# mbdriscoll/indigo

Hardware: AMD Instinct MI355X
Metric: SENSE AHA evals/sec (256^3 x 8-coil non-Cartesian) (higher is better)
Workload: dtype complex64 (f32)

## Files before the change

indigo_amd/backends/hip_csr.py:

```python
import logging

import numpy as np

from indigo_amd import _lib, grid_formats
from indigo_amd._lib import cplx as _cplx
from indigo_amd.backends.backend import Backend

log = logging.getLogger(__name__)
_C64 = np.dtype('complex64')

_BRICK_ARRAYS = dict(tasks=".brickTasks", table=".brickTable", entries=".brickEntries", rounds=".brickRoundRows", shared=".sharedBricks")
_SLOT_ARRAYS = dict(tasks=".slotTasks", table=".slotTable", entries=".slotEntries", slot_ptr=".slotPtr", shared=".slotSharedBricks")
_SHARE_ARRAYS = dict(tasks=".shareTasks", table=".shareTable", shares=".shares", shared=".shareSharedBricks")
_WIDE_ARRAYS = dict(owned=".wideOwnedTiles", tasks=".wideTasks", table=".wideTable", entries=".wideEntries", rows=".wideEntryRows")
_RUN_ARRAYS = dict(order=".runOrder", dptr=".runPtr", dcols=".runCols", entries=".runEntries")


def _ptr(a):
    return None if a is None else a._arr


class csr_matrix(Backend.csr_matrix):

    def __init__(self, backend, A, name='mat'):
        super().__init__(backend, A, name)
        self._host_csr = A if A.dtype == _C64 else A.astype(_C64)
        self._perm = self._sep = self._grid_dims = None
        self._support, self._support_host, self._support_zw = None, None, 16
        self._support_fine, self._support_fine_by, self._support_fine_host_by = None, {}, {}
        self._bricks, self._bricks_by, self._slots, self._slots_by, self._shares_by = None, {}, None, {}, {}
        self._invalidate()

    def _invalidate(self):
        self._t = None
        self._weights_real = None
        self._xrows = None
        self._values_re = self._runs_fmt = None
        self._wide = False
        self._tried = set()

    def _upload(self, fmt, names):
        if fmt is None:
            return None
        b = self._backend
        return dict(fmt, **{key: b.copy_array(fmt[key], name=self._name + suffix) for key, suffix in names.items() if fmt[key] is not None})

    def _host(self, part):
        if self._host_csr is not None:
            return getattr(self._host_csr, part)
        return dict(indptr=self.rowPtrs, indices=self.colInds, data=self.values)[part].to_host()

    def _transposed(self):
        if self._t is None:
            b = self._backend
            pt, it, dt = b.csr_transpose(self._host_csr)
            self._t = (b.copy_array(pt, name=self._name + ".T.rowPtrs"),
                       b.copy_array(it, name=self._name + ".T.colInds"),
                       b.copy_array(dt, name=self._name + ".T.data"))
            self._host_csr = None
        return self._t

    def set_grid_support(self, table, n0, nm, zw=16):
        self._support = (self._backend.copy_array(np.ascontiguousarray(table, dtype=np.int16).reshape(-1),
                                                  name=self._name + ".support"), int(n0), int(nm))
        self._support_zw = int(zw)
        self._support_host = table

    def set_grid_support_fine(self, table, tile, ncols=None):
        built, key = self._bricks_by, None if ncols is None else int(ncols)
        assert not (any(v is not None for v in built.values()) if key is None else built.get(key) is not None), \
            "set_grid_support_fine must come before set_grid_bricks: the runs of bricks are sized for the table's segments"
        assert int(tile) in (4, 8, 16)
        self._support_fine = (self._backend.copy_array(np.ascontiguousarray(table, dtype=np.int16).reshape(-1),
                                                       name=self._name + ".supportFine"), int(tile))
        self._support_fine_by[key] = self._support_fine
        self._support_fine_host_by[key] = (table, int(tile))

    def _format(self, which, ncols, exact=False):
        by = getattr(self, which + '_by')
        key = None if ncols is None else int(ncols)
        if key in by or exact:
            return by.get(key)
        return by.get(None)

    def _fine_tile(self, ncols):
        fine = self._format('_support_fine', ncols)
        return fine[1] if fine is not None else 16

    def set_grid_bricks(self, n0, nm, ns, ncols=8, bm=2, bs=2, chunk=4096, run=4096):
        A = self._host_csr
        assert A is not None and A.shape[1] == n0 * nm * ns
        fmt = grid_formats.bricks(A.indptr, A.indices, A.data, n0, nm, ns, ncols, bm, bs, chunk, run,
                                  tile=self._fine_tile(ncols), real_entries=self._real_weights(A.data))
        if fmt is None:
            log.info("%s: no brick-binned format (%s); the adjoint keeps the gather route", self._name, _lib.last_error(None))
        self._bricks = self._bricks_by[int(ncols)] = self._upload(fmt, _BRICK_ARRAYS)

    def set_grid_slots(self, n0, nm, ns, ncols=1, bm=2, bs=2, chunk=256, run=128):
        A = self._host_csr
        assert A is not None and A.shape[1] == n0 * nm * ns
        fmt = grid_formats.slots(A.indptr, A.indices, A.data, n0, nm, ns, ncols, bm, bs, chunk, run,
                                 tile=self._fine_tile(ncols), real_entries=self._real_weights(A.data))
        if fmt is None:
            log.info("%s: no slot format; the adjoint keeps the gather route", self._name)
        self._slots = self._slots_by[int(ncols)] = self._upload(fmt, _SLOT_ARRAYS)

    def set_grid_separable(self, sep):
        n0, nm, ns = (int(v) for v in sep['dims'])
        assert sep['records'].shape[0] == self.shape[0] and n0 * nm * ns == self.shape[1]
        rec = np.ascontiguousarray(sep['records'])
        self._sep = dict(tw=int(sep['tw']), dims=(n0, nm, ns), gconst=complex(sep['gconst']), host=rec, stride=rec.shape[1],
                         records=self._backend.copy_array(rec.reshape(-1), name=self._name + ".sepRecords"), recx=None, stride_x=0, order={})

    def _gather_order(self, ncols):
        by = self._sep['order']
        if ncols not in by:
            order = grid_formats.gather_order(self._sep['host'], self._sep['tw'], ncols)
            by[ncols] = None if order is None else self._backend.copy_array(order, name=self._name + ".gatherOrder%d" % ncols)
        return by[ncols]

    def set_grid_shares(self, ncols=8, bm=8, bs=2, chunk=1024, run=1024):
        sep = self._sep
        assert sep is not None
        fine = self._format('_support_fine_host', ncols)
        tab, tile = fine if fine is not None else (self._support_host, 16)
        fmt = grid_formats.shares(sep['host'], sep['tw'], sep['dims'], ncols, bm, bs, chunk, run,
                                  table=tab, tile=tile, zw=self._support_zw)
        if fmt is None:
            log.info("%s: no share format; the adjoint keeps the stored-tap routes", self._name)
        elif sep['recx'] is None:
            recx, sep['stride_x'] = grid_formats.records_with_rows(sep['host'])
            sep['recx'] = self._backend.copy_array(recx, name=self._name + ".sepRecordsWithRows")
        self._shares_by[int(ncols)] = self._upload(fmt, _SHARE_ARRAYS)

    def set_grid_dims(self, n0, nm, ns):
        assert int(n0) * int(nm) * int(ns) == self.shape[1]
        self._grid_dims = (int(n0), int(nm), int(ns))
        self._wide = False
        self._tried.discard('wide')

    def _dims(self):
        return self._grid_dims or grid_formats.guess_grid_dims(self.shape[1])

    def _wide_bricks(self):
        if 'wide' not in self._tried:
            self._tried.add('wide')
            t, data = self._backend.tuning, self._host('data')
            self._wide = self._upload(grid_formats.wide_bricks(
                self._host('indptr'), self._host('indices'), data, self.shape[1], self._dims(),
                t.get('wide_brick_shape', (2, 2)), t.get('wide_task_shape', (8192, 2048)), real_entries=self._real_weights(data)), _WIDE_ARRAYS)
        return self._wide

    def _touched(self):
        if self._xrows is None:
            b = self._backend
            indices = self._host('indices')
            mark = np.zeros(self.shape[1], dtype=bool)
            mark[indices] = True
            touched = np.flatnonzero(mark).astype(np.int32)
            compact = np.searchsorted(touched, indices).astype(np.int32)
            self._xrows = (b.copy_array(touched, name=self._name + ".touchedCols"), b.copy_array(compact, name=self._name + ".compactColInds"))
        return self._xrows

    def _runs(self, sub):
        if 'runs' not in self._tried:
            self._tried.add('runs')
            fmt = grid_formats.runs(self._host('indptr'), sub[1].to_host(), self._host('data'), sub[0].to_host(), self._dims(),
                                    self._backend.tuning.get('runs_order', True))
            if fmt is None:
                log.info("%s: no run format (%s); the forward product keeps the per-nonzero gather", self._name, _lib.last_error(None))
            self._runs_fmt = self._upload(fmt, _RUN_ARRAYS)
        return self._runs_fmt

    def set_row_order(self, perm):
        b = self._backend
        perm = np.ascontiguousarray(perm, dtype=np.int32)
        assert self._host_csr is not None and perm.shape == (self.shape[0],)
        Ap = self._host_csr[perm]
        Ap.sort_indices()
        self.rowPtrs = b.copy_array(Ap.indptr.astype(np.int32), name=self._name + ".rowPtrs")
        self.colInds = b.copy_array(Ap.indices.astype(np.int32), name=self._name + ".colInds")
        self.values = b.copy_array(Ap.data.astype(_C64), name=self._name + ".data")
        self._host_csr = Ap
        self._invalidate()
        self._perm = b.copy_array(perm, name=self._name + ".rowOrder")

    def _real_weights(self, data):
        if not self._backend.tuning.get('real_entries', True):
            return False
        if self._weights_real is None:
            self._weights_real = grid_formats.weights_are_real(data)
        return self._weights_real

    def _real_values(self):
        if 'values_re' not in self._tried:
            self._tried.add('values_re')
            data = self._host('data')
            if self._real_weights(data):
                self._values_re = self._backend.copy_array(np.ascontiguousarray(data.real, dtype=np.float32), name=self._name + ".dataRe")
        return self._values_re

    def forward_route(self, ncols):
        t = self._backend.tuning
        if self._grid_il:
            if self._sep is not None and ncols in (2, 4, 8) and t.get('sep_gather', True):
                return 'sep'
            return 'il_rw' if ncols in (2, 4, 8) and self._real_values() is not None else 'il'
        if self._perm is None and 16 <= ncols <= 64 and self._col_frac <= 0.6 and self.values.size >= self.shape[1] and t['xrows']:
            sub = self._touched()
            return 'xrows_runs' if ncols == 64 and t.get('runs', True) and sub[0].size * 512 < 2 ** 32 and self._runs(sub) is not None else 'xrows'
        return 'csr' if self._perm is None else 'rowperm'

    def adjoint_route(self, ncols, beta, y):
        b, perm = self._backend, self._perm
        scatter = perm is None and beta == 0 and y.contiguous
        shf = self._format('_shares', ncols, exact=True)
        if shf is not None and scatter and self._grid_il and shf['ntasks'] > 0 and b.tuning.get('sep_scatter', True):
            return 'shares'
        br = self._format('_bricks', ncols, exact=True)
        if br is not None and scatter and self._grid_il and ncols == br['ncols']:
            return 'bricks'
        sl = self._format('_slots', ncols, exact=True)
        if sl is not None and scatter and ncols == sl['ncols'] and sl['ntasks'] > 0:
            return 'slots'
        if (ncols == 64 and beta == 0 and perm is None and not self._grid_il and self.shape[1] % 16 == 0
# ... 107 lines not shown
```

indigo_amd/csrc/ig_fft.hip:

```cpp
#include "ig_common.h"
#include "ig_packed.h"
#include "ig_fft_ab.h"
#include "ig_fft_ab_list.h"
#include "ig_fft_zc.h"
#include <array>
#include <vector>
#include <functional>
#include <algorithm>
#include <cmath>
#include <cmath>
#include <cstring>
#include <string>
#include <memory>
#include <complex>

namespace {

constexpr int MAX_STAGES = 16;
constexpr int E = 8;
constexpr int LDS_NMAX = 4096;
constexpr size_t LDS_BUDGET = 150 * 1024;

struct Radices { int r[MAX_STAGES]; };

// ... 137 lines not shown
            z[0][r] = x[r];
#pragma unroll
            for (int q = 1; q < 4; ++q) z[q][r] = mul_w32(x[r + q * M], r * q * (32 / N));
        }
#pragma unroll
        for (int q = 0; q < 4; ++q) RegFFT<M>::run(z[q]);
#pragma unroll
        for (int q = 0; q < 4; ++q)
#pragma unroll
            for (int k = 0; k < M; ++k) x[4 * k + q] = z[q][k];
    }
};

template <int N> struct RegFFTHalfIn {
    __device__ static __forceinline__ void run(float2 (&x)[N]) {
        constexpr int M = N / 4;
        float2 z[4][M];
#pragma unroll
        for (int r = 0; r < M; ++r) {
            const float2 a1 = x[r + M], a2 = x[r + 2 * M];
            const float2 t3 = mul_mi(a1);
            z[0][r] = cadd(a2, a1);
            z[1][r] = mul_w32(csub(t3, a2), r * (32 / N));
            z[2][r] = mul_w32(csub(a2, a1), r * 2 * (32 / N));
            const float2 s = cadd(a2, t3);
            z[3][r] = mul_w32(make_float2(-s.x, -s.y), r * 3 * (32 / N));
        }
#pragma unroll
        for (int q = 0; q < 4; ++q) RegFFT<M>::run(z[q]);
#pragma unroll
        for (int q = 0; q < 4; ++q)
#pragma unroll
            for (int k = 0; k < M; ++k) x[4 * k + q] = z[q][k];
    }
};

__device__ __forceinline__ void pbfly2(cx& a, cx& b) { const cx t = a - b; a = a + b; b = t; }
template <bool INV = false, bool ASM = true>
__device__ __forceinline__ void pbfly4(cx& a0, cx& a1, cx& a2, cx& a3) {
    const cx t0 = a0 + a2, t1 = a0 - a2, t2 = a1 + a3, dd = a1 - a3;
    a0 = t0 + t2; a2 = t0 - t2;
    if (ASM) {
        a1 = INV ? padd_pi(t1, dd) : padd_mi(t1, dd);
        a3 = INV ? padd_mi(t1, dd) : padd_pi(t1, dd);
    } else {
        const cx t3 = INV ? cmul_pi_c(dd) : cmul_mi_c(dd);
        a1 = t1 + t3; a3 = t1 - t3;
    }
}
template <bool INV = false, bool ASM = true>
__device__ __forceinline__ cx pmul_w32(cx a, int j) {
    j &= 31;
    if (INV) j = (32 - j) & 31;
    if (j == 0) return a;
    if (j == 8) return ASM ? cmul_mi(a) : cmul_mi_c(a);
    if (j == 16) return cneg(a);
    if (j == 24) return ASM ? cmul_pi(a) : cmul_pi_c(a);
    const float c = cos32(j), s = -cos32(j + 24);
    return cxmul(a, mk(c, s));
}
template <int N, bool INV = false, bool ASM = true> struct PFFT;
template <bool INV, bool ASM> struct PFFT<4, INV, ASM> {
    __device__ static __forceinline__ void run(cx (&x)[4]) { pbfly4<INV, ASM>(x[0], x[1], x[2], x[3]); }
};
template <bool INV, bool ASM> struct PFFT<8, INV, ASM> {
    __device__ static __forceinline__ void run(cx (&v)[8]) {
        pbfly4<INV, ASM>(v[0], v[2], v[4], v[6]);
        pbfly4<INV, ASM>(v[1], v[3], v[5], v[7]);
        const float h = 0.70710678118654752440f;
        v[3] = cxmul(v[3], mk(h, INV ? h : -h));
        v[7] = cxmul(v[7], mk(-h, INV ? h : -h));
        pbfly2(v[0], v[1]); pbfly2(v[2], v[3]); pbfly2(v[6], v[7]);
        if (ASM) {
            const cx e = v[4], o = v[5];
            v[4] = INV ? padd_pi(e, o) : padd_mi(e, o);
            v[5] = INV ? padd_mi(e, o) : padd_pi(e, o);
        } else {
            v[5] = INV ? cmul_pi_c(v[5]) : cmul_mi_c(v[5]);
            pbfly2(v[4], v[5]);
        }
        const cx x4 = v[1], x1 = v[2], x5 = v[3], x2 = v[4], x6 = v[5], x3 = v[6];
        v[1] = x1; v[2] = x2; v[3] = x3; v[4] = x4; v[5] = x5; v[6] = x6;
    }
};
template <int N, bool INV, bool ASM> struct PFFT {
    __device__ static __forceinline__ void run(cx (&x)[N]) {
        constexpr int M = N / 4;
        cx z[4][M];
#pragma unroll
        for (int r = 0; r < M; ++r) {
            pbfly4<INV, ASM>(x[r], x[r + M], x[r + 2 * M], x[r + 3 * M]);
            z[0][r] = x[r];
#pragma unroll
            for (int q = 1; q < 4; ++q) z[q][r] = pmul_w32<INV, ASM>(x[r + q * M], r * q * (32 / N));
        }
#pragma unroll
        for (int q = 0; q < 4; ++q) PFFT<M, INV, ASM>::run(z[q]);
#pragma unroll
        for (int q = 0; q < 4; ++q)
#pragma unroll
            for (int k = 0; k < M; ++k) x[4 * k + q] = z[q][k];
    }
};
template <int N> struct PFFTHalfIn {
    __device__ static __forceinline__ void run(cx (&x)[N]) {
        constexpr int M = N / 4;
        cx z[4][M];
#pragma unroll
        for (int r = 0; r < M; ++r) {
            const cx a1 = x[r + M], a2 = x[r + 2 * M];
            z[0][r] = a2 + a1;
            z[1][r] = pmul_w32(cneg(padd_pi(a2, a1)), r * (32 / N));
            z[2][r] = pmul_w32(a2 - a1, r * 2 * (32 / N));
            z[3][r] = pmul_w32(cneg(padd_mi(a2, a1)), r * 3 * (32 / N));
        }
#pragma unroll
        for (int q = 0; q < 4; ++q) PFFT<M>::run(z[q]);
#pragma unroll
        for (int q = 0; q < 4; ++q)
#pragma unroll
            for (int k = 0; k < M; ++k) x[4 * k + q] = z[q][k];
    }
};

template <int R1, int R2, int T, int W, bool AXIS0, int WMODE, bool BOXED, int HALF>
__global__ void __launch_bounds__(W * T, (!AXIS0 && R1 == 32 && (W == 32 || HALF == 1 || HALF == 3)) ? 4 : 1)
k_fft_2stage(PassDesc d, const float2* __restrict__ tw) {
    constexpr int n = R1 * R2, B1 = R2 / T, B2 = R1 / T, NT = W * T;
    constexpr bool NT_LD = true, NT_ST = true;
    constexpr bool HALF_IN = HALF == 1 || HALF == 3, HALF_OUT = HALF == 2 || HALF == 4;
    constexpr int SUMW = WMODE >= 3 ? (1 << (WMODE - 3)) : 0;
    constexpr bool SINV = HALF_OUT;
    const bool inv = (HALF_OUT || HALF_IN) ? false : (d.inverse != 0);
    static_assert(R2 % T == 0 && R1 % T == 0 && T == 16 && B1 == 1, "lane groups of 16, one stage-1 butterfly per thread");
    extern __shared__ float2 lds[];
    float2* __restrict__ tws = lds + (AXIS0 ? 16 * 17 * W : 16 * T * W);
    const int tid = threadIdx.x;
    constexpr int TWN = n / NT;
    constexpr bool TW_LATE = (n % NT == 0) && TWN <= 2;
    float2 tw_mine[TW_LATE ? TWN : 1];
    if (TW_LATE) {
#pragma unroll
        for (int i = 0; i < TWN; ++i) tw_mine[i] = tw[n + tid + i * NT];
    } else for (int k = tid; k < n; k += NT) tws[k] = tw[n + k];

    const int t = AXIS0 ? (tid % T) : (tid / W);
    const int w = AXIS0 ? (tid / T) : (tid % W);
    unsigned tr, k1, k2;
    pass_tile(d, tr, k1, k2);
    const int64_t k0u = (int64_t)tr * ((!AXIS0 && d.cw) ? (d.cw_log2 >= 0 ? W >> d.cw_log2 : W / d.cw) : W);
    int in_lo = d.in_lo, in_hi = d.in_hi, out_lo = d.out_lo, out_hi = d.out_hi;
    short2 k1r = make_short2(0, 0x7fff), trg = make_short2(0, 0x7fff);
    PassRecords rcd{0u, 0u, 0x7fff0000u, 0xffffffffu, false, false, false, true, false};
    if (BOXED && !AXIS0) rcd = pass_records(d, tw, tr, k1, 16, t, true);
    const bool has_k1r = rcd.has_k1r, has_trg = rcd.has_trg, has_zb = rcd.has_zb;
    int64_t o_in = k0u * d.in_s[0], o_out = k0u * d.out_s[0];
    if (BOXED && !AXIS0 && WMODE == 0 && d.zc_log2) {
        const int64_t q = k0u >> d.zc_log2, e = k0u - (q << d.zc_log2);
        if (d.in_zt) o_in = q * d.in_zt + e;
        if (d.out_zt) o_out = q * d.out_zt + e;
    }
    const float2* const b_in = d.in + (o_in + (int64_t)k1 * d.in_s[1] + (int64_t)k2 * d.in_s[2]);
    float2* const b_out = d.out + (o_out + (int64_t)k1 * d.out_s[1] + (int64_t)k2 * d.out_s[2]);
    const float2* const b_w = WMODE ? d.w + (k0u * d.w_s[0] + (int64_t)k1 * d.w_s[1] + (int64_t)k2 * d.w_s[2]) : nullptr;
    const rsrc_t r_in = make_rsrc(b_in), r_out = make_rsrc(b_out), r_w = make_rsrc(b_w);
    const unsigned isj = AXIS0 ? 1u : (unsigned)d.in_sj, osj = AXIS0 ? 1u : (unsigned)d.out_sj, wsj = AXIS0 ? 1u : (unsigned)d.w_sj;
    bool valid;
    unsigned l_in, l_out, l_w;
    if (!AXIS0 && d.cw) {
        const unsigned yl = d.cw_log2 >= 0 ? (unsigned)w >> d.cw_log2 : (unsigned)w / (unsigned)d.cw, a = (unsigned)w - yl * (unsigned)d.cw;
        valid = k0u + yl < d.ext0;
        l_in = (a * (unsigned)d.in_sa + yl * (unsigned)d.in_s[0] + (unsigned)t * isj) * 8u;
        l_out = (a * (unsigned)d.out_sa + yl * (unsigned)d.out_s[0] + (unsigned)t * osj) * 8u;
        l_w = (a * (unsigned)d.w_sa + yl * (unsigned)d.w_s[0] + (unsigned)t * wsj) * 8u;
    } else {
        valid = k0u + w < d.ext0;
        l_in = ((unsigned)w * (unsigned)d.in_s[0] + (unsigned)t * isj) * 8u;
        l_out = ((unsigned)w * (unsigned)d.out_s[0] + (unsigned)t * osj) * 8u;
        l_w = ((unsigned)w * (unsigned)d.w_s[0] + (unsigned)t * wsj) * 8u;
    }
    if (!valid) l_in = l_out = l_w = IG_OOB;
    if (!WMODE) l_w = IG_OOB;
    if (SUMW && (w % SUMW) != 0) l_out = IG_OOB;
    if (has_k1r) k1r = rcd.k1_hull();
    if (has_k1r) {
        if ((int)k1 < k1r.x || (int)k1 >= k1r.y) return;
    }
    const bool defer_out = HALF_IN && has_trg && d.tile_range_mode == 1 && (rcd.scalar || has_k1r);
    if (has_trg && !defer_out) {
        const short2 r = trg = rcd.range();
        if (d.tile_range_mode == 1) {
            out_lo = out_lo > r.x ? out_lo : r.x;
            out_hi = out_hi < r.y ? out_hi : r.y;
            if (out_hi <= out_lo) return;
        } else {
            in_lo = in_lo > r.x ? in_lo : r.x;
            in_hi = in_hi < r.y ? in_hi : r.y;
        }
    }

    auto ceil16 = [](int a) -> int { a += 15; return a <= 0 ? 0 : (a >= 512 ? 32 : a >> 4); };
    auto below = [](int h) -> uint32_t { return h >= 32 ? 0xffffffffu : ((1u << h) - 1u); };
    uint32_t ibits = 0xffffffffu, obits = 0xffffffffu;
    if (BOXED) {
        ibits = below(ceil16(in_hi - t)) & ~below(ceil16(in_lo - t));
        if (has_zb && d.tile_range_mode != 1) ibits &= rcd.bits();
    }
    uint32_t gin = 0xffffffffu;
    if (BOXED && !AXIS0 && WMODE == 0 && !HALF_IN && HALF != 4) {
        gin = 0;
#pragma unroll
        for (int l = 0; l < 64; l += W) gin |= (uint32_t)__builtin_amdgcn_readlane((int)ibits, l);
    }
    constexpr bool GATE_ST = BOXED && !AXIS0 && WMODE == 0 && !HALF_OUT && HALF != 3;
    uint32_t gout = 0xffffffffu;
    constexpr int GRP = 4;
    auto opaque = [](const float2*& q) { asm("" : "+s"(q)); };
    cx v[R1];
    {
        cx wv[R1];
        constexpr int K0 = HALF_IN ? R1 / 4 : 0, K1 = HALF_IN ? 3 * R1 / 4 : R1;
        const int64_t st_in = (int64_t)R2 * d.in_sj, st_w = WMODE == 1 ? (int64_t)R2 * d.w_sj : 0;
        const unsigned so_in = (unsigned)st_in * 8u, so_w = (unsigned)st_w * 8u;
        const float2* p_in = AXIS0 ? b_in : b_in + K0 * st_in;
        const float2* p_w = (AXIS0 || WMODE != 1) ? b_w : b_w + K0 * st_w;
        rsrc_t g_in = make_rsrc(p_in), g_w = make_rsrc(p_w);
#pragma unroll
        for (int k = K0; k < K1; ++k) {
            const int g = (k - K0) % GRP;
            if (!AXIS0 && g == 0 && k > K0) {
                p_in += GRP * st_in; opaque(p_in); g_in = make_rsrc(p_in);
                if (WMODE == 1) { p_w += GRP * st_w; opaque(p_w); g_w = make_rsrc(p_w); }
            }
            const bool stat = !BOXED || HALF_IN || HALF == 4;
            const unsigned off = stat ? 0u : (unsigned)__builtin_amdgcn_sbfe((int)~ibits, k, 1);
            if (!stat && !AXIS0 && WMODE == 0 && !((gin >> k) & 1u)) v[k] = mk(0.f, 0.f);
            else if (AXIS0) {
                v[k] = from2(buf_ld<NT_LD>(r_in, l_in | off, (unsigned)(k * R2) * 8u));
                if (WMODE == 1) wv[k] = from2(buf_ld<false>(r_w, l_w | off, (unsigned)(k * R2) * 8u));
            } else {
                v[k] = from2(buf_ld<NT_LD>(g_in, l_in | off, (unsigned)g * so_in));
                if (WMODE == 1) wv[k] = from2(buf_ld<false>(g_w, l_w | off, (unsigned)g * so_w));
            }
        }
#pragma unroll
        for (int k = K0; k < K1; ++k) {
            if (WMODE == 1) v[k] = cxmul_r(v[k], wv[k]);
            if (inv) v[k] = cconj(v[k]);
        }
    }
    if (defer_out) {
        trg = rcd.range();
        out_lo = out_lo > trg.x ? out_lo : trg.x;
        out_hi = out_hi < trg.y ? out_hi : trg.y;
    }
    if (BOXED) {
        obits = below(ceil16(out_hi - t)) & ~below(ceil16(out_lo - t));
        if (has_zb && d.tile_range_mode == 1) obits &= rcd.bits();
    }
    if (GATE_ST) {
        gout = 0;
#pragma unroll
        for (int l = 0; l < 64; l += W) gout |= (uint32_t)__builtin_amdgcn_readlane((int)obits, l);
    }
    if (TW_LATE) {
#pragma unroll
        for (int i = 0; i < TWN; ++i) tws[tid + i * NT] = tw_mine[i];
    }
    __syncthreads();
    if (HALF_IN) PFFTHalfIn<R1>::run(v);
    else PFFT<R1, SINV>::run(v);
    {
        const float2* __restrict__ twt = tws + t * R1;
#pragma unroll
        for (int k = 1; k < R1; ++k) v[k] = SINV ? cxmulc(from2(twt[k]), v[k]) : cxmul_r(v[k], from2(twt[k]));
    }

    float2* __restrict__ lw = AXIS0 ? lds + w * (16 * 17) + t * 17 : lds + (t * 16) * W + w;
    float2* __restrict__ lr = AXIS0 ? lds + w * (16 * 17) + t      : lds + t * W + w;
#pragma unroll
    for (int q = 0; q < B2; ++q) {
        if (q > 0) __syncthreads();
#pragma unroll
        for (int kk = 0; kk < 16; ++kk) lw[kk * (AXIS0 ? 1 : W)] = to2(v[16 * q + kk]);
        __syncthreads();
        cx u[R2];
#pragma unroll
        for (int r = 0; r < R2; ++r) u[r] = from2(lr[r * (AXIS0 ? 17 : 16 * W)]);
        PFFT<R2, SINV>::run(u);
        constexpr int Q0 = HALF_OUT ? R2 / 4 : 0, Q1 = HALF_OUT ? 3 * R2 / 4 : R2;
        const int64_t st_out = (int64_t)R1 * d.out_sj, st_w = WMODE >= 2 ? (int64_t)R1 * d.w_sj : 0;
        const unsigned so_out = (unsigned)st_out * 8u, so_w = (unsigned)st_w * 8u;
        const float2* p_out = AXIS0 ? b_out : b_out + (q * T) * d.out_sj + Q0 * st_out;
        const float2* p_w = (AXIS0 || WMODE < 2) ? b_w : b_w + (q * T) * d.w_sj + Q0 * st_w;
        cx wv[R2];
        if (WMODE >= 2) {
            rsrc_t g_w = make_rsrc(p_w);
#pragma unroll
            for (int r = Q0; r < Q1; ++r) {
                const int g = (r - Q0) % GRP;
                if (!AXIS0 && g == 0 && r > Q0) { p_w += GRP * st_w; opaque(p_w); g_w = make_rsrc(p_w); }
                const bool stat = !BOXED || HALF_OUT || HALF == 3;
                const unsigned off = stat ? 0u : (unsigned)__builtin_amdgcn_sbfe((int)~obits, q + r * B2, 1);
                if (AXIS0) wv[r] = from2(buf_ld<false>(r_w, l_w | off, (unsigned)(q * T + r * R1) * 8u));
                else wv[r] = from2(buf_ld<false>(g_w, l_w | off, (unsigned)g * so_w));
            }
        }
        rsrc_t g_out = make_rsrc(p_out);
        v4i_t gw_out = make_rsrc_words(p_out);
#pragma unroll
        for (int r = Q0; r < Q1; ++r) {
            const int g = (r - Q0) % GRP;
            if (!AXIS0 && g == 0 && r > Q0) {
                p_out += GRP * st_out; opaque(p_out);
                if (GATE_ST) gw_out = make_rsrc_words(p_out); else g_out = make_rsrc(p_out);
            }
            const bool stat = !BOXED || HALF_OUT || HALF == 3;
            cx ac = u[r];
            if (inv) ac = cconj(ac);
            if (WMODE >= 2) ac = cxmulc(wv[r], ac);
            float2 a = to2(ac);
            const unsigned off = stat ? 0u : (unsigned)__builtin_amdgcn_sbfe((int)~obits, q + r * B2, 1);
            if (SUMW) {
                if (SUMW >= 2)  { a.x += dpp_f<0xB1>(a.x);  a.y += dpp_f<0xB1>(a.y); }
                if (SUMW >= 4)  { a.x += dpp_f<0x4E>(a.x);  a.y += dpp_f<0x4E>(a.y); }
                if (SUMW >= 8)  { a.x += dpp_f<0x104>(a.x); a.y += dpp_f<0x104>(a.y); }
                if (SUMW >= 16) { a.x += dpp_f<0x108>(a.x); a.y += dpp_f<0x108>(a.y); }
            }
            if (AXIS0) buf_st<NT_ST>(r_out, l_out | off, (unsigned)(q * T + r * R1) * 8u, a);
            else if (GATE_ST) buf_st_gated<NT_ST>(gw_out, l_out | off, (unsigned)g * so_out, a, (gout >> (q + r * B2)) & 1u);
            else buf_st<NT_ST>(g_out, l_out | off, (unsigned)g * so_out, a);
        }
    }
}


constexpr bool F3A_NT_LD = true, F3A_NT_ST = false, F3B_NT_LD = false, F3B_NT_ST = false;
constexpr int F3_LDS_ELEMS = 64 * 72;

__device__ __forceinline__ void wave_sync() {
    __builtin_amdgcn_fence(__ATOMIC_RELEASE, "wavefront");
    __builtin_amdgcn_wave_barrier();
    __builtin_amdgcn_fence(__ATOMIC_ACQUIRE, "wavefront");
}

__global__ void __launch_bounds__(512, 4)
k_fft3d_a(const float2* __restrict__ in, float2* __restrict__ out, const float2* __restrict__ tw, int inverse) {
    extern __shared__ float2 lds[];
    float2* __restrict__ tws = lds + F3_LDS_ELEMS;
    const int tid = threadIdx.x;
    for (int k = tid; k < 256; k += 512) tws[k] = tw[k];
    const unsigned lin = blockIdx.x + gridDim.x * (blockIdx.y + gridDim.y * blockIdx.z), tot = gridDim.x * gridDim.y * gridDim.z;
    const unsigned logical = (lin & 7u) * (tot >> 3) + (lin >> 3);
    const int n2 = (int)(logical & 3u), z = (int)((logical >> 2) & 255u);
    const int64_t base = ((int64_t)(logical >> 10) << 24) + ((int64_t)z << 16);
    const int xl = tid & 63, a = tid >> 6;
    const bool inv = inverse != 0;

    cx v[4][8];
    {
        const int a_u = __builtin_amdgcn_readfirstlane(a);
        const rsrc_t r_in = make_rsrc(in + base + 256 * n2 + 1024 * a_u);
#pragma unroll
        for (int b = 0; b < 8; ++b)
#pragma unroll
            for (int j = 0; j < 4; ++j) {
                v[j][b] = from2(buf_ld<F3A_NT_LD>(r_in, (unsigned)xl * 8u, (unsigned)(64 * j + 8192 * b) * 8u));
                if (inv) v[j][b] = cconj(v[j][b]);
            }
    }
    __syncthreads();
#pragma unroll
    for (int j = 0; j < 4; ++j) {
        PFFT<8, false, false>::run(v[j]);
#pragma unroll
        for (int kb = 1; kb < 8; ++kb) v[j][kb] = cxmul(v[j][kb], from2(tws[(4 * a * kb) & 255]));
    }
    cx r[4][8];
    float2* __restrict__ img1 = lds + F3_LDS_ELEMS + 256;
#pragma unroll
    for (int jp = 0; jp < 2; ++jp) {
        if (jp) __syncthreads();
#pragma unroll
        for (int kb = 0; kb < 8; ++kb) {
            lds[(a * 8 + kb) * 64 + xl] = to2(v[2 * jp][kb]);
            img1[(a * 8 + kb) * 64 + xl] = to2(v[2 * jp + 1][kb]);
        }
        __syncthreads();
#pragma unroll
        for (int ap = 0; ap < 8; ++ap) {
            r[2 * jp][ap] = from2(lds[(ap * 8 + a) * 64 + xl]);
            r[2 * jp + 1][ap] = from2(img1[(ap * 8 + a) * 64 + xl]);
        }
    }
    const int kb = a;
    cx p[8][4];
#pragma unroll
    for (int j = 0; j < 4; ++j) PFFT<8, false, false>::run(r[j]);
#pragma unroll
    for (int ka = 0; ka < 8; ++ka) {
        const cx wy = from2(tws[(n2 * (kb + 8 * ka)) & 255]);
        cx t4[4];
#pragma unroll
        for (int j = 0; j < 4; ++j) t4[j] = cxmul(r[j][ka], wy);
        PFFT<4, false, false>::run(t4);
        p[ka][0] = t4[0];
#pragma unroll
        for (int kj = 1; kj < 4; ++kj) p[ka][kj] = cxmul(t4[kj], from2(tws[(xl * kj) & 255]));
    }
    const int c = tid & 7, l = (tid >> 3) & 7, line = (tid >> 3);
    cx q[4][8];
#pragma unroll
    for (int jp = 0; jp < 2; ++jp) {
        __syncthreads();
#pragma unroll
        for (int ka = 0; ka < 8; ++ka) {
// ... 329 lines not shown
    const int64_t blocks = (ncols + anyfft::AB_W - 1) / anyfft::AB_W;
    IG_REQUIRE(ctx, blocks <= 0x7fffffffLL, "ig_fft_exec: too many tiles");
    const dim3 grid((unsigned)blocks), block((unsigned)(anyfft::AB_W * ax.ab_B));
    const bool ax0 = ax.inner == 1;
    int r = ig_ab_launch_part0(ctx->stream, ax.n, ax0, grid, block, ax.lds_bytes, in, out, ax.d_tw, ax.inner, ncols, inverse);
    if (!r) r = ig_ab_launch_part1(ctx->stream, ax.n, ax0, grid, block, ax.lds_bytes, in, out, ax.d_tw, ax.inner, ncols, inverse);
    if (!r) r = ig_ab_launch_part2(ctx->stream, ax.n, ax0, grid, block, ax.lds_bytes, in, out, ax.d_tw, ax.inner, ncols, inverse);
    if (!r) r = ig_ab_launch_part3(ctx->stream, ax.n, ax0, grid, block, ax.lds_bytes, in, out, ax.d_tw, ax.inner, ncols, inverse);
    if (r == 2) return ig_fail(ctx, IG_ERR_UNSUPPORTED, "ig_fft_exec: device %d refused %zu bytes of LDS for the %lld-point kernel", ctx->device, ax.lds_bytes, (long long)ax.n);
    if (!r) return ig_fail(ctx, IG_ERR_UNSUPPORTED, "ig_fft_exec: no A x B kernel for n = %lld", (long long)ax.n);
    IG_LAUNCH_CHECK(ctx, "k_fft_ab");
    return IG_OK;
}

int plan_chirp(ig_ctx* ctx, AxisPlan& ax, int64_t m);

int64_t chirp_ab_length(int64_t n, int& A, int& B) {
    int64_t m = 0;
    for (int64_t c = 2 * n - 1; c <= 1024 && c * 100 <= (2 * n - 1) * 108; ++c)
        if (ab_split(c, A, B)) { if (!m) m = c; if (B % 4 == 0) { m = c; break; } }
    for (int64_t c = 2 * n - 1; c <= 1024 && !m; ++c) if (ab_split(c, A, B)) m = c;
    if (m) ab_split(m, A, B);
    return m;
}

int plan_axis(ig_ctx* ctx, ig_fft* p, int a) {
    AxisPlan& ax = p->axis[a];
    ax.n = p->dims[a];
    ax.inner = 1;
    for (int d = 0; d < a; ++d) ax.inner *= p->dims[d];
    ax.outer = p->total / (ax.n * ax.inner);
    if (ax.n == 1) { ax.kind = 2; return IG_OK; }

    const bool force_generic = ctx->opt_fft_kernels == 2;
    Radices rad{};
    int ns = 0;
    const bool two_stage = !force_generic && (ax.n == 512 || ax.n == 256) &&
                           32 * ax.inner * 8 < 0x7fffffffLL;
    if (two_stage) {
        ax.kind = 3; ax.W = 16; ax.T = 16; ax.nstages = 2;
        ax.rad.r[0] = ax.n == 512 ? 32 : 16; ax.rad.r[1] = 16;
        ax.lds_bytes = ((size_t)16 * 17 * ax.W + ax.n) * 8;
    }
    const bool use_ab = ctx->opt_fft_kernels == 0;
    bool ab = false;
    if (!two_stage && !force_generic && use_ab) {
        int A = 0, B = 0;
        if (ab_split(ax.n, A, B)) {
            ab = true;
            ax.kind = 4; ax.ab_A = A; ax.ab_B = B; ax.W = anyfft::AB_W; ax.T = B; ax.nstages = 2;
            ax.rad.r[0] = A; ax.rad.r[1] = B;
            ax.lds_bytes = ab_lds(ax.n, ax.inner == 1);
        }
    }
    bool lds_ok = !ab && !two_stage && !force_generic && ax.n <= LDS_NMAX && factor_lds(ax.n, rad, ns);
    if (lds_ok) {
        int T = 1;
        for (int s = 0; s < ns; ++s) {
            const int R = rad.r[s];
            const int bpt = E / R;
            const int nb = (int)(ax.n / R);
            const int need = (nb + bpt - 1) / bpt;
            if (need > T) T = need;
        }
        int W = 16;
        while (W > 1 && ((int64_t)W * T > 1024 || ((size_t)ax.n * (W + 1) + ax.n) * 8 > 72 * 1024)) W >>= 1;
        while (W < 64 && (int64_t)(W * 2) * T <= 256 && ((size_t)ax.n * (2 * W + 1) + ax.n) * 8 <= 72 * 1024) W <<= 1;
        const size_t lds = ((size_t)ax.n * (W + 1) + ax.n) * 8;
        if ((int64_t)W * T > 1024 || lds > LDS_BUDGET) lds_ok = false;
        else {
            ax.kind = 0; ax.rad = rad; ax.nstages = ns; ax.W = W; ax.T = T; ax.lds_bytes = lds;
            if (lds > 48 * 1024) {
                IG_HIP(ctx, hipFuncSetAttribute(reinterpret_cast<const void*>(&k_fft_lds<true>),
                                                hipFuncAttributeMaxDynamicSharedMemorySize, (int)LDS_BUDGET));
                IG_HIP(ctx, hipFuncSetAttribute(reinterpret_cast<const void*>(&k_fft_lds<false>),
                                                hipFuncAttributeMaxDynamicSharedMemorySize, (int)LDS_BUDGET));
            }
        }
    }
    if (!lds_ok && !two_stage && !ab) {
        ax.kind = 1;
        factor_generic(ax.n, ax.gen_radices);
        ax.nstages = (int)ax.gen_radices.size();
        int64_t big = 1;
        for (int64_t r : ax.gen_radices) big = std::max(big, r);
        if (big > 7 && ax.n >= 32 && ctx->opt_fft_kernels == 0 && !p->is_chirp_sub) {
            int A = 0, B = 0;
            int64_t m = chirp_ab_length(ax.n, A, B);
            Radices r2{};
            int ns2 = 0;
            for (int64_t c = 2 * ax.n - 1; c <= LDS_NMAX && !m; ++c) if (factor_lds(c, r2, ns2)) m = c;
            if (m) {
                if (int rc = plan_chirp(ctx, ax, m)) return rc;
                ax.kind = 5;
            }
        }
    }
    const size_t ntw = (size_t)ax.n * (ax.kind == 3 ? 2 : 1);
    std::vector<float2> tw(ntw);
    for (int64_t k = 0; k < ax.n; ++k) {
        const double ang = -2.0 * M_PI * (double)k / (double)ax.n;
        tw[k] = make_float2((float)cos(ang), (float)sin(ang));
    }
    if (ax.kind == 3) {
        const int64_t R1 = ax.n / 16;
        for (int64_t t = 0; t < 16; ++t)
            for (int64_t k = 0; k < R1; ++k) tw[ax.n + t * R1 + k] = tw[(t * k) % ax.n];
    }
    IG_HIP(ctx, hipMalloc((void**)&ax.d_tw, sizeof(float2) * ntw));
    IG_HIP(ctx, hipMemcpy(ax.d_tw, tw.data(), sizeof(float2) * ntw, hipMemcpyHostToDevice));
    return IG_OK;
}

static dim3 pass_grid(PassDesc& d, int64_t tpr) {
    d.tpr = (unsigned)tpr;
    d.cw_log2 = -1;
    if (d.cw > 0 && (d.cw & (d.cw - 1)) == 0) { d.cw_log2 = 0; while ((1 << d.cw_log2) < d.cw) ++d.cw_log2; }
    const int64_t rows = d.ncols / d.ext0, ext2 = d.ext1 > 0 ? rows / d.ext1 : 0;
    d.grid3 = (d.ext1 >= 1 && d.ext1 <= 65535 && ext2 >= 1 && ext2 <= 65535 && d.ext1 * ext2 == rows) ? 1 : 0;
    return d.grid3 ? dim3((unsigned)tpr, (unsigned)d.ext1, (unsigned)ext2) : dim3((unsigned)(tpr * rows));
}

static int pass_tiles(ig_ctx* ctx, PassDesc& d, int64_t cpt, int64_t reach, bool weights, const char* kernel, dim3& grid) {
    const int64_t tpr = (d.ext0 + cpt - 1) / cpt;
    const int64_t blocks = tpr * (d.ncols / d.ext0);
    IG_REQUIRE(ctx, blocks <= 0x7fffffffLL && d.ext1 <= 0x7fffffffLL, "ig_fft: too many tiles");
    grid = pass_grid(d, tpr);
    const int64_t lim = 0x7fffffffLL / 8;
    const int64_t span_in = reach * d.in_sj + 15 * d.in_s[0] + 15 * d.in_sa, span_out = reach * d.out_sj + 15 * d.out_s[0] + 15 * d.out_sa;
    const int64_t span_w = weights ? reach * d.w_sj + 15 * d.w_s[0] + 15 * d.w_sa : 0;
    IG_REQUIRE(ctx, d.in_sj >= 0 && d.out_sj >= 0 && d.in_s[0] >= 0 && d.out_s[0] >= 0 && span_in < lim && span_out < lim && span_w < lim,
               "ig_fft: axis stride too large for the %s kernel", kernel);
    return IG_OK;
}

static bool two_stage_variant(const AxisPlan& ax, const PassDesc& d, bool axis0, int wmode, bool& boxed, int& half) {
    boxed = d.tile_range || !(d.in_lo <= 0 && d.in_hi >= (int)ax.n && d.out_lo <= 0 && d.out_hi >= (int)ax.n);
    const int qn = (int)ax.n / 4;
    half = 0;
    if (boxed) {
        const bool in_full = d.in_lo <= 0 && d.in_hi >= (int)ax.n, out_full = d.out_lo <= 0 && d.out_hi >= (int)ax.n;
        if (d.in_lo == qn && d.in_hi == 3 * qn && !(d.tile_range && d.tile_range_mode == 2))
            half = (out_full && !d.tile_range && !d.tile_bits) ? 3 : 1;
        else if (d.out_lo == qn && d.out_hi == 3 * qn && !(d.tile_range && d.tile_range_mode == 1))
            half = (in_full && !d.tile_range && !d.tile_bits) ? 4 : 2;
        if (wmode == 1 && half != 3) half = 0;
        if (wmode >= 2 && half != 4) half = 0;
        if (((half == 1 || half == 3) && d.inverse) || ((half == 2 || half == 4) && !d.inverse)) half = 0;
    }
    const bool big_stride = (d.in_sj > d.out_sj ? d.in_sj : d.out_sj) * 8 >= (1 << 20);
    const bool w32_generic = half == 0 && (big_stride || d.tile_bits != nullptr);
    const bool w32 = (ax.n == 512 && !axis0 && wmode == 0 && !d.cw && d.ext0 % 32 == 0 &&
        (half == 1 || half == 3 || half == 2 || half == 4 || w32_generic) &&
        (!d.tile_range || d.tile_shift >= 1));
    return d.wide ? d.wide == 2 : w32;
}

int launch_2stage(ig_ctx* ctx, const AxisPlan& ax, const PassDesc& d_in, bool axis0, int wmode) {
    PassDesc d = d_in;
    if (d.ncols == 0) return IG_OK;
    IG_REQUIRE(ctx, !d.tile_bits || d.tile_words == 16 || d.tile_words == 0, "ig_fft: the two-stage kernel reads support bitmaps of 16 words per entry (got %d)", d.tile_words);
    const int64_t cpt = (!axis0 && d.cw) ? ax.W / d.cw : ax.W;
    IG_REQUIRE(ctx, !d.cw || (!axis0 && d.cw <= ax.W && ax.W % d.cw == 0), "ig_fft: bad lane split");
    dim3 grid;
    if (int rc = pass_tiles(ctx, d, cpt, axis0 ? ax.n + 15 : 3 * (ax.n / 16) + 15, wmode != 0, "two-stage", grid)) return rc;
    const dim3 block((unsigned)(ax.W * ax.T));
#define IG_2S(R1_, AX0_, WM_, BX_, HF_)                                                             \
    hipLaunchKernelGGL((k_fft_2stage<R1_, 16, 16, 16, AX0_, WM_, BX_, HF_>), grid, block, ax.lds_bytes, ctx->stream, d, ax.d_tw)
#define IG_2S_W(R1_, AX0_)                                                                           \
    do {                                                                                             \
        if (!boxed && wmode == 0) IG_2S(R1_, AX0_, 0, false, 0);                                     \
        else if (wmode == 0) {                                                                       \
            if (half == 1) IG_2S(R1_, AX0_, 0, true, 1); else if (half == 2) IG_2S(R1_, AX0_, 0, true, 2);   \
            else if (half == 3) IG_2S(R1_, AX0_, 0, true, 3); else if (half == 4) IG_2S(R1_, AX0_, 0, true, 4); \
            else IG_2S(R1_, AX0_, 0, true, 0); }                                                     \
        else if (wmode == 1) { if (half == 3) IG_2S(R1_, AX0_, 1, true, 3); else IG_2S(R1_, AX0_, 1, true, 0); } \
        else { if (half == 4) IG_2S(R1_, AX0_, 2, true, 4); else IG_2S(R1_, AX0_, 2, true, 0); }      \
    } while (0)
    bool boxed; int half;
    const bool w32 = two_stage_variant(ax, d, axis0, wmode, boxed, half);
    if (w32) {
        PassDesc d2 = d;
        if (d2.tile_range) d2.tile_shift = d.tile_shift - 1;
        const dim3 g2 = pass_grid(d2, d.ext0 / 32), b2(512);
        const size_t lds2 = ((size_t)16 * 16 * 32 + 512) * 8;
        if (!ctx->fft_w32_attr) {
            IG_HIP(ctx, hipFuncSetAttribute(reinterpret_cast<const void*>(&k_fft_2stage<32, 16, 16, 32, false, 0, true, 1>), hipFuncAttributeMaxDynamicSharedMemorySize, (int)lds2));
            IG_HIP(ctx, hipFuncSetAttribute(reinterpret_cast<const void*>(&k_fft_2stage<32, 16, 16, 32, false, 0, true, 3>), hipFuncAttributeMaxDynamicSharedMemorySize, (int)lds2));
            IG_HIP(ctx, hipFuncSetAttribute(reinterpret_cast<const void*>(&k_fft_2stage<32, 16, 16, 32, false, 0, true, 2>), hipFuncAttributeMaxDynamicSharedMemorySize, (int)lds2));
            IG_HIP(ctx, hipFuncSetAttribute(reinterpret_cast<const void*>(&k_fft_2stage<32, 16, 16, 32, false, 0, true, 4>), hipFuncAttributeMaxDynamicSharedMemorySize, (int)lds2));
            IG_HIP(ctx, hipFuncSetAttribute(reinterpret_cast<const void*>(&k_fft_2stage<32, 16, 16, 32, false, 0, true, 0>), hipFuncAttributeMaxDynamicSharedMemorySize, (int)lds2));
            ctx->fft_w32_attr = true;
        }
        if (half == 0) hipLaunchKernelGGL((k_fft_2stage<32, 16, 16, 32, false, 0, true, 0>), g2, b2, lds2, ctx->stream, d2, ax.d_tw);
        else if (half == 1) hipLaunchKernelGGL((k_fft_2stage<32, 16, 16, 32, false, 0, true, 1>), g2, b2, lds2, ctx->stream, d2, ax.d_tw);
        else if (half == 3) hipLaunchKernelGGL((k_fft_2stage<32, 16, 16, 32, false, 0, true, 3>), g2, b2, lds2, ctx->stream, d2, ax.d_tw);
        else if (half == 2) hipLaunchKernelGGL((k_fft_2stage<32, 16, 16, 32, false, 0, true, 2>), g2, b2, lds2, ctx->stream, d2, ax.d_tw);
        else hipLaunchKernelGGL((k_fft_2stage<32, 16, 16, 32, false, 0, true, 4>), g2, b2, lds2, ctx->stream, d2, ax.d_tw);
    } else
    if (wmode == 3) {
        IG_REQUIRE(ctx, !axis0 && d.cw >= 1, "ig_fft: the coil-summing pass is a strided pass with a lane split");
#define IG_2S_SUM(R1_, HF_) do { switch (d.cw) { case 1: IG_2S(R1_, false, 3, true, HF_); break; case 2: IG_2S(R1_, false, 4, true, HF_); break; \
                                 case 4: IG_2S(R1_, false, 5, true, HF_); break; case 8: IG_2S(R1_, false, 6, true, HF_); break;              \
                                 default: IG_2S(R1_, false, 7, true, HF_); break; } } while (0)
        if (ax.n == 512) { if (half == 4) IG_2S_SUM(32, 4); else IG_2S_SUM(32, 0); }
        else             { if (half == 4) IG_2S_SUM(16, 4); else IG_2S_SUM(16, 0); }
#undef IG_2S_SUM
    } else
    if (ax.n == 512) { if (axis0) IG_2S_W(32, true); else IG_2S_W(32, false); }
    else             { if (axis0) IG_2S_W(16, true); else IG_2S_W(16, false); }
#undef IG_2S_W
#undef IG_2S
    IG_LAUNCH_CHECK(ctx, "k_fft_2stage");
    return IG_OK;
}

bool abd_supported(int64_t n) {
#define IG_ABD_CASE(A_, B_, R_) if (n == (A_) * (B_)) return true;
    IG_ABD_LIST(IG_ABD_CASE)
#undef IG_ABD_CASE
    return false;
}
int launch_ab_desc(ig_ctx* ctx, const AxisPlan& ax, const PassDesc& d_in, int wmode) {
    PassDesc d = d_in;
    if (d.ncols == 0) return IG_OK;
    IG_REQUIRE(ctx, !d.cw || (d.cw <= anyfft::AB_W && anyfft::AB_W % d.cw == 0), "ig_fft: bad lane split");
    IG_REQUIRE(ctx, !d.tile_bits || d.tile_words == (d.tile_range_mode == 1 ? ax.ab_A : ax.ab_B), "ig_fft: the support bitmap has %d words per entry, this pass needs %d",
               d.tile_words, d.tile_range_mode == 1 ? ax.ab_A : ax.ab_B);
    const int64_t cpt = d.cw ? anyfft::AB_W / d.cw : anyfft::AB_W;
    dim3 grid;
    if (int rc = pass_tiles(ctx, d, cpt, ax.ab_B - 1, wmode != 0, "two-stage", grid)) return rc;
    int wm = wmode;
    if (wmode == 3) {
        IG_REQUIRE(ctx, d.cw == 2 || d.cw == 4 || d.cw == 8 || d.cw == 16, "ig_fft: the coil-summing A x B pass takes 2, 4, 8 or 16 interleaved coils");
        wm = d.cw == 2 ? 4 : d.cw == 4 ? 5 : d.cw == 8 ? 6 : 7;
    }
    const dim3 block((unsigned)(anyfft::AB_W * ax.ab_B));
    int r = ig_abd_launch_part0(ctx->stream, ax.n, wm, grid, block, d, ax.d_tw);
    if (!r) r = ig_abd_launch_part1(ctx->stream, ax.n, wm, grid, block, d, ax.d_tw);
    if (!r) r = ig_abd_launch_part2(ctx->stream, ax.n, wm, grid, block, d, ax.d_tw);
    if (!r) r = ig_abd_launch_part3(ctx->stream, ax.n, wm, grid, block, d, ax.d_tw);
    if (r == 2) return ig_fail(ctx, IG_ERR_UNSUPPORTED, "ig_fft: device %d refused the LDS the %lld-point zero-pad-aware kernel needs", ctx->device, (long long)ax.n);
    if (!r)
        return ig_fail(ctx, IG_ERR_UNSUPPORTED, "ig_fft: no zero-pad-aware kernel for n = %lld", (long long)ax.n);
    IG_LAUNCH_CHECK(ctx, "k_fft_ab_desc");
    return IG_OK;
}

int plan_chirp(ig_ctx* ctx, AxisPlan& ax, int64_t m) {
    auto ch = std::make_shared<Chirp>();
    ch->m = m;
    const int64_t n = ax.n;
    {
        ig_fft tmp;
        tmp.ctx = ctx; tmp.is_chirp_sub = true; tmp.rank = 3; tmp.batch = 1;
        tmp.dims[0] = ax.inner; tmp.dims[1] = m; tmp.dims[2] = ax.outer;
        tmp.total = ax.inner * m * ax.outer;
        if (int rc = plan_axis(ctx, &tmp, 1)) return rc;
        ch->sub = tmp.axis[1];
        tmp.axis[1].d_tw = nullptr;
    }
    IG_REQUIRE(ctx, ch->sub.kind == 0 || ch->sub.kind == 3 || ch->sub.kind == 4, "ig_fft_plan: no fast kernel for the chirp-z length %lld", (long long)m);
    ch->fused = ch->sub.kind == 4 && ax.inner >= 16;
    typedef std::complex<double> cd;
    std::vector<cd> b((size_t)n), h((size_t)m, cd(0, 0)), H((size_t)m);
    for (int64_t j = 0; j < n; ++j) {
        const double ang = -M_PI * (double)((j * j) % (2 * n)) / (double)n;
        b[j] = cd(cos(ang), sin(ang));
    }
    h[0] = cd(1, 0);
    for (int64_t j = 1; j < n; ++j) h[j] = h[m - j] = std::conj(b[j]);
    {
        std::vector<double> cs((size_t)m);
        for (int64_t k = 0; k < m; ++k) cs[k] = cos(2.0 * M_PI * (double)k / (double)m);
        for (int64_t k = 0; k < m; ++k) {
            cd acc = h[0];
            for (int64_t j = 1; j < n; ++j) acc += 2.0 * h[j] * cs[(j * k) % m];
            H[k] = acc;
        }
    }
    std::vector<float2> t((size_t)m);
    auto upload = [&](float2*& dst, const std::function<cd(int64_t)>& f) -> int {
        for (int64_t k = 0; k < m; ++k) { const cd v = f(k); t[k] = make_float2((float)v.real(), (float)v.imag()); }
        IG_HIP(ctx, hipMalloc((void**)&dst, sizeof(float2) * (size_t)m));
        IG_HIP(ctx, hipMemcpy(dst, t.data(), sizeof(float2) * (size_t)m, hipMemcpyHostToDevice));
        return IG_OK;
    };
    for (int dir = 0; dir < 2; ++dir) {
        auto cj = [dir](cd v) { return dir ? std::conj(v) : v; };
        if (int rc = upload(ch->d_b[dir], [&](int64_t k) { return k < n ? cj(b[k]) : cd(0, 0); })) return rc;
        if (int rc = upload(ch->d_bhat[dir], [&](int64_t k) { return cj(H[k]); })) return rc;
        if (int rc = upload(ch->d_bout[dir], [&](int64_t k) { return k < n ? cj(b[k]) / (double)m : cd(0, 0); })) return rc;
        IG_HIP(ctx, hipMalloc((void**)&ch->d_hat_out[dir], sizeof(float2) * 2 * (size_t)m));
        IG_HIP(ctx, hipMemcpy(ch->d_hat_out[dir], ch->d_bhat[dir], sizeof(float2) * (size_t)m, hipMemcpyDeviceToDevice));
        IG_HIP(ctx, hipMemcpy(ch->d_hat_out[dir] + m, ch->d_bout[dir], sizeof(float2) * (size_t)m, hipMemcpyDeviceToDevice));
    }
    ax.chirp = ch;
    return IG_OK;
}

int plan_chirp_shift(ig_ctx* ctx, Chirp& ch, int64_t n, int64_t c) {
    typedef std::complex<double> cd;
    const int64_t m = ch.m;
    for (int d = 0; d < 2; ++d) {
        if (ch.d_in_s[d]) { (void)hipFree(ch.d_in_s[d]); ch.d_in_s[d] = nullptr; }
        if (ch.d_hat_out_s[d]) { (void)hipFree(ch.d_hat_out_s[d]); ch.d_hat_out_s[d] = nullptr; }
    }
    ch.shift = c;
    if (c == 0) return IG_OK;
    auto bt = [n](int64_t t) { const double ang = -M_PI * (double)((t * t) % (2 * n)) / (double)n; return cd(cos(ang), sin(ang)); };
    std::vector<double> cs((size_t)m), sn((size_t)m);
    for (int64_t k = 0; k < m; ++k) { cs[k] = cos(2.0 * M_PI * (double)k / (double)m); sn[k] = sin(2.0 * M_PI * (double)k / (double)m); }
    std::vector<float2> t((size_t)(2 * m));
    for (int dir = 0; dir < 2; ++dir) {
        std::vector<cd> h((size_t)m, cd(0, 0)), H((size_t)m);
        for (int64_t u = -(n - 1); u <= n - 1; ++u)
            h[(size_t)((u % m + m) % m)] = dir == 0 ? std::conj(bt(u + c)) : bt(u - c);
        for (int64_t k = 0; k < m; ++k) {
            cd acc(0, 0);
            for (int64_t u = 0; u < m; ++u) {
                if (h[u] == cd(0, 0)) continue;
                const int64_t q = (u * k) % m;
                acc += h[u] * cd(cs[q], -sn[q]);
            }
            H[k] = acc;
        }
        for (int64_t j = 0; j < m; ++j) {
            const cd v = j < n ? (dir == 0 ? bt(j - c) : std::conj(bt(j))) : cd(0, 0);
            t[j] = make_float2((float)v.real(), (float)v.imag());
        }
        IG_HIP(ctx, hipMalloc((void**)&ch.d_in_s[dir], sizeof(float2) * (size_t)m));
        IG_HIP(ctx, hipMemcpy(ch.d_in_s[dir], t.data(), sizeof(float2) * (size_t)m, hipMemcpyHostToDevice));
        for (int64_t k = 0; k < m; ++k) {
            t[k] = make_float2((float)H[k].real(), (float)H[k].imag());
            const cd v = k < n ? (dir == 0 ? bt(k) : std::conj(bt(k - c))) / (double)m : cd(0, 0);
            t[m + k] = make_float2((float)v.real(), (float)v.imag());
// ... 168 lines not shown
            d.in_sj = d.out_sj = ax.inner; d.w_sj = 0;
            d.ncols = ax.inner * ax.outer;
            if (ax.inner == 1) {
                d.ext0 = ax.outer; d.ext1 = 1; d.in_s[0] = d.out_s[0] = ax.n; d.in_s[1] = d.out_s[1] = 0;
            } else {
                d.ext0 = ax.inner; d.ext1 = ax.outer; d.in_s[0] = d.out_s[0] = 1; d.in_s[1] = d.out_s[1] = ax.inner * ax.n;
            }
            d.in_s[2] = d.out_s[2] = 0;
            d.in_lo = d.out_lo = 0; d.in_hi = d.out_hi = (int)ax.n; d.inverse = inv;
            return launch_2stage(ctx, ax, d, ax.inner == 1, 0);
        }
        if (ax.kind == 4) {
            ig_prof_scope prof(ctx, a == 0 ? "fft_ab_axis0" : a == 1 ? "fft_ab_axis1" : "fft_ab_axis2", bytes);
            return launch_ab(ctx, ax, in, out, inv);
        }
        IG_REQUIRE(ctx, ax.kind == 0, "ig_fft_exec: not a fast axis");
        ig_prof_scope prof(ctx, a == 0 ? "fft_lds_axis0" : a == 1 ? "fft_lds_axis1" : "fft_lds_axis2", bytes);
        const int64_t ncols = ax.inner * ax.outer;
        const int64_t blocks = (ncols + ax.W - 1) / ax.W;
        IG_REQUIRE(ctx, blocks <= 0x7fffffffLL, "ig_fft_exec: too many tiles");
        const dim3 grid((unsigned)blocks), block((unsigned)(ax.W * ax.T));
        if (ax.inner == 1)
            hipLaunchKernelGGL(k_fft_lds<true>, grid, block, ax.lds_bytes, ctx->stream, in, out, ax.d_tw,
                               (int)ax.n, ax.inner, ncols, ax.W, ax.T, ax.nstages, ax.rad, inv);
        else
            hipLaunchKernelGGL(k_fft_lds<false>, grid, block, ax.lds_bytes, ctx->stream, in, out, ax.d_tw,
                               (int)ax.n, ax.inner, ncols, ax.W, ax.T, ax.nstages, ax.rad, inv);
        IG_LAUNCH_CHECK(ctx, "k_fft_lds");
        return IG_OK;
    };
    for (int a = 0; a < p->rank; ++a) {
        const AxisPlan& ax = p->axis[a];
        if (ax.kind == 2) continue;
        if (ax.kind == 0 || ax.kind == 3 || ax.kind == 4) {
            if (int rc = fast_axis(ax, cur, y, inverse, a, pass_bytes)) return rc;
            cur = y;
        } else if (ax.kind == 5) {
            const Chirp& ch = *ax.chirp;
            const int dir = inverse ? 1 : 0;
            if (cur == work) {
                IG_HIP(ctx, hipMemcpyAsync(y, cur, (size_t)p->total * 8, hipMemcpyDeviceToDevice, ctx->stream));
                cur = y;
            }
            if (ch.fused) {
                ig_prof_scope prof(ctx, a == 1 ? "fft_chirp_axis1" : "fft_chirp_axis2", pass_bytes);
                PassDesc d{};
                d.in = cur; d.in_sj = ax.inner; d.in_s[0] = 1; d.in_s[1] = ax.inner * ax.n;
                d.out = y; d.out_sj = ax.inner; d.out_s[0] = 1; d.out_s[1] = ax.inner * ax.n;
                d.ext0 = ax.inner; d.ext1 = ax.outer; d.ncols = ax.inner * ax.outer;
                d.in_lo = d.out_lo = 0; d.in_hi = d.out_hi = (int)ax.n; d.inverse = inverse;
                if (int rc = launch_chirp_desc(ctx, ax, d)) return rc;
            } else {
                const int64_t total_m = p->total / ax.n * ch.m;
                int64_t g = (total_m + 255) / 256;
                const int64_t cap = (int64_t)ctx->num_cu * 16;
                if (g > cap) g = cap;
                {
                    ig_prof_scope prof(ctx, "fft_chirp_pre");
                    hipLaunchKernelGGL(k_chirp_pre, dim3((unsigned)g), dim3(256), 0, ctx->stream, cur, work, ch.d_b[dir], ax.n, ch.m, ax.inner, total_m);
                    IG_LAUNCH_CHECK(ctx, "k_chirp_pre");
                }
                if (int rc = fast_axis(ch.sub, work, work, 0, a, 0.0)) return rc;
                {
                    ig_prof_scope prof(ctx, "fft_chirp_mul");
                    hipLaunchKernelGGL(k_chirp_mul, dim3((unsigned)g), dim3(256), 0, ctx->stream, work, ch.d_bhat[dir], ch.m, ax.inner, total_m);
                    IG_LAUNCH_CHECK(ctx, "k_chirp_mul");
                }
                if (int rc = fast_axis(ch.sub, work, work, 1, a, 0.0)) return rc;
                {
                    ig_prof_scope prof(ctx, "fft_chirp_post");
                    hipLaunchKernelGGL(k_chirp_post, dim3((unsigned)g), dim3(256), 0, ctx->stream, (const float2*)work, y, ch.d_bout[dir], ax.n, ch.m, ax.inner, p->total);
                    IG_LAUNCH_CHECK(ctx, "k_chirp_post");
                }
            }
            cur = y;
        } else {
            int64_t Ns = 1;
            int64_t g = (p->total + 255) / 256;
            const int64_t cap = (int64_t)ctx->num_cu * 16;
            if (g > cap) g = cap;
            for (size_t s = 0; s < ax.gen_radices.size(); ++s) {
                const int64_t R = ax.gen_radices[s];
                IG_REQUIRE(ctx, R <= 0x7fffffffLL, "ig_fft_exec: radix too large");
                float2* dst = (cur == y) ? work : y;
                ig_prof_scope prof(ctx, "fft_generic_stage", pass_bytes / (double)ax.gen_radices.size());
                hipLaunchKernelGGL(k_fft_generic_stage, dim3((unsigned)g), dim3(256), 0, ctx->stream,
                                   cur, dst, ax.d_tw, ax.n, ax.inner, p->total, (int)R, Ns, inverse);
                IG_LAUNCH_CHECK(ctx, "k_fft_generic_stage");
                cur = dst;
                Ns *= R;
            }
        }
    }
    if (cur != y) {
        IG_HIP(ctx, hipMemcpyAsync(y, cur, (size_t)p->total * 8, hipMemcpyDeviceToDevice, ctx->stream));
    }
    return IG_OK;
}


int ig_fft_plan_padded(ig_ctx* ctx, const int64_t* dims, const int64_t* box_lo, const int64_t* box_dims,
                       int64_t batch, int grid_layout, ig_fft** plan, size_t* workspace_bytes) {
    IG_REQUIRE(ctx, ctx && dims && box_lo && box_dims && plan, "ig_fft_plan_padded: bad arguments");
    IG_REQUIRE(ctx, grid_layout >= 0 && grid_layout <= 2, "ig_fft_plan_padded: grid_layout must be 0 (x,y,z), 1 (x,z,y) or 2 (c,x,z,y)");
    IG_REQUIRE(ctx, grid_layout != 2 || batch == 1 || batch == 2 || batch == 4 || batch == 8 || batch == 16,
               "ig_fft_plan_padded: the coil-interleaved layout needs a batch of 1, 2, 4, 8 or 16 (got %lld)", (long long)batch);
    for (int a = 0; a < 3; ++a) {
        IG_REQUIRE(ctx, box_lo[a] >= 0 && box_dims[a] >= 1 && box_lo[a] + box_dims[a] <= dims[a],
                   "ig_fft_plan_padded: box [%lld, %lld) outside grid axis %d of length %lld", (long long)box_lo[a],
                   (long long)(box_lo[a] + box_dims[a]), a, (long long)dims[a]);
    }
    size_t ws = 0;
    int rc = ig_fft_plan(ctx, 3, dims, batch, plan, &ws);
    if (rc != IG_OK) return rc;
    ig_fft* p = *plan;
    for (int a = 0; a < 3; ++a) {
        const bool cz_ok = p->axis[a].kind == 5 && p->axis[a].chirp->sub.kind == 4 && a >= 1 && grid_layout == 2 && batch >= 2;
        if (cz_ok) p->axis[a].chirp->fused = true;
        const bool ab_ok = (p->axis[a].kind == 4 && abd_supported(dims[a]) && grid_layout == 2 && batch >= 2) || cz_ok;
        if (p->axis[a].kind != 3 && !ab_ok) {
            ig_fft_destroy(p);
            *plan = nullptr;
            return ig_fail(ctx, IG_ERR_UNSUPPORTED,
                           "ig_fft_plan_padded: grid axis %d has length %lld; the padded path needs 256 or 512 -- or, with 2, 4, 8 or 16 "
                           "coil-interleaved batch members (grid_layout 2: a chunk of any coil count padded to such a width, indigo_amd.fused.plan_chunks), "
                           "any length from 128 to 640 with factors 2, 3, 5, 7 only that splits as A x B with A, B <= 32, or on the y / z axes a length "
                           "with a larger prime factor (chirp-z)", a, (long long)dims[a]);
        }
        if (ab_ok) p->has_ab_axis = true;
        if (a == 2) { p->zw_in = cz_ok ? p->axis[a].chirp->sub.ab_B : ab_ok ? p->axis[a].ab_B : 16; p->zw_out = cz_ok ? p->axis[a].chirp->sub.ab_B : ab_ok ? p->axis[a].ab_A : 16; }
        if (cz_ok) p->has_chirp_axis = true;
        p->box_lo[a] = box_lo[a];
        p->box_dims[a] = box_dims[a];
    }
    p->padded = true;
    p->layout = grid_layout;
    p->workspace_bytes = ((size_t)p->total + (size_t)(dims[0] * box_dims[1] * box_dims[2] * batch)) * 8;
    if (workspace_bytes) *workspace_bytes = p->workspace_bytes;
    p->desc = std::string("padded layout=") + (grid_layout == 2 ? "cxzy " : grid_layout ? "xzy " : "xyz ") + p->desc;
    return IG_OK;
}

typedef std::array<int64_t, 4> Strides;

struct PaddedGeom {
    int64_t n[3], b[3], l[3], C;
    int64_t vol, bvol, cvol;
    bool interleaved;
    Strides img, wgt, mid, grid;
    bool mid_in_grid;
    int64_t mid_base;
    int64_t snt;
    int tile_shift;
    int zw_in, zw_out;
    int64_t hull_y, bits, bits_out;
};

static int lg2(int64_t v) { int s = 0; while ((1LL << s) < v) ++s; return s; }

static PaddedGeom padded_geom(const ig_fft* p, bool inverse, int64_t x_bstride, bool sum_coils) {
    PaddedGeom g{};
    for (int a = 0; a < 3; ++a) { g.n[a] = p->dims[a]; g.b[a] = p->box_dims[a]; g.l[a] = p->box_lo[a]; }
    const int64_t n0 = g.n[0], n1 = g.n[1], n2 = g.n[2], b0 = g.b[0], b1 = g.b[1], C = g.C = p->batch;
    g.vol = n0 * n1 * n2; g.bvol = b0 * b1 * g.b[2]; g.cvol = n0 * b1 * g.b[2];
    g.interleaved = p->layout == 2;
    const int64_t k = g.interleaved ? C : 1;
    if (g.interleaved && inverse) g.img = sum_coils ? Strides{1, b0, b0 * b1, 0} : Strides{C, C * b0, C * b0 * b1, 1};
    else g.img = {1, b0, b0 * b1, x_bstride};
    g.wgt = {k, k * b0, k * b0 * b1, g.interleaved ? 1 : g.bvol};
    if (p->layout == 0) g.grid = {1, n0, n0 * n1, g.vol};
    else g.grid = {k, k * n0 * n2, k * n0, g.interleaved ? 1 : g.vol};
    g.mid_in_grid = p->layout == 0;
    if (g.mid_in_grid) { g.mid = g.grid; g.mid_base = g.l[1] * n0 + g.l[2] * n0 * n1; }
    else g.mid = {k, k * n0, k * n0 * b1, g.interleaved ? 1 : g.cvol};
    if (p->layout >= 1) {
        g.snt = n0 / p->support_tile;
        g.tile_shift = g.interleaved ? lg2((int)(C * p->support_tile / 16)) : 0;
        g.zw_in = p->zw_in; g.zw_out = p->zw_out;
        g.hull_y = n1 * g.snt; g.bits = g.hull_y + g.snt;
        g.bits_out = g.zw_out != g.zw_in ? n1 * g.snt * g.zw_in : 0;
    }
    return g;
}

struct PaddedBufs { float2* img; float2* grid; float2* full; float2* mid; };

static PaddedBufs padded_bufs(const ig_fft* p, const PaddedGeom& g, float2* img, float2* grid, float2* full, float2* work) {
    return PaddedBufs{img, grid, full, g.mid_in_grid ? full + g.mid_base : work + (size_t)p->total};
}

static void pass_strides(const PaddedGeom& g, const Strides& S, int a, int64_t& sj, int64_t& sa, int64_t* s) {
    sj = S[a]; s[0] = S[a == 0 ? 1 : 0]; s[1] = S[a == 2 ? 1 : 2];
    if (!g.interleaved) s[2] = S[3];
    else if (a == 0) sa = S[3];
    else s[0] = S[3];
}

static PassDesc pass_desc(const PaddedGeom& g, int a, bool inverse, float2* box, const Strides& box_s, float2* full, const Strides& full_s,
                          int64_t e0, int64_t e1) {
    PassDesc d{};
    const bool lanes = g.interleaved && a == 0, folded = g.interleaved && a != 0;
    const int lo = (int)g.l[a], hi = (int)(g.l[a] + g.b[a]), n = (int)g.n[a];
    d.inverse = inverse ? 1 : 0;
    d.in = inverse ? full : box; d.out = inverse ? box : full;
    pass_strides(g, inverse ? full_s : box_s, a, d.in_sj, d.in_sa, d.in_s);
    pass_strides(g, inverse ? box_s : full_s, a, d.out_sj, d.out_sa, d.out_s);
    d.in_lo = inverse ? 0 : lo; d.in_hi = inverse ? n : hi; d.out_lo = inverse ? lo : 0; d.out_hi = inverse ? hi : n;
    d.cw = lanes ? (int)g.C : 0;
    d.ext0 = e0 * (folded ? g.C : 1); d.ext1 = e1; d.ncols = e0 * e1 * (lanes ? 1 : g.C);
    return d;
}

static PassDesc pass_x(const PaddedGeom& g, bool inverse, const PaddedBufs& m, const float2* w, int64_t z0, int64_t nz, bool sum_coils,
                       int& wmode, bool& axis0) {
    PassDesc d = pass_desc(g, 0, inverse, m.img - g.l[0] * g.img[0] + z0 * g.img[2], g.img, m.mid + z0 * g.mid[2], g.mid, g.b[1], nz);
    d.w = w ? w - g.l[0] * g.wgt[0] + z0 * g.wgt[2] : nullptr;
    pass_strides(g, g.wgt, 0, d.w_sj, d.w_sa, d.w_s);
    wmode = sum_coils ? 3 : !w ? 0 : inverse ? 2 : 1;
    axis0 = !g.interleaved;
    return d;
}

static PassDesc pass_y(const PaddedGeom& g, bool inverse, const PaddedBufs& m, const short2* support, int64_t z0, int64_t nz) {
    PassDesc d = pass_desc(g, 1, inverse, m.mid - g.l[1] * g.mid[1] + z0 * g.mid[2], g.mid, m.full + (g.l[2] + z0) * g.grid[2], g.grid, g.n[0], nz);
    if (support) { d.tile_range = support + g.hull_y; d.tile_range_mode = inverse ? 2 : 1; d.tile_range_k1 = 0; d.tile_shift = g.tile_shift; }
    return d;
}

static PassDesc pass_z(const PaddedGeom& g, bool inverse, const PaddedBufs& m, const short2* support) {
    PassDesc d = pass_desc(g, 2, inverse, m.full, g.grid, m.grid, g.grid, g.n[0], g.n[1]);
    if (g.snt) {
        d.tile_range = support; d.tile_range_mode = inverse ? 2 : 1; d.tile_range_k1 = g.snt; d.tile_shift = g.tile_shift;
    }
    if (support) {
        d.tile_bits = reinterpret_cast<const uint32_t*>(support + g.bits) + (inverse ? 0 : g.bits_out);
        d.tile_words = inverse ? g.zw_in : g.zw_out;
        if (inverse) d.k1_range = support + g.hull_y;
    }
    return d;
}

static bool zc_route(const ig_fft* p, const PaddedGeom& g, float2* zc, bool inverse, int64_t z0, PassDesc& dy, PassDesc& dz) {
    if (!p->ctx->opt_fft_zc || !g.interleaved || !zc || p->axis[1].kind != 3 || p->axis[2].kind != 3) return false;
    bool by, bz; int half;
    const bool wy = two_stage_variant(p->axis[1], dy, false, 0, by, half), wz = two_stage_variant(p->axis[2], dz, false, 0, bz, half);
    if (!by || !bz || (wy && !wz)) return false;
    const ZcGeom z{g.n[0], g.n[1], g.b[2], g.C, wz ? 32 : 16};
    if (!zc_valid(z)) return false;
    const ZcSide sy = zc_side(z, 1), sz = zc_side(z, 2);
    float2* const y_base = zc + zc_offset(z, 0, 0, z0, 0);
    float2* const z_base = zc - g.l[2] * sz.sj;
    if (!inverse) {
        dy.out = y_base; dy.out_sj = sy.sj; dy.out_s[0] = 1; dy.out_s[1] = sy.s1; dy.out_s[2] = 0; dy.out_zt = sy.zt;
        dz.in = z_base;  dz.in_sj = sz.sj;  dz.in_s[0] = 1;  dz.in_s[1] = sz.s1;  dz.in_s[2] = 0;  dz.in_zt = sz.zt;
    } else {
        dz.out = z_base; dz.out_sj = sz.sj; dz.out_s[0] = 1; dz.out_s[1] = sz.s1; dz.out_s[2] = 0; dz.out_zt = sz.zt;
        dy.in = y_base;  dy.in_sj = sy.sj;  dy.in_s[0] = 1;  dy.in_s[1] = sy.s1;  dy.in_s[2] = 0;  dy.in_zt = sy.zt;
    }
    dy.zc_log2 = dz.zc_log2 = sz.piece_log2;
    dy.wide = wy ? 2 : 1; dz.wide = wz ? 2 : 1;
    return true;
}

static int exec_padded(ig_fft* p, float2* x, int64_t x_bstride, const float2* w, float2* y, float2* work, const short2* support) {
    ig_ctx* ctx = p->ctx;
    const PaddedGeom g = padded_geom(p, false, x_bstride, false);
    const PaddedBufs m = padded_bufs(p, g, x, y, y, work);
    const int64_t plane = g.n[0] * g.n[1], b2 = g.b[2];
    PassDesc dy = pass_y(g, false, m, support, 0, b2), dz = pass_z(g, false, m, support);
    zc_route(p, g, work, false, 0, dy, dz);
    {
        ig_prof_scope prof(ctx, "fft_pad_x", (double)(g.bvol + (w ? g.bvol : 0) + g.cvol) * g.C * 8.0);
        int wmode; bool axis0;
        const PassDesc d = pass_x(g, false, m, w, 0, b2, false, wmode, axis0);
        if (int rc = launch_pass(ctx, p->axis[0], d, axis0, wmode)) return rc;
    }
    {
        ig_prof_scope prof(ctx, "fft_pad_y", (double)(g.cvol + plane * b2) * g.C * 8.0);
        if (int rc = launch_pass(ctx, p->axis[1], dy, false, 0)) return rc;
    }
    {
        ig_prof_scope prof(ctx, "fft_pad_z", (double)(plane * b2 + g.vol) * g.C * 8.0);
        if (int rc = launch_pass(ctx, p->axis[2], dz, false, 0)) return rc;
    }
    return IG_OK;
}

static int exec_cropped(ig_fft* p, float2* y, const float2* w, float2* x, int64_t x_bstride, float2* work, const short2* support,
                        bool sum_coils, int phases, int64_t z0, int64_t z1) {
    ig_ctx* ctx = p->ctx;
    const PaddedGeom g = padded_geom(p, true, x_bstride, sum_coils);
    const PaddedBufs m = padded_bufs(p, g, x, y, work, work);
    const int64_t plane = g.n[0] * g.n[1], b2 = g.b[2];
    const int64_t nz = z1 - z0;
    PassDesc dy = pass_y(g, true, m, support, z0, nz > 0 ? nz : 0), dz = pass_z(g, true, m, support);
    zc_route(p, g, work, true, z0, dy, dz);
    if (phases & 1) {
        ig_prof_scope prof(ctx, "fft_crop_z", (double)(g.vol + plane * b2) * g.C * 8.0);
        if (int rc = launch_pass(ctx, p->axis[2], dz, false, 0)) return rc;
    }
    if (!(phases & 2) || nz <= 0) return IG_OK;
    {
        ig_prof_scope prof(ctx, "fft_crop_y", (double)(plane * nz + g.n[0] * g.b[1] * nz) * g.C * 8.0);
        if (int rc = launch_pass(ctx, p->axis[1], dy, false, 0)) return rc;
    }
    {
        const double bytes = sum_coils ? (double)(g.cvol + g.bvol) * g.C * 8.0 + (double)g.bvol * 8.0 : (double)(g.cvol + g.bvol + (w ? g.bvol : 0)) * g.C * 8.0;
        ig_prof_scope prof(ctx, "fft_crop_x", bytes * (double)nz / (double)b2);
        int wmode; bool axis0;
        const PassDesc d = pass_x(g, true, m, w, z0, nz, sum_coils, wmode, axis0);
        if (int rc = launch_pass(ctx, p->axis[0], d, axis0, wmode)) return rc;
    }
    return IG_OK;
}

int64_t ig_fft_zc_size(const int64_t* dims, const int64_t* box_dims, int64_t coils, int64_t piece_bytes) {
    if (!dims || !box_dims || piece_bytes < 8 || piece_bytes % 8) return -1;
    const ZcGeom z{dims[0], dims[1], box_dims[2], coils, piece_bytes / 8};
    return zc_valid(z) && box_dims[2] <= dims[2] ? zc_size(z) * 8 : -1;
}

int64_t ig_fft_zc_offset(const int64_t* dims, const int64_t* box_dims, int64_t coils, int64_t piece_bytes, int64_t kx, int64_t ky, int64_t z, int64_t coil) {
    if (ig_fft_zc_size(dims, box_dims, coils, piece_bytes) < 0) return -1;
    const ZcGeom g{dims[0], dims[1], box_dims[2], coils, piece_bytes / 8};
    if (kx < 0 || kx >= g.n0 || ky < 0 || ky >= g.n1 || z < 0 || z >= g.b2 || coil < 0 || coil >= g.C) return -1;
    return zc_offset(g, kx, ky, z, coil) * 8;
}

int ig_fft_support_words(int64_t n, int* zw_in, int* zw_out) {
    if (!zw_in || !zw_out) return ig_fail(nullptr, IG_ERR_ARG, "ig_fft_support_words: bad arguments");
    int A = 0, B = 0;
    if (n == 256 || n == 512) { *zw_in = *zw_out = 16; return IG_OK; }
    if (abd_supported(n) && ab_split(n, A, B)) { *zw_in = B; *zw_out = A; return IG_OK; }
    {
        const int64_t big = largest_prime_factor(n);
        if (big > 7 && n >= 32 && chirp_ab_length(n, A, B) && n <= 32 * (int64_t)B) { *zw_in = *zw_out = B; return IG_OK; }
    }
    return ig_fail(nullptr, IG_ERR_UNSUPPORTED, "ig_fft_support_words: no zero-pad-aware z pass for an axis of %lld points", (long long)n);
}

int ig_fft_padded_axis_kind(int64_t n, int* kind) {
    if (!kind || n < 1) return ig_fail(nullptr, IG_ERR_ARG, "ig_fft_padded_axis_kind: bad arguments");
    int A = 0, B = 0;
    *kind = 0;
    if (n == 256 || n == 512) { *kind = 3; return IG_OK; }
    if (abd_supported(n)) { *kind = 4; return IG_OK; }
    const int64_t big = largest_prime_factor(n);
    if (big > 7 && n >= 32)
        for (int64_t c = 2 * n - 1; c <= 1024; ++c) if (ab_split(c, A, B)) { *kind = 5; break; }
    return IG_OK;
}

int ig_fft_set_axis_shift(ig_fft* p, int axis, int64_t shift) {
    if (!p) return ig_fail(nullptr, IG_ERR_ARG, "ig_fft_set_axis_shift: plan is NULL");
    ig_ctx* ctx = p->ctx;
    IG_REQUIRE(ctx, p->padded && p->layout == 2 && axis >= 1 && axis < p->rank, "ig_fft_set_axis_shift: the y or z axis of a zero-padded plan of the coil-interleaved layout");
    AxisPlan& ax = p->axis[axis];
    IG_REQUIRE(ctx, shift >= 0 && shift < ax.n, "ig_fft_set_axis_shift: shift %lld outside [0, %lld)", (long long)shift, (long long)ax.n);
    if (shift == 0 && !(ax.kind == 5 && ax.chirp && ax.chirp->shift)) return IG_OK;
    if (!(ax.kind == 5 && ax.chirp && ax.chirp->fused))
        return ig_fail(ctx, IG_ERR_UNSUPPORTED, "ig_fft_set_axis_shift: axis %d (%lld points) is no one-launch chirp-z axis", axis, (long long)ax.n);
    if (int rc = ig_set_device(ctx)) return rc;
    IG_HIP(ctx, hipStreamSynchronize(ctx->stream));
    return plan_chirp_shift(ctx, *ax.chirp, ax.n, shift);
}

int ig_fft_set_support_tile(ig_fft* p, int tile) {
    if (!p) return ig_fail(nullptr, IG_ERR_ARG, "ig_fft_set_support_tile: plan is NULL");
    ig_ctx* ctx = p->ctx;
    IG_REQUIRE(ctx, p->padded && p->layout == 2, "ig_fft_set_support_tile: a zero-padded plan of the coil-interleaved layout");
    IG_REQUIRE(ctx, (tile == 2 || tile == 4 || tile == 8 || tile == 16) && p->batch * tile >= 16 && p->dims[0] % tile == 0,
               "ig_fft_set_support_tile: tile %d (2, 4, 8 or 16 kx points; coils * tile >= 16)", tile);
    p->support_tile = tile;
    return IG_OK;
}

static int check_padded_exec(ig_fft* p, const char* fn, int need_layout, bool arrays, const int16_t* support,
                             bool slab = false, int phase = 0, int64_t z0 = 0, int64_t z1 = 0) {
    if (!p) return ig_fail(nullptr, IG_ERR_ARG, "%s: plan is NULL", fn);
    ig_ctx* ctx = p->ctx;
    if (need_layout == 1) IG_REQUIRE(ctx, p->padded && p->layout == 1, "%s: needs a plan of ig_fft_plan_padded with grid_layout 1 (layout 2: ig_fft_exec_cropped_sum_slab)", fn);
    else if (need_layout == 2) IG_REQUIRE(ctx, p->padded && p->layout == 2, "%s: needs a plan of ig_fft_plan_padded with grid_layout 2", fn);
    else IG_REQUIRE(ctx, p->padded, "%s: plan was not made by ig_fft_plan_padded", fn);
    IG_REQUIRE(ctx, arrays, "%s: NULL array", fn);
    IG_REQUIRE(ctx, !support || (p->layout >= 1 && (!p->has_chirp_axis || p->layout == 2)), "%s: a support table needs grid layout 1 or 2 (chirp-z axes: layout 2, hulls only)", fn);
// ... 66 lines not shown
```

indigo_amd/csrc/ig_fft_ab.h:

```cpp
#pragma once
#include <type_traits>

struct PassDesc {
    const float2* in; float2* out; const float2* w;
    const float2* w2;
    int chirp_out;
    int64_t in_sj, out_sj, w_sj;
    int64_t in_s[3], out_s[3], w_s[3];
    int64_t ext0, ext1, ncols;
    unsigned tpr;
    int grid3;
    int cw_log2;
    int cw;
    int64_t in_sa, out_sa, w_sa;
    int tile_shift;
    int in_lo, in_hi, out_lo, out_hi;
    int inverse;
    const short2* tile_range;
    int tile_range_mode;
    int64_t tile_range_k1;
    const uint32_t* tile_bits;
    int tile_words;
    const short2* k1_range;
    int zc_log2;
    int64_t in_zt, out_zt;
    int wide;
};


#include "ig_packed.h"

__device__ __forceinline__ void pass_tile(const PassDesc& d, unsigned& tr, unsigned& k1, unsigned& k2) {
    if (d.grid3) { tr = blockIdx.x; k1 = blockIdx.y; k2 = blockIdx.z; }
    else { const unsigned tile = blockIdx.x, rest = tile / d.tpr; tr = tile % d.tpr; k1 = rest % (unsigned)d.ext1; k2 = rest / (unsigned)d.ext1; }
}
struct PassRecords {
    uint32_t rec_v, rec_s, hull_s, zb_raw;
    bool has_k1r, has_trg, has_zb, word_ok, scalar;
    __device__ __forceinline__ short2 k1_hull() const { return make_short2((short)(hull_s & 0xffffu), (short)(hull_s >> 16)); }
    __device__ __forceinline__ short2 range() const {
        const uint32_t a = scalar ? rec_s : (uint32_t)__builtin_amdgcn_readfirstlane((int)rec_v);
        return make_short2((short)(a & 0xffffu), (short)(a >> 16));
    }
    __device__ __forceinline__ uint32_t bits() const { return has_zb ? (word_ok ? zb_raw : 0u) : 0xffffffffu; }
};
__device__ __forceinline__ PassRecords pass_records(const PassDesc& d, const void* safe, unsigned tr, unsigned k1, int words, int word, bool word_ok) {
    PassRecords r;
    r.rec_v = 0; r.rec_s = 0; r.hull_s = 0x7fff0000u; r.zb_raw = 0xffffffffu; r.word_ok = word_ok;
    r.has_k1r = d.k1_range != nullptr; r.has_trg = d.tile_range != nullptr; r.has_zb = d.tile_bits != nullptr;
    r.scalar = r.has_trg && d.tile_range_k1 == 0;
    if (r.has_k1r) r.hull_s = *reinterpret_cast<const uint32_t*>(d.k1_range + (tr >> d.tile_shift));
    if (r.scalar) r.rec_s = *reinterpret_cast<const uint32_t*>(d.tile_range + (tr >> d.tile_shift));
    if ((r.has_trg && !r.scalar) || r.has_zb) {
        const int64_t tidx = (int64_t)k1 * d.tile_range_k1 + (tr >> d.tile_shift);
        const uint32_t* pt = (r.has_trg && !r.scalar) ? reinterpret_cast<const uint32_t*>(d.tile_range + tidx) : reinterpret_cast<const uint32_t*>(safe);
        const uint32_t* pb = (r.has_zb && word_ok) ? d.tile_bits + (tidx * words + word) : reinterpret_cast<const uint32_t*>(safe);
        r.zb_raw = *pb;
        r.rec_v = *pt;
    }
    return r;
}

namespace anyfft {

constexpr double kPi = 3.14159265358979323846264338327950288;

constexpr double c_cos_x(double x) {
    double x2 = x * x, term = 1.0, sum = 1.0;
    for (int k = 1; k <= 16; ++k) { term *= -x2 / ((2.0 * k - 1.0) * (2.0 * k)); sum += term; }
    return sum;
}
constexpr double c_sin_x(double x) {
    double x2 = x * x, term = x, sum = x;
    for (int k = 1; k <= 16; ++k) { term *= -x2 / ((2.0 * k) * (2.0 * k + 1.0)); sum += term; }
    return sum;
}
constexpr int c_mod(int m, int n) { return ((m % n) + n) % n; }
constexpr double c_angle(int m, int n) {
    int r = c_mod(m, n);
    if (2 * r > n) r -= n;
    return 2.0 * kPi * (double)r / (double)n;
}
constexpr float cos2pi(int m, int n) {
    const int r = c_mod(m, n);
    if (r == 0) return 1.0f;
    if (2 * r == n) return -1.0f;
    if (4 * r == n || 4 * r == 3 * n) return 0.0f;
    return (float)c_cos_x(c_angle(m, n));
}
constexpr float sin2pi(int m, int n) {
    const int r = c_mod(m, n);
    if (r == 0 || 2 * r == n) return 0.0f;
    if (4 * r == n) return 1.0f;
    if (4 * r == 3 * n) return -1.0f;
    return (float)c_sin_x(c_angle(m, n));
}

template <int I, int N, typename F>
__device__ __forceinline__ void static_for(F&& f) {
    if constexpr (I < N) {
        f(std::integral_constant<int, I>{});
        static_for<I + 1, N>(f);
    }
}

__device__ __forceinline__ float2 d_add(float2 a, float2 b) { return make_float2(a.x + b.x, a.y + b.y); }
__device__ __forceinline__ float2 d_sub(float2 a, float2 b) { return make_float2(a.x - b.x, a.y - b.y); }
__device__ __forceinline__ float2 d_addmi(float2 a, float2 b) { return make_float2(a.x + b.y, a.y - b.x); }
__device__ __forceinline__ float2 d_addpi(float2 a, float2 b) { return make_float2(a.x - b.y, a.y + b.x); }
__device__ __forceinline__ float2 d_fma_r(float c, float2 t, float2 acc) { return make_float2(fmaf(c, t.x, acc.x), fmaf(c, t.y, acc.y)); }
__device__ __forceinline__ float2 d_mul_r(float c, float2 t) { return make_float2(c * t.x, c * t.y); }
__device__ __forceinline__ cx d_add(cx a, cx b) { return a + b; }
__device__ __forceinline__ cx d_sub(cx a, cx b) { return a - b; }
__device__ __forceinline__ cx d_addmi(cx a, cx b) { return padd_mi(a, b); }
__device__ __forceinline__ cx d_addpi(cx a, cx b) { return padd_pi(a, b); }
__device__ __forceinline__ cx d_fma_r(float c, cx t, cx acc) { return cfma_r(c, t, acc); }
__device__ __forceinline__ cx d_mul_r(float c, cx t) { cx r; r.v = t.v * v2f{c, c}; return r; }

template <int M, int N>
__device__ __forceinline__ float2 rot(float2 a) {
    constexpr int r = c_mod(M, N);
    if constexpr (r == 0) return a;
    else if constexpr (4 * r == N) return make_float2(a.y, -a.x);
    else if constexpr (2 * r == N) return make_float2(-a.x, -a.y);
    else if constexpr (4 * r == 3 * N) return make_float2(-a.y, a.x);
    else {
        constexpr float c = cos2pi(r, N), s = -sin2pi(r, N);
        return make_float2(fmaf(a.x, c, -a.y * s), fmaf(a.x, s, a.y * c));
    }
}
template <int M, int N>
__device__ __forceinline__ cx rot(cx a) {
    constexpr int r = c_mod(M, N);
    if constexpr (r == 0) return a;
    else if constexpr (4 * r == N) return cmul_mi(a);
    else if constexpr (2 * r == N) return cneg(a);
    else if constexpr (4 * r == 3 * N) return cmul_pi(a);
    else {
        constexpr float c = cos2pi(r, N), s = -sin2pi(r, N);
        return cxmul(a, mk(c, s));
    }
}

constexpr int pick_radix(int n) { return n % 4 == 0 ? 4 : n % 2 == 0 ? 2 : n % 3 == 0 ? 3 : n % 5 == 0 ? 5 : n % 7 == 0 ? 7 : n; }

template <int N, typename T = float2, bool BASE = (pick_radix(N) == N)>
struct RegDFT;

template <typename T> struct RegDFT<1, T, true> { __device__ static __forceinline__ void run(T (&)[1]) {} };
template <typename T> struct RegDFT<2, T, true> {
    __device__ static __forceinline__ void run(T (&x)[2]) {
        const T a = x[0], b = x[1];
        x[0] = d_add(a, b); x[1] = d_sub(a, b);
    }
};
template <typename T> struct RegDFT<4, T, true> {
    __device__ static __forceinline__ void run(T (&x)[4]) {
        const T t0 = d_add(x[0], x[2]), t1 = d_sub(x[0], x[2]), t2 = d_add(x[1], x[3]), d = d_sub(x[1], x[3]);
        x[0] = d_add(t0, t2); x[2] = d_sub(t0, t2);
        x[1] = d_addmi(t1, d); x[3] = d_addpi(t1, d);
    }
};
template <int P, typename T>
struct RegDFT<P, T, true> {
    static_assert(P == 3 || P == 5 || P == 7, "RegDFT: lengths with factors 2, 3, 5, 7 only");
    __device__ static __forceinline__ void run(T (&x)[P]) {
        constexpr int H = (P - 1) / 2;
        T t[H], d[H];
        static_for<0, H>([&](auto q_) {
            constexpr int q = decltype(q_)::value + 1;
            t[q - 1] = d_add(x[q], x[P - q]);
            d[q - 1] = d_sub(x[q], x[P - q]);
        });
        const T x0 = x[0];
        T s0 = x0;
        static_for<0, H>([&](auto q_) { s0 = d_add(s0, t[decltype(q_)::value]); });
        x[0] = s0;
        static_for<0, H>([&](auto k_) {
            constexpr int k = decltype(k_)::value + 1;
            T a = x0, b = d_mul_r(sin2pi(k, P), d[0]);
            static_for<0, H>([&](auto q_) {
                constexpr int q = decltype(q_)::value + 1;
                constexpr float c = cos2pi(q * k, P), s = sin2pi(q * k, P);
                a = d_fma_r(c, t[q - 1], a);
                if constexpr (q > 1) b = d_fma_r(s, d[q - 1], b);
            });
            x[k] = d_addmi(a, b);
            x[P - k] = d_addpi(a, b);
        });
    }
};
template <int N, typename T>
struct RegDFT<N, T, false> {
    __device__ static __forceinline__ void run(T (&x)[N]) {
        constexpr int P = pick_radix(N), Q = N / P;
        T y[Q][P];
        static_for<0, Q>([&](auto n2_) {
            constexpr int n2 = decltype(n2_)::value;
            T a[P];
            static_for<0, P>([&](auto n1_) { constexpr int n1 = decltype(n1_)::value; a[n1] = x[Q * n1 + n2]; });
            RegDFT<P, T>::run(a);
            static_for<0, P>([&](auto k1_) { constexpr int k1 = decltype(k1_)::value; y[n2][k1] = rot<n2 * k1, N>(a[k1]); });
        });
// ... 382 lines not shown
```

indigo_amd/csrc/ig_spmm.hip:

```cpp
#include "ig_spmm_common.h"
#include <hip/amd_detail/amd_hip_unsafe_atomics.h>
#include <algorithm>
#include <atomic>
#include <cstring>
#include <type_traits>

namespace {

struct GridMask {
    const uint32_t* bits;
    int64_t n0, nm;
};

constexpr int WL_SUB = 32;
struct WorkLists {
    int32_t*  rows[2];
    uint32_t* count;
    uint32_t  cap;
    const int32_t* yperm;
};

__device__ __forceinline__ bool wl_append(const WorkLists& wl, int which, int sub, bool want, int32_t row) {
    const uint64_t bal = __ballot(want);
    if (!bal) return false;
// ... 734 lines not shown
                float2 sum = make_float2(0.f, 0.f);
#pragma unroll
                for (int w = 0; w < 16; ++w) sum = cadd(sum, part[w][tid]);
                if (col_ok) {
                    float2* yp = Y + j * ldy + out_row(yperm, row) * syr;
                    float2 out = cmul(alpha, sum);
                    if (BMODE == 1) cfma(out, beta, *yp);
                    *yp = out;
                }
            }
            __syncthreads();
        }
    }
}

template <int CL, int NL, bool ATOMIC>
__global__ void __launch_bounds__(BLK)
k_csrmm_scatter(int64_t M, int64_t N,
                const int32_t* __restrict__ rowptr, const int32_t* __restrict__ colind,
                const float2* __restrict__ vals,
                const float2* __restrict__ X, int64_t ldx,
                float2* __restrict__ Y, int64_t ldy,
                float2 alpha, int xcd_remap) {
    constexpr int RPW = 64 / (CL * NL);
    const int lane = threadIdx.x & 63;
    const int c = lane % CL;
    const int i = (lane / CL) % NL;
    const int r = lane / (CL * NL);
    const int64_t blk = xcd_remap ? xcd_block(blockIdx.x, gridDim.x) : (int64_t)blockIdx.x;
    const int64_t wave = blk * WAVES_PER_BLOCK + (threadIdx.x >> 6);
    const int64_t row = wave * RPW + r;
    if (row >= M) return;
    const int32_t p0 = rowptr[row], p1 = rowptr[row + 1];
    if (p0 == p1) return;

    for (int64_t jb = 0; jb < N; jb += CL) {
        const int64_t j = jb + c;
        if (j >= N) continue;
        const float2 ax = cmul(alpha, X[j * ldx + row]);
        float2* __restrict__ ycol = Y + j * ldy;
        for (int32_t p = p0 + i; p < p1; p += NL) {
            const int32_t k = colind[p];
            const float2 t = cmulc(vals[p], ax);
            if (ATOMIC) {
                unsafeAtomicAdd(&ycol[k].x, t.x);
                unsafeAtomicAdd(&ycol[k].y, t.y);
            } else {
                float2 y = ycol[k];
                y.x += t.x; y.y += t.y;
                ycol[k] = y;
            }
        }
    }
}

template <bool ZERO>
__global__ void __launch_bounds__(BLK)
k_panel_scale(int64_t rows, int64_t N, float2* __restrict__ Y, int64_t ld, float2 beta) {
    const int64_t j = blockIdx.y;
    float2* __restrict__ col = Y + j * ld;
    for (int64_t k = (int64_t)blockIdx.x * BLK + threadIdx.x; k < rows; k += (int64_t)gridDim.x * BLK) {
        if (ZERO) col[k] = make_float2(0.f, 0.f);
        else      col[k] = cmul(beta, col[k]);
    }
}

template <int NP>
__global__ void __launch_bounds__(BLK)
k_pack_panel(int64_t rows, int64_t N, const float2* __restrict__ X, int64_t ld, float2* __restrict__ Xp,
             const int32_t* __restrict__ xperm) {
    for (int64_t e = (int64_t)blockIdx.x * BLK + threadIdx.x; e < rows * NP; e += (int64_t)gridDim.x * BLK) {
        const int64_t k = e / NP;
        const int c = (int)(e % NP);
        const int64_t src = xperm ? (int64_t)xperm[k] : k;
        Xp[e] = c < N ? X[c * ld + src] : make_float2(0.f, 0.f);
    }
}

template <int NP>
__global__ void __launch_bounds__(BLK)
k_pack_panel_tiled(int64_t rows, int64_t N, const float2* __restrict__ X, int64_t ld, float2* __restrict__ Xp,
                   const int32_t* __restrict__ xperm) {
    __shared__ float2 tile[NP][65];
    const int tid = threadIdx.x;
    const int kk = tid & 63, c0 = tid >> 6;
    constexpr int PER = NP / (BLK / 64);
    float2 v[PER];
    auto load = [&](int64_t k0) {
        const int64_t k = k0 + kk;
        const int64_t src = k < rows ? (xperm ? (int64_t)xperm[k] : k) : 0;
#pragma unroll
        for (int u = 0; u < PER; ++u) {
            const int c = c0 + u * (BLK / 64);
            v[u] = (c < N && k < rows) ? X[c * ld + src] : make_float2(0.f, 0.f);
        }
    };
    int64_t k0 = (int64_t)blockIdx.x * 64;
    if (k0 < rows) load(k0);
    for (; k0 < rows; k0 += (int64_t)gridDim.x * 64) {
#pragma unroll
        for (int u = 0; u < PER; ++u) tile[c0 + u * (BLK / 64)][kk] = v[u];
        __syncthreads();
        const int64_t kn = k0 + (int64_t)gridDim.x * 64;
        if (kn < rows) load(kn);
        for (int e = tid; e < 64 * NP; e += BLK) {
            const int r = e / NP, c = e % NP;
            if (k0 + r < rows) Xp[(k0 + r) * NP + c] = tile[c][r];
        }
        __syncthreads();
    }
}

}

int ig_pack_panel(ig_ctx* ctx, int64_t rows, int64_t N, int np, const float2* X, int64_t ldx, const int32_t* xperm,
                  bool may_decline, const float2** packed) {
    *packed = nullptr;
    const size_t need = (size_t)rows * np * 8;
    if (may_decline && (need == 0 || need > ((size_t)16 << 30))) return IG_OK;
    if (ctx->xpack_bytes < need) {
        if (may_decline) {
            size_t free_b = 0, total_b = 0;
            if (hipMemGetInfo(&free_b, &total_b) != hipSuccess) { (void)hipGetLastError(); free_b = 0; }
            if (need > (free_b + ctx->xpack_bytes) / 4) return IG_OK;
        }
        if (ctx->d_xpack) { IG_HIP(ctx, hipStreamSynchronize(ctx->stream)); IG_HIP(ctx, hipFree(ctx->d_xpack)); ctx->d_xpack = nullptr; ctx->xpack_bytes = 0; }
        if (!may_decline) {
            IG_HIP(ctx, hipMalloc((void**)&ctx->d_xpack, need));
        } else if (hipMalloc((void**)&ctx->d_xpack, need) != hipSuccess) { (void)hipGetLastError(); ctx->d_xpack = nullptr; return IG_OK; }
        ctx->xpack_bytes = need;
    }
    ig_prof_scope prof(ctx, "pack_panel", (double)rows * N * 8.0 + (double)need);
    float2* xp = (float2*)ctx->d_xpack;
    const int64_t cap = (int64_t)ctx->num_cu * 16;
    int64_t g = np <= 8 ? (rows * np + BLK - 1) / BLK : (rows + 63) / 64;
    if (g > cap) g = cap;
#define IG_PACK(KERNEL_) hipLaunchKernelGGL(KERNEL_, dim3((unsigned)g), dim3(BLK), 0, ctx->stream, rows, N, X, ldx, xp, xperm)
    if (np == 1)       IG_PACK(k_pack_panel<1>);
    else if (np == 2)  IG_PACK(k_pack_panel<2>);
    else if (np == 4)  IG_PACK(k_pack_panel<4>);
    else if (np == 8)  IG_PACK(k_pack_panel<8>);
    else if (np == 16) IG_PACK(k_pack_panel_tiled<16>);
    else if (np == 32) IG_PACK(k_pack_panel_tiled<32>);
    else               IG_PACK(k_pack_panel_tiled<64>);
#undef IG_PACK
    IG_LAUNCH_CHECK(ctx, "k_pack_panel");
    *packed = xp;
    return IG_OK;
}

namespace {


template <int NC, int NSEG , bool PAIR = false, bool REALW = false>
__global__ void __launch_bounds__(BLK)
k_grid_bricks(const BrickTask* __restrict__ tasks, int ntasks, const BrickRef* __restrict__ btab,
              const BrickEntry* __restrict__ entries , const uint32_t* __restrict__ round_rows,
              const float2* __restrict__ Xp ,
              float2* __restrict__ Y, float2 alpha, const uint32_t* __restrict__ bits,
              int n0, int nm, int bm_log2, int bs_log2, int nbx, int nbm, int st_log2 , int zw ) {
    extern __shared__ float2 acc_all[];
    constexpr int TPR = 64 / NC;
    constexpr int RS = 64 / TPR;
    const int tid = threadIdx.x, lane = tid & 63;
    const int wv = __builtin_amdgcn_readfirstlane(tid >> 6);
    const int task = blockIdx.x * WAVES_PER_BLOCK + wv;
    if (task >= ntasks) return;
    const BrickTask tk = tasks[task];
    const int nb = tk.nb_flags & 0xffff;
    const bool shared = (tk.nb_flags >> 16) & 1;
    const int32_t nent = tk.hi - tk.lo, nround = nent / TPR;
    const int xs_log2 = 4 - st_log2, seg_log2 = xs_log2 + bm_log2 + bs_log2;
    const int BM = 1 << bm_log2, nseg = NSEG ? (PAIR ? 2 * NSEG : NSEG) : 1 << seg_log2, ncell = 16 << (bm_log2 + bs_log2);
    float2* __restrict__ acc = acc_all + (size_t)wv * ncell * NC;
    const int coil = lane % NC, tsub = lane / NC, xround = (lane / NC) % RS;
    constexpr bool REGS = NC == 8;
    const int eslot = REGS ? ((lane & 15) >> 1) * 8 + 2 * (lane >> 4) + (lane & 1) : lane;
    const rsrc_t r_en = REALW ? make_rsrc(reinterpret_cast<const float2*>(entries) + tk.lo) : make_rsrc(entries + tk.lo);
    const rsrc_t r_rr = make_rsrc(round_rows + tk.lo / TPR), r_x = make_rsrc(Xp);

    struct Set { u3 en; uint32_t rid; float2 x; };
    Set s0, s1, s2, s3;
    auto request_samples = [&](Set& s, int st) {
        const int32_t q = st * RS + xround;
        s.rid = (uint32_t)buf_ld_i32(r_rr, q < nround ? (unsigned)q * 4u : IG_OOB);
    };
    auto request_entries = [&](Set& s, int st) {
        const int32_t idx = st * 64 + eslot;
        if (REALW) {
            const float2 t = buf_ld<false>(r_en, idx < nent ? (unsigned)idx * 8u : IG_OOB, 0);
            s.en.x = __float_as_uint(t.x); s.en.y = __float_as_uint(t.y); s.en.z = 0u;
        } else {
            s.en = buf_ld_u3(r_en, idx < nent ? (unsigned)idx * 12u : IG_OOB);
        }
    };
    auto request_rows = [&](Set& s, int st) {
        const int32_t q = st * RS + xround;
        s.x = buf_ld<false>(r_x, q < nround ? (s.rid * (unsigned)NC + (unsigned)coil) * 8u : IG_OOB, 0);
    };
    request_samples(s0, 0);
    request_samples(s1, 1);
    const float2 my_ref = buf_ld<false>(make_rsrc(btab + tk.bt), lane < nb ? (unsigned)lane * 8u : IG_OOB, 0);
    request_entries(s0, 0);
    request_samples(s2, 2);
    request_samples(s3, 3);
    request_entries(s1, 1);
    request_entries(s2, 2);
    request_rows(s0, 0);
    request_samples(s0, 4);
    request_rows(s1, 1);
    int my_end = 0x7fffffff, my_pt = 0, my_bx = 0, my_m0 = 0, my_s0 = 0;
    if (lane < nb) {
        const int brick = (int)__float_as_uint(my_ref.x);
        if (!shared) my_end = (int)__float_as_uint(my_ref.y) - tk.lo;
        my_bx = brick % nbx;
        my_m0 = ((brick / nbx) % nbm) << bm_log2;
        my_s0 = (brick / (nbx * nbm)) << bs_log2;
        my_pt = my_bx * 16 + n0 * (my_m0 + nm * my_s0);
    }
    uint32_t my_mask = 0xffffffffu;
    if (bits) {
        const int nt = n0 >> st_log2;
        const rsrc_t r_bits = make_rsrc(bits);
        uint32_t w[8];
#pragma unroll
        for (int p = 0; p < 8; ++p) {
            const int pair = p * 64 + lane, j = pair >> seg_log2, seg = pair & (nseg - 1);
            const int jbx = __shfl(my_bx, j & 63), jm0 = __shfl(my_m0, j & 63), js0 = __shfl(my_s0, j & 63);
            const int xs = seg & ((1 << xs_log2) - 1), im = (seg >> xs_log2) & (BM - 1), is = seg >> (xs_log2 + bm_log2);
            const int km = jm0 + im, ks = js0 + is;
            const int kmq = km / zw, kmr = km - kmq * zw;
            w[p] = (uint32_t)buf_ld_i32(r_bits, j < nb ? (unsigned)((ks * nt + (jbx << xs_log2) + xs) * zw + kmr) * 4u : IG_OOB) >> kmq;
        }
        my_mask = 0u;
#pragma unroll
        for (int p = 0; p < 8; ++p) {
            const uint64_t bal = __ballot(w[p] & 1u);
            const int first = (p * 64) >> seg_log2, per = 64 >> seg_log2;
            if (lane >= first && lane < first + per)
                my_mask = (uint32_t)(bal >> ((lane - first) << seg_log2)) & (nseg == 32 ? 0xffffffffu : (1u << nseg) - 1u);
        }
    }
    for (int e = lane; e < ncell * NC; e += 64) acc[e] = make_float2(0.f, 0.f);

    int cur = 0;
    int32_t cur_end = __builtin_amdgcn_readlane(my_end, 0);
    auto flush_segment = [&](int pt, uint32_t mask, int seg) {
        const uint32_t flags = PAIR ? (mask >> (2 * seg)) & 3u : (mask >> seg) & 1u;
        if (!flags) return;
        const bool mine = PAIR ? ((flags >> (lane >> 5)) & 1u) != 0 : true;
        const int f_log2 = PAIR ? 3 : st_log2, fx_log2 = 4 - f_log2;
        const int xs = seg & ((1 << fx_log2) - 1), im = (seg >> fx_log2) & (BM - 1), is = seg >> (fx_log2 + bm_log2);
        const int cell0 = (xs << f_log2) + 16 * (im + BM * is);
        float2* src = acc + (size_t)cell0 * NC;
        float2* dst = Y + ((int64_t)pt + (xs << f_log2) + (int64_t)n0 * (im + (int64_t)nm * is)) * NC;
        const int nel = NC << f_log2;
        for (int e = lane; e < nel; e += 64) {
            const float2 o = cmul(alpha, src[e]);
            if (mine) {
                if (shared) {
                    asm volatile("global_atomic_add_f32 %0, %1, off\n\tglobal_atomic_add_f32 %0, %2, off offset:4"
                                 :: "v"(dst + e), "v"(o.x), "v"(o.y) : "memory");
                } else {
                    asm volatile("global_store_dwordx2 %0, %1, off" :: "v"(dst + e), "v"(o) : "memory");
                }
            }
            src[e] = make_float2(0.f, 0.f);
        }
    };
    auto flush = [&]() {
        const int pt = __builtin_amdgcn_readlane(my_pt, cur);
        const uint32_t mask = (uint32_t)__builtin_amdgcn_readlane((int)my_mask, cur);
        if (NSEG) {
#pragma unroll
            for (int seg = 0; seg < (NSEG ? NSEG : 1); ++seg) flush_segment(pt, mask, seg);
        } else {
            for (int seg = 0; seg < nseg; ++seg) flush_segment(pt, mask, seg);
        }
        ++cur;
        cur_end = __builtin_amdgcn_readlane(my_end, cur & 63);
    };
    auto super_trip = [&](const Set& s, Set& next, Set& rows_ahead, Set& entries_ahead, int st) {
        const uint32_t e_cell = s.en.x, e_re = s.en.y, e_im = s.en.z;
        const float x_re = s.x.x, x_im = s.x.y;
        request_rows(rows_ahead, st + 2);
        request_entries(entries_ahead, st + 3);
        request_samples(next, st + 5);
        auto accumulate = [&](uint32_t cell, float vr, float vi, float xr, float xi) {
            if (cell != 0xffffffffu) {
                float2* a = acc + (int)cell * NC + coil;
                float2 v = *a;
                if (REALW) {
                    v.x = fmaf(vr, xr, v.x);
                    v.y = fmaf(vr, xi, v.y);
                } else {
                    v.x += fmaf(vr, xr, vi * xi);
                    v.y += fmaf(vr, xi, -vi * xr);
                }
                *a = v;
            }
        };
        if constexpr (REGS) {
            int ur[4], ui[4];
            {
                const unsigned wr = __float_as_uint(x_re), wi = __float_as_uint(x_im);
                const auto hr = __builtin_amdgcn_permlane32_swap(wr, wr, false, false);
                const auto hi = __builtin_amdgcn_permlane32_swap(wi, wi, false, false);
                const auto r01 = __builtin_amdgcn_permlane16_swap(hr[0], hr[0], false, false), r23 = __builtin_amdgcn_permlane16_swap(hr[1], hr[1], false, false);
                const auto i01 = __builtin_amdgcn_permlane16_swap(hi[0], hi[0], false, false), i23 = __builtin_amdgcn_permlane16_swap(hi[1], hi[1], false, false);
                ur[0] = (int)r01[0]; ur[1] = (int)r01[1]; ur[2] = (int)r23[0]; ur[3] = (int)r23[1];
                ui[0] = (int)i01[0]; ui[1] = (int)i01[1]; ui[2] = (int)i23[0]; ui[3] = (int)i23[1];
            }
            int ec = (int)e_cell, ew = (int)e_re, ez = (int)e_im;
            auto round = [&](int start, auto half) -> bool {
                constexpr int H = decltype(half)::value;
                if (start >= nent) return false;
                if (start >= cur_end) flush();
                constexpr int LO = 0x150 + 2 * H, HI = 0x151 + 2 * H;
                const uint32_t cell = (uint32_t)__builtin_amdgcn_update_dpp(__builtin_amdgcn_mov_dpp(ec, LO, 0xf, 0x3, false), ec, HI, 0xf, 0xc, false);
                const float vr = __int_as_float(__builtin_amdgcn_update_dpp(__builtin_amdgcn_mov_dpp(ew, LO, 0xf, 0x3, false), ew, HI, 0xf, 0xc, false));
                const float vi = REALW ? 0.f : __int_as_float(__builtin_amdgcn_update_dpp(__builtin_amdgcn_mov_dpp(ez, LO, 0xf, 0x3, false), ez, HI, 0xf, 0xc, false));
                const float xr = __int_as_float(__builtin_amdgcn_update_dpp(ur[0], ur[0], 0x128, 0xf, H ? 0x3 : 0xc, false));
                const float xi = __int_as_float(__builtin_amdgcn_update_dpp(ui[0], ui[0], 0x128, 0xf, H ? 0x3 : 0xc, false));
                accumulate(cell, vr, vi, xr, xi);
                return true;
            };
#pragma unroll 1
            for (int p = 0; p < RS / 2; ++p) {
                const int32_t start = st * 64 + p * 2 * TPR;
                if (!round(start, std::integral_constant<int, 0>())) break;
                if (!round(start + TPR, std::integral_constant<int, 1>())) break;
                ec = __builtin_amdgcn_mov_dpp(ec, 0x12c, 0xf, 0xf, false);
                ew = __builtin_amdgcn_mov_dpp(ew, 0x12c, 0xf, 0xf, false);
                if (!REALW) ez = __builtin_amdgcn_mov_dpp(ez, 0x12c, 0xf, 0xf, false);
                ur[0] = ur[1]; ur[1] = ur[2]; ur[2] = ur[3];
                ui[0] = ui[1]; ui[1] = ui[2]; ui[2] = ui[3];
            }
        } else {
            for (int r = 0; r < RS; ++r) {
                const int32_t start = st * 64 + r * TPR;
                if (start >= nent) break;
                if (start >= cur_end) flush();
                const int from_e = (r * TPR + tsub) * 4, from_x = (r * NC + coil) * 4;
                const uint32_t cell = (uint32_t)__builtin_amdgcn_ds_bpermute(from_e, (int)e_cell);
                const float vr = __int_as_float(__builtin_amdgcn_ds_bpermute(from_e, (int)e_re));
                const float vi = REALW ? 0.f : __int_as_float(__builtin_amdgcn_ds_bpermute(from_e, (int)e_im));
                const float xr = __int_as_float(__builtin_amdgcn_ds_bpermute(from_x, __float_as_int(x_re)));
                const float xi = __int_as_float(__builtin_amdgcn_ds_bpermute(from_x, __float_as_int(x_im)));
                accumulate(cell, vr, vi, xr, xi);
            }
        }
    };
    const int nst = (nent + 63) / 64;
    for (int st = 0; st < nst; st += 4) {
        super_trip(s0, s1, s2, s3, st);
        super_trip(s1, s2, s3, s0, st + 1);
        super_trip(s2, s3, s0, s1, st + 2);
        super_trip(s3, s0, s1, s2, st + 3);
    }
    flush();
}

struct SlotEntry { uint32_t cell; float re, im; uint32_t row; };

template <int NC, bool REALW = false>
__global__ void __launch_bounds__(BLK)
k_grid_slots(const BrickTask* __restrict__ tasks, int ntasks, const BrickRef* __restrict__ btab,
             const int32_t* __restrict__ slot_ptr, const SlotEntry* __restrict__ entries,
             const float2* __restrict__ Xp , float2* __restrict__ Y, float2 alpha,
             const uint32_t* __restrict__ bits, int n0, int nm, int bm_log2, int bs_log2, int nbx, int nbm, int st_log2, int zw ) {
    extern __shared__ float2 acc_all[];
    const int tid = threadIdx.x, lane = tid & 63;
    const int wv = __builtin_amdgcn_readfirstlane(tid >> 6);
    const int task = blockIdx.x * WAVES_PER_BLOCK + wv;
    if (task >= ntasks) return;
    const BrickTask tk = tasks[task];
    const int nb = tk.nb_flags & 0xffff;
    const bool shared = (tk.nb_flags >> 16) & 1;
    const int32_t nslot = tk.hi - tk.lo;
    const int xs_log2 = 4 - st_log2, seg_log2 = xs_log2 + bm_log2 + bs_log2;
    const int BM = 1 << bm_log2, nseg = 1 << seg_log2, ncell = 16 << (bm_log2 + bs_log2);
    float2* __restrict__ acc = acc_all + (size_t)wv * ncell * NC;
    const float2 my_ref = buf_ld<false>(make_rsrc(btab + tk.bt), lane < nb ? (unsigned)lane * 8u : IG_OOB, 0);
    int my_end = 0x7fffffff, my_pt = 0, my_bx = 0, my_m0 = 0, my_s0 = 0;
    if (lane < nb) {
        const int brick = (int)__float_as_uint(my_ref.x);
        if (!shared) my_end = (int)__float_as_uint(my_ref.y) - tk.lo;
        my_bx = brick % nbx;
        my_m0 = ((brick / nbx) % nbm) << bm_log2;
        my_s0 = (brick / (nbx * nbm)) << bs_log2;
        my_pt = my_bx * 16 + n0 * (my_m0 + nm * my_s0);
    }
    uint32_t my_mask = 0xffffffffu;
    if (bits) {
        const int nt = n0 >> st_log2;
        const rsrc_t r_bits = make_rsrc(bits);
        uint32_t w[8];
#pragma unroll
        for (int p = 0; p < 8; ++p) {
            const int pair = p * 64 + lane, j = pair >> seg_log2, seg = pair & (nseg - 1);
            const int jbx = __shfl(my_bx, j & 63), jm0 = __shfl(my_m0, j & 63), js0 = __shfl(my_s0, j & 63);
            const int xs = seg & ((1 << xs_log2) - 1), im = (seg >> xs_log2) & (BM - 1), is = seg >> (xs_log2 + bm_log2);
            const int km = jm0 + im, ks = js0 + is;
            const int kmq = km / zw, kmr = km - kmq * zw;
            w[p] = (uint32_t)buf_ld_i32(r_bits, j < nb ? (unsigned)((ks * nt + (jbx << xs_log2) + xs) * zw + kmr) * 4u : IG_OOB) >> kmq;
        }
        my_mask = 0u;
#pragma unroll
        for (int p = 0; p < 8; ++p) {
            const uint64_t bal = __ballot(w[p] & 1u);
            const int first = (p * 64) >> seg_log2, per = 64 >> seg_log2;
            if (lane >= first && lane < first + per)
                my_mask = (uint32_t)(bal >> ((lane - first) << seg_log2)) & (nseg == 32 ? 0xffffffffu : (1u << nseg) - 1u);
        }
    }
    for (int e = lane; e < ncell * NC; e += 64) acc[e] = make_float2(0.f, 0.f);

    int cur = 0;
    int32_t cur_end = __builtin_amdgcn_readlane(my_end, 0);
    auto flush = [&]() {
        __builtin_amdgcn_fence(__ATOMIC_RELEASE, "wavefront");
        __builtin_amdgcn_wave_barrier();
        __builtin_amdgcn_fence(__ATOMIC_ACQUIRE, "wavefront");
        const int pt = __builtin_amdgcn_readlane(my_pt, cur);
        const uint32_t mask = (uint32_t)__builtin_amdgcn_readlane((int)my_mask, cur);
        for (int seg = 0; seg < nseg; ++seg) {
            if (!((mask >> seg) & 1u)) continue;
            const int xs = seg & ((1 << xs_log2) - 1), im = (seg >> xs_log2) & (BM - 1), is = seg >> (xs_log2 + bm_log2);
            const int cell0 = (xs << st_log2) + 16 * (im + BM * is);
            float2* src = acc + (size_t)cell0 * NC;
            float2* dst = Y + ((int64_t)pt + (xs << st_log2) + (int64_t)n0 * (im + (int64_t)nm * is)) * NC;
            const int nel = NC << st_log2;
            for (int e = lane; e < nel; e += 64) {
                const float2 o = cmul(alpha, src[e]);
                if (shared) {
                    asm volatile("global_atomic_add_f32 %0, %1, off\n\tglobal_atomic_add_f32 %0, %2, off offset:4"
                                 :: "v"(dst + e), "v"(o.x), "v"(o.y) : "memory");
                } else {
                    asm volatile("global_store_dwordx2 %0, %1, off" :: "v"(dst + e), "v"(o) : "memory");
                }
                src[e] = make_float2(0.f, 0.f);
            }
        }
        ++cur;
        cur_end = __builtin_amdgcn_readlane(my_end, cur & 63);
    };

    const rsrc_t r_sp = make_rsrc(slot_ptr + tk.lo), r_en = make_rsrc(entries), r_x = make_rsrc(Xp);
    struct XV { float2 v[NC]; };
    auto load_entry = [&](int32_t off, int32_t n) -> SlotEntry {
        SlotEntry e;
        if (REALW) {
            const u3 q = buf_ld_u3(r_en, lane < n ? (unsigned)(off + lane) * 12u : IG_OOB);
            e.cell = lane < n ? q.x : 0xffffffffu; e.re = __uint_as_float(q.y); e.im = 0.f; e.row = q.z;
        } else {
            const float4 q = buf_ld_f4(r_en, lane < n ? (unsigned)(off + lane) * 16u : IG_OOB);
            e.cell = lane < n ? __float_as_uint(q.x) : 0xffffffffu; e.re = q.y; e.im = q.z; e.row = __float_as_uint(q.w);
        }
        return e;
    };
    auto load_x = [&](const SlotEntry& e) -> XV {
        XV x;
        const unsigned o = e.cell != 0xffffffffu ? e.row * (unsigned)(NC * 8) : IG_OOB;
        if (NC == 1) x.v[0] = buf_ld<false>(r_x, o, 0);
        else {
#pragma unroll
            for (int c = 0; c < NC; c += 2) {
                const float4 q = buf_ld_f4(r_x, o == IG_OOB ? IG_OOB : o + (unsigned)c * 8u);
                x.v[c] = make_float2(q.x, q.y); x.v[c + 1] = make_float2(q.z, q.w);
            }
        }
        return x;
    };
    for (int32_t base = 0; base < nslot; base += 63) {
        const int32_t left = nslot - base, cnt = left < 63 ? left : 63;
        const int32_t sp = buf_ld_i32(r_sp, lane <= cnt ? (unsigned)(base + lane) * 4u : IG_OOB);
        auto slot_off = [&](int i) { return __builtin_amdgcn_readlane(sp, i); };
        SlotEntry e0 = load_entry(slot_off(0), slot_off(1) - slot_off(0));
        SlotEntry e1 = cnt > 1 ? load_entry(slot_off(1), slot_off(2) - slot_off(1)) : SlotEntry{0xffffffffu, 0.f, 0.f, 0u};
        XV x0 = load_x(e0);
#pragma unroll 1
        for (int i = 0; i < cnt; ++i) {
            SlotEntry e2{0xffffffffu, 0.f, 0.f, 0u};
            if (i + 2 < cnt) e2 = load_entry(slot_off(i + 2), slot_off(i + 3) - slot_off(i + 2));
            const XV x1 = load_x(e1);
            if (base + i >= cur_end) flush();
            if (e0.cell != 0xffffffffu) {
#pragma unroll
                for (int c = 0; c < NC; ++c) {
                    float2* a = acc + (int)e0.cell * NC + c;
                    float2 t = *a;
                    if (REALW) {
                        t.x = fmaf(e0.re, x0.v[c].x, t.x);
                        t.y = fmaf(e0.re, x0.v[c].y, t.y);
                    } else {
                        t.x += fmaf(e0.re, x0.v[c].x, e0.im * x0.v[c].y);
                        t.y += fmaf(e0.re, x0.v[c].y, -e0.im * x0.v[c].x);
                    }
                    *a = t;
                }
            }
            e0 = e1; e1 = e2; x0 = x1;
        }
    }
    flush();
}

template <int NC>
__global__ void __launch_bounds__(BLK)
k_grid_bricks_zero(const int32_t* __restrict__ shared_bricks, float2* __restrict__ Y, const uint32_t* __restrict__ bits,
                   int n0, int nm, int bm_log2, int bs_log2, int nbx, int nbm, int st_log2, int zw) {
    const int brick = shared_bricks[blockIdx.x];
    const int xs_log2 = 4 - st_log2;
    const int BM = 1 << bm_log2, nseg = 1 << (xs_log2 + bm_log2 + bs_log2);
// ... 421 lines not shown
                               (const float2*)X, ldx, (float2*)Y_il, K, make_float2(ar, ai), make_float2(0.f, 0.f),
                               mask, nullptr, nullptr, false, true);
}

namespace {
struct RowBricks {
    int64_t id[64]; int32_t cnt[64]; int n = 0;
    bool add(int64_t b) {
        for (int q = 0; q < n; ++q) if (id[q] == b) { ++cnt[q]; return true; }
        if (n == 64) return false;
        id[n] = b; cnt[n] = 1; ++n;
        return true;
    }
};
}

namespace {
struct BrickGeom { int64_t n0, nm, ns, nbx, nbm, nbs, nb; int bm, bs, unit; };
int count_rows(const BrickGeom& g, const int32_t* rowptr, const int32_t* colind, int64_t lo, int64_t hi, int32_t* cnt, int* overflow) {
    const int64_t P = g.n0 * g.nm * g.ns;
    for (int64_t t = lo; t < hi; ++t) {
        RowBricks rb;
        for (int32_t p = rowptr[t]; p < rowptr[t + 1]; ++p) {
            const int64_t col = colind[p];
            if (col < 0 || col >= P) return 1;
            const int64_t kx = col % g.n0, km = (col / g.n0) % g.nm, ks = col / (g.n0 * g.nm);
            if (!rb.add(kx / 16 + g.nbx * (km / g.bm + g.nbm * (ks / g.bs)))) return 2;
        }
        for (int q = 0; q < rb.n; ++q) {
            const int64_t padded = (rb.cnt[q] + g.unit - 1) / g.unit * g.unit;
            if ((int64_t)cnt[rb.id[q]] + padded > 0x7fffffffLL) { *overflow = 1; return 0; }
            cnt[rb.id[q]] += (int32_t)padded;
        }
    }
    return 0;
}
}

int ig_grid_bricks_count(int64_t M, const int32_t* rowptr, const int32_t* colind, int64_t n0, int64_t nm, int64_t ns,
                         int bm, int bs, int unit, int32_t* brick_entries ) {
    if (M < 0 || !rowptr || !brick_entries || !bricks_ok(n0, nm, ns, bm, bs, unit))
        return ig_fail(nullptr, IG_ERR_ARG, "ig_grid_bricks_count: the grid must divide into 16 x bm x bs bricks (powers of two, bm*bs <= 64), unit a power of two <= 64");
    BrickGeom g{n0, nm, ns, n0 / 16, nm / bm, ns / bs, 0, bm, bs, unit};
    g.nb = g.nbx * g.nbm * g.nbs;
    const int nt = brick_threads(M);
    const int64_t per = (M + nt - 1) / nt;
    std::vector<std::vector<int32_t>> cnt((size_t)nt);
    std::vector<int> rc((size_t)nt, 0), ovf((size_t)nt, 0);
    run_threads(nt, [&](int t) {
        cnt[t].assign((size_t)g.nb, 0);
        const int64_t lo = std::min<int64_t>(M, t * per), hi = std::min<int64_t>(M, lo + per);
        rc[t] = count_rows(g, rowptr, colind, lo, hi, cnt[t].data(), &ovf[t]);
    });
    for (int t = 0; t < nt; ++t) {
        if (rc[t] == 1) return ig_fail(nullptr, IG_ERR_ARG, "ig_grid_bricks_count: column index outside the grid");
        if (rc[t] == 2) return ig_fail(nullptr, IG_ERR_UNSUPPORTED, "ig_grid_bricks_count: a row touches more than 64 bricks");
    }
    std::atomic<int> bad{0};
    run_threads(nt, [&](int t) {
        const int64_t pb = (g.nb + nt - 1) / nt, lo = std::min<int64_t>(g.nb, t * pb), hi = std::min<int64_t>(g.nb, lo + pb);
        for (int64_t b = lo; b < hi; ++b) {
            int64_t sum = 0;
            for (int u = 0; u < nt; ++u) sum += cnt[u][b];
            if (sum > 0x7fffffffLL) { bad = 1; sum = 0; }
            brick_entries[b] = (int32_t)sum;
        }
    });
    for (int t = 0; t < nt; ++t) if (ovf[t]) bad = 1;
    if (bad) return ig_fail(nullptr, IG_ERR_ARG, "ig_grid_bricks_count: a brick exceeds 2^31 entries");
    return IG_OK;
}

int ig_grid_bricks_fill(int64_t M, const int32_t* rowptr, const int32_t* colind, const void* vals, int64_t n0, int64_t nm, int64_t ns,
                        int bm, int bs, int unit, const int64_t* brick_ptr ,
                        void* entries ,
                        uint32_t* round_rows ) {
    if (M < 0 || !rowptr || !brick_ptr || !bricks_ok(n0, nm, ns, bm, bs, unit) || (rowptr[M] > rowptr[0] && (!colind || !vals || !entries || !round_rows)))
        return ig_fail(nullptr, IG_ERR_ARG, "ig_grid_bricks_fill: bad arguments");
    BrickGeom g{n0, nm, ns, n0 / 16, nm / bm, ns / bs, 0, bm, bs, unit};
    g.nb = g.nbx * g.nbm * g.nbs;
    const int64_t nbx = g.nbx, nbm = g.nbm;
    const int nt = brick_threads(M);
    const int64_t per = (M + nt - 1) / nt;
    std::vector<std::vector<int32_t>> cur((size_t)nt);
    std::vector<int> rc((size_t)nt, 0), ovf((size_t)nt, 0);
    run_threads(nt, [&](int t) {
        cur[t].assign((size_t)g.nb, 0);
        const int64_t lo = std::min<int64_t>(M, t * per), hi = std::min<int64_t>(M, lo + per);
        rc[t] = count_rows(g, rowptr, colind, lo, hi, cur[t].data(), &ovf[t]);
    });
    for (int t = 0; t < nt; ++t)
        if (rc[t] || ovf[t]) return ig_fail(nullptr, rc[t] == 2 ? IG_ERR_UNSUPPORTED : IG_ERR_ARG, "ig_grid_bricks_fill: the matrix does not fit the brick format (see ig_grid_bricks_count)");
    std::atomic<int> mismatch{0};
    run_threads(nt, [&](int t) {
        const int64_t pb = (g.nb + nt - 1) / nt, lo = std::min<int64_t>(g.nb, t * pb), hi = std::min<int64_t>(g.nb, lo + pb);
        for (int64_t b = lo; b < hi; ++b) {
            int64_t run = 0;
            for (int u = 0; u < nt; ++u) { const int32_t c = cur[u][b]; cur[u][b] = (int32_t)run; run += c; }
            if (run != brick_ptr[b + 1] - brick_ptr[b]) mismatch = 1;
        }
    });
    if (mismatch) return ig_fail(nullptr, IG_ERR_ARG, "ig_grid_bricks_fill: brick_ptr does not come from ig_grid_bricks_count");
    const float2* v = (const float2*)vals;
    BrickEntry* out = (BrickEntry*)entries;
    run_threads(nt, [&](int th) {
        int32_t* cursor = cur[th].data();
        const int64_t lo = std::min<int64_t>(M, th * per), hi = std::min<int64_t>(M, lo + per);
        for (int64_t t = lo; t < hi; ++t) {
            RowBricks rb;
            int64_t start[64];
            for (int32_t p = rowptr[t]; p < rowptr[t + 1]; ++p) {
                const int64_t col = colind[p];
                const int64_t kx = col % n0, km = (col / n0) % nm, ks = col / (n0 * nm);
                const int64_t b = kx / 16 + nbx * (km / bm + nbm * (ks / bs));
                const int before = rb.n;
                rb.add(b);
                int q = 0;
                while (rb.id[q] != b) ++q;
                if (rb.n > before) start[q] = brick_ptr[b] + cursor[b];
                BrickEntry e;
                e.cell = (uint32_t)((kx % 16) + 16 * ((km % bm) + bm * (ks % bs)));
                e.re = v[p].x; e.im = v[p].y;
                out[start[q] + rb.cnt[q] - 1] = e;
            }
            for (int q = 0; q < rb.n; ++q) {
                const int64_t padded = (rb.cnt[q] + unit - 1) / unit * unit;
                for (int64_t i = rb.cnt[q]; i < padded; ++i) {
                    BrickEntry e; e.cell = 0xffffffffu; e.re = 0.f; e.im = 0.f;
                    out[start[q] + i] = e;
                }
                for (int64_t i = 0; i < padded; i += unit) round_rows[(start[q] + i) / unit] = (uint32_t)t;
                cursor[rb.id[q]] += (int32_t)padded;
            }
        }
    });
    return IG_OK;
}

int ig_ccsrmm_t_bricks(ig_ctx* ctx, int64_t M, int64_t K, int64_t N, float ar, float ai,
                       const void* entries, const uint32_t* round_rows, const void* X, int64_t ldx, void* Y_il, const int16_t* support, int64_t n0, int64_t nm,
                       int bm, int bs, const int32_t* tasks, int64_t ntasks, const int32_t* brick_table,
                       const int32_t* shared_bricks, int64_t nshared, int support_tile, int support_zwords, int entry_words) {
    IG_REQUIRE(ctx, ctx != nullptr, "ig_ccsrmm_t_bricks: ctx is NULL");
    IG_REQUIRE(ctx, entry_words == 3 || entry_words == 2, "ig_ccsrmm_t_bricks: entries of 3 words {cell, re, im} or 2 {cell, re} (got %d)", entry_words);
    const bool realw = entry_words == 2;
    const int zw = support_zwords > 0 ? support_zwords : 16;
    IG_REQUIRE(ctx, M >= 0 && K >= 0 && M <= 0x7fffffffLL, "ig_ccsrmm_t_bricks: bad dimensions");
    IG_REQUIRE(ctx, N == 4 || N == 8, "ig_ccsrmm_t_bricks: 4 or 8 columns (got %lld); entries must be padded to 64/N per row and brick", (long long)N);
    IG_REQUIRE(ctx, (ntasks == 0 || (entries && round_rows)) && (M == 0 || X) && (K == 0 || Y_il) && ldx >= M, "ig_ccsrmm_t_bricks: NULL array or short leading dimension");
    IG_REQUIRE(ctx, n0 > 0 && nm > 0 && K % (n0 * nm) == 0 && K < 0x7fffffffLL && bricks_ok(n0, nm, K / (n0 * nm), bm, bs, 8) && bm * bs <= 32,
               "ig_ccsrmm_t_bricks: rows (%lld) are not a grid of n0=%lld x nm=%lld x ... that divides into 16 x %d x %d bricks", (long long)K, (long long)n0, (long long)nm, bm, bs);
    const int64_t ns = K / (n0 * nm);
    IG_REQUIRE(ctx, !support || (zw <= 64 && nm <= 32 * (int64_t)zw), "ig_ccsrmm_t_bricks: the support bitmaps hold 32 bits in each of %d words: nm <= %d", zw, 32 * zw);
    IG_REQUIRE(ctx, support_tile == 16 || support_tile == 8 || support_tile == 4, "ig_ccsrmm_t_bricks: support_tile %d (kx points per entry of the support table: 16, 8 or 4)", support_tile);
    IG_REQUIRE(ctx, (16 / support_tile) * bm * bs <= 32, "ig_ccsrmm_t_bricks: at most 32 segments per brick (%d x %d x %d)", 16 / support_tile, bm, bs);
    const int st_log2 = support_tile == 16 ? 4 : support_tile == 8 ? 3 : 2;
    IG_REQUIRE(ctx, ntasks >= 0 && ntasks <= 0x7fffffffLL && (ntasks == 0 || (tasks && brick_table)) && nshared >= 0 && (nshared == 0 || shared_bricks), "ig_ccsrmm_t_bricks: bad task list");
    IG_REQUIRE(ctx, M * N * 8 < 0x7fffffffLL, "ig_ccsrmm_t_bricks: the panel (%lld x %lld) exceeds the 2 GB window of a buffer descriptor", (long long)M, (long long)N);
    if (K == 0 || ntasks == 0) return IG_OK;
    if (int rc = ig_set_device(ctx)) return rc;
    const int64_t nt = n0 / 16;
    const int64_t snt = n0 / support_tile;
    const uint32_t* bits = support ? reinterpret_cast<const uint32_t*>(support + 2 * (ns * snt + snt)) : nullptr;
    const float2 alpha = make_float2(ar, ai);
    const float2* xp = nullptr;
    if (int rc = ig_pack_panel(ctx, M, N, (int)N, (const float2*)X, ldx, nullptr, false, &xp)) return rc;
    int bm_log2 = 0, bs_log2 = 0;
    while ((1 << bm_log2) < bm) ++bm_log2;
    while ((1 << bs_log2) < bs) ++bs_log2;
    const int nbx = (int)nt, nbm = (int)(nm / bm);
    const size_t lds = (size_t)WAVES_PER_BLOCK * 16 * bm * bs * N * 8;
    IG_REQUIRE(ctx, lds <= 64 * 1024, "ig_ccsrmm_t_bricks: bricks of 16 x %d x %d points x %lld columns need %zu bytes of LDS per workgroup (limit 64 KB)", bm, bs, (long long)N, lds);
    const unsigned blocks = (unsigned)((ntasks + WAVES_PER_BLOCK - 1) / WAVES_PER_BLOCK);
#define IG_BRICKS(NC_, NSEG_) IG_BRICKS_P(NC_, NSEG_, false)
#define IG_BRICKS_P(NC_, NSEG_, PAIR_) do {                                                                                            \
        if (nshared) {                                                                                                          \
            ig_prof_scope prof(ctx, "grid_bricks_zero");                                                                        \
            hipLaunchKernelGGL((k_grid_bricks_zero<NC_>), dim3((unsigned)nshared), dim3(BLK), 0, ctx->stream, shared_bricks, (float2*)Y_il, bits, (int)n0, (int)nm, bm_log2, bs_log2, nbx, nbm, st_log2, zw); } \
        ig_prof_scope prof(ctx, "csrmm_bricks_conj");                                                                           \
        with_flag(realw, [&](auto rw) {                                                                                         \
            hipLaunchKernelGGL((k_grid_bricks<NC_, NSEG_, PAIR_, rw>), dim3(blocks), dim3(BLK), lds, ctx->stream, (const BrickTask*)tasks, (int)ntasks, (const BrickRef*)brick_table, (const BrickEntry*)entries, round_rows, \
                           xp, (float2*)Y_il, alpha, bits, (int)n0, (int)nm, bm_log2, bs_log2, nbx, nbm, st_log2, zw); }); } while (0)
    const int nseg_total = (16 / support_tile) * bm * bs;
    if (N == 8 && nseg_total == 4) IG_BRICKS(8, 4);
    else if (N == 8 && nseg_total == 8) IG_BRICKS(8, 8);
    else if (N == 8 && nseg_total == 16 && support_tile == 4) IG_BRICKS_P(8, 8, true);
    else if (N == 8) IG_BRICKS(8, 0);
    else IG_BRICKS(4, 0);
#undef IG_BRICKS
#undef IG_BRICKS_P
    IG_LAUNCH_CHECK(ctx, "k_grid_bricks");
    return IG_OK;
}

int ig_grid_slots_build(int64_t nbricks, const int64_t* brick_ptr, const void* entries12, const uint32_t* entry_rows, int ncell,
                        void* entries16, int32_t* brick_slots, int32_t* slot_ptr, int64_t* nslots) {
    if (nbricks < 0 || !brick_ptr || ncell < 1 || ncell > 1024 || !brick_slots || !slot_ptr || !nslots ||
        (brick_ptr[nbricks] > 0 && (!entries12 || !entry_rows || !entries16)) || brick_ptr[nbricks] > 0x7fffffffLL)
        return ig_fail(nullptr, IG_ERR_ARG, "ig_grid_slots_build: bad arguments");
    const BrickEntry* in = (const BrickEntry*)entries12;
    SlotEntry* out = (SlotEntry*)entries16;
    const int nt = brick_threads(nbricks * 8);
    const int64_t per = (nbricks + nt - 1) / nt;
    std::atomic<int> bad{0};
    run_threads(nt, [&](int th) {
        std::vector<int32_t> mult((size_t)ncell), gsize;
        const int64_t lo = std::min<int64_t>(nbricks, th * per), hi = std::min<int64_t>(nbricks, lo + per);
        for (int64_t b = lo; b < hi; ++b) {
            const int64_t p0 = brick_ptr[b], p1 = brick_ptr[b + 1];
            if (p1 == p0) { brick_slots[b] = 0; continue; }
            std::fill(mult.begin(), mult.end(), 0);
            gsize.clear();
            for (int64_t p = p0; p < p1; ++p) {
                const uint32_t c = in[p].cell;
                if (c >= (uint32_t)ncell) { bad = 1; continue; }
                const int k = mult[c]++;
                if ((size_t)k >= gsize.size()) gsize.push_back(0);
                ++gsize[k];
            }
            int64_t ns = 0;
            for (int32_t g : gsize) ns += (g + 63) / 64;
            brick_slots[b] = (int32_t)ns;
        }
    });
    if (bad) return ig_fail(nullptr, IG_ERR_ARG, "ig_grid_slots_build: a cell index outside the brick");
    std::vector<int64_t> first((size_t)nbricks + 1, 0);
    for (int64_t b = 0; b < nbricks; ++b) first[b + 1] = first[b] + brick_slots[b];
    if (first[nbricks] > 0x7fffffffLL) return ig_fail(nullptr, IG_ERR_ARG, "ig_grid_slots_build: more than 2^31 - 1 slots");
    *nslots = first[nbricks];
    run_threads(nt, [&](int th) {
        std::vector<int32_t> mult((size_t)ncell), gstart;
        std::vector<int32_t> gsize;
        const int64_t lo = std::min<int64_t>(nbricks, th * per), hi = std::min<int64_t>(nbricks, lo + per);
        for (int64_t b = lo; b < hi; ++b) {
            const int64_t p0 = brick_ptr[b], p1 = brick_ptr[b + 1];
            if (p1 == p0) continue;
            std::fill(mult.begin(), mult.end(), 0);
            gsize.clear();
            for (int64_t p = p0; p < p1; ++p) {
                const int k = mult[in[p].cell]++;
                if ((size_t)k >= gsize.size()) gsize.push_back(0);
                ++gsize[k];
            }
            gstart.assign(gsize.size() + 1, 0);
            for (size_t k = 0; k < gsize.size(); ++k) gstart[k + 1] = gstart[k] + gsize[k];
            int64_t s = first[b];
            for (size_t k = 0; k < gsize.size(); ++k)
                for (int32_t o = 0; o < gsize[k]; o += 64) slot_ptr[s++] = (int32_t)(p0 + gstart[k] + o);
            std::fill(mult.begin(), mult.end(), 0);
            std::vector<int32_t> cursor(gstart.begin(), gstart.end() - 1);
            for (int64_t p = p0; p < p1; ++p) {
                const int k = mult[in[p].cell]++;
                SlotEntry e; e.cell = in[p].cell; e.re = in[p].re; e.im = in[p].im; e.row = entry_rows[p];
                out[p0 + cursor[k]++] = e;
            }
        }
    });
    slot_ptr[first[nbricks]] = (int32_t)brick_ptr[nbricks];
    return IG_OK;
}

int ig_ccsrmm_t_slots(ig_ctx* ctx, int64_t M, int64_t K, int64_t N, float ar, float ai,
                      const void* entries16, const int32_t* slot_ptr, const void* X, int64_t ldx, void* Y_il, const int16_t* support,
                      int64_t n0, int64_t nm, int bm, int bs, const int32_t* tasks, int64_t ntasks, const int32_t* brick_table,
                      const int32_t* shared_bricks, int64_t nshared, int support_tile, int support_zwords, int entry_words) {
    IG_REQUIRE(ctx, ctx != nullptr, "ig_ccsrmm_t_slots: ctx is NULL");
    IG_REQUIRE(ctx, entry_words == 4 || entry_words == 3, "ig_ccsrmm_t_slots: entries of 4 words {cell, re, im, row} or 3 {cell, re, row} (got %d)", entry_words);
    const bool realw = entry_words == 3;
    const int zw = support_zwords > 0 ? support_zwords : 16;
    IG_REQUIRE(ctx, M >= 0 && K >= 0 && M <= 0x7fffffffLL, "ig_ccsrmm_t_slots: bad dimensions");
    IG_REQUIRE(ctx, N == 1 || N == 2 || N == 4, "ig_ccsrmm_t_slots: 1, 2 or 4 columns (got %lld; at 8 the round format of ig_ccsrmm_t_bricks is faster: 0.77 against 1.28 ms)", (long long)N);
    IG_REQUIRE(ctx, (ntasks == 0 || (entries16 && slot_ptr)) && (M == 0 || X) && (K == 0 || Y_il) && ldx >= M, "ig_ccsrmm_t_slots: NULL array or short leading dimension");
    IG_REQUIRE(ctx, n0 > 0 && nm > 0 && K % (n0 * nm) == 0 && K < 0x7fffffffLL && bricks_ok(n0, nm, K / (n0 * nm), bm, bs, 1) && bm * bs <= 32,
               "ig_ccsrmm_t_slots: rows (%lld) are not a grid of n0=%lld x nm=%lld x ... that divides into 16 x %d x %d bricks", (long long)K, (long long)n0, (long long)nm, bm, bs);
    const int64_t ns = K / (n0 * nm);
    IG_REQUIRE(ctx, !support || (zw <= 64 && nm <= 32 * (int64_t)zw), "ig_ccsrmm_t_slots: the support bitmaps hold 32 bits in each of %d words: nm <= %d", zw, 32 * zw);
    IG_REQUIRE(ctx, support_tile == 16 || support_tile == 8 || support_tile == 4, "ig_ccsrmm_t_slots: support_tile %d", support_tile);
    IG_REQUIRE(ctx, (16 / support_tile) * bm * bs <= 32, "ig_ccsrmm_t_slots: at most 32 segments per brick");
    const int st_log2 = support_tile == 16 ? 4 : support_tile == 8 ? 3 : 2;
    IG_REQUIRE(ctx, ntasks >= 0 && ntasks <= 0x7fffffffLL && (ntasks == 0 || (tasks && brick_table)) && nshared >= 0 && (nshared == 0 || shared_bricks), "ig_ccsrmm_t_slots: bad task list");
    IG_REQUIRE(ctx, M * N * 8 < 0x7fffffffLL, "ig_ccsrmm_t_slots: the panel exceeds the 2 GB window of a buffer descriptor");
    if (K == 0 || ntasks == 0) return IG_OK;
    if (int rc = ig_set_device(ctx)) return rc;
    const int64_t snt = n0 / support_tile;
    const uint32_t* bits = support ? reinterpret_cast<const uint32_t*>(support + 2 * (ns * snt + snt)) : nullptr;
    const float2 alpha = make_float2(ar, ai);
    const float2* xp = (const float2*)X;
    if (N > 1)
        if (int rc = ig_pack_panel(ctx, M, N, (int)N, (const float2*)X, ldx, nullptr, false, &xp)) return rc;
    int bm_log2 = 0, bs_log2 = 0;
    while ((1 << bm_log2) < bm) ++bm_log2;
    while ((1 << bs_log2) < bs) ++bs_log2;
    const int nbx = (int)(n0 / 16), nbm = (int)(nm / bm);
    const size_t lds = (size_t)WAVES_PER_BLOCK * 16 * bm * bs * N * 8;
    IG_REQUIRE(ctx, lds <= 64 * 1024, "ig_ccsrmm_t_slots: brick images need %zu bytes of LDS per workgroup (limit 64 KB)", lds);
    const unsigned blocks = (unsigned)((ntasks + WAVES_PER_BLOCK - 1) / WAVES_PER_BLOCK);
#define IG_SLOTS(NC_) do {                                                                                                      \
        if (nshared) {                                                                                                          \
            ig_prof_scope prof(ctx, "grid_bricks_zero");                                                                        \
            hipLaunchKernelGGL((k_grid_bricks_zero<NC_>), dim3((unsigned)nshared), dim3(BLK), 0, ctx->stream, shared_bricks, (float2*)Y_il, bits, (int)n0, (int)nm, bm_log2, bs_log2, nbx, nbm, st_log2, zw); } \
        ig_prof_scope prof(ctx, "csrmm_slots_conj");                                                                            \
        with_flag(realw, [&](auto rw) {                                                                                         \
            hipLaunchKernelGGL((k_grid_slots<NC_, rw>), dim3(blocks), dim3(BLK), lds, ctx->stream, (const BrickTask*)tasks, (int)ntasks, (const BrickRef*)brick_table, slot_ptr, (const SlotEntry*)entries16, \
                           xp, (float2*)Y_il, alpha, bits, (int)n0, (int)nm, bm_log2, bs_log2, nbx, nbm, st_log2, zw); }); } while (0)
    if (N == 1) IG_SLOTS(1); else if (N == 2) IG_SLOTS(2); else IG_SLOTS(4);
#undef IG_SLOTS
    IG_LAUNCH_CHECK(ctx, "k_grid_slots");
    return IG_OK;
}


int ig_csr_inspect(const int32_t* rowptr, const int32_t* colind, int64_t M, int64_t K,
                   int64_t* nzrow, int64_t* nzcol, int* exwrite) {
    if (!rowptr || !nzrow || !nzcol || !exwrite || M < 0 || K < 0)
        return ig_fail(nullptr, IG_ERR_ARG, "ig_csr_inspect: bad arguments");
    std::vector<uint8_t> seen((size_t)K, 0);
    int64_t rows = 0;
    for (int64_t m = 0; m < M; ++m) {
        const int32_t b = rowptr[m], e = rowptr[m + 1];
        if (e < b) return ig_fail(nullptr, IG_ERR_ARG, "ig_csr_inspect: rowptr not monotone at row %lld", (long long)m);
        if (e > b) ++rows;
        for (int32_t p = b; p < e; ++p) {
            const int32_t k = colind[p];
            if (k < 0 || k >= K)
                return ig_fail(nullptr, IG_ERR_ARG, "ig_csr_inspect: column index %d out of range at nnz %d", k, p);
            if (seen[k] < 2) ++seen[k];
        }
    }
    int64_t cols = 0;
    int exw = 1;
    for (int64_t k = 0; k < K; ++k) {
        if (seen[k]) ++cols;
        if (seen[k] > 1) exw = 0;
    }
    *nzrow = rows; *nzcol = cols; *exwrite = exw;
    return IG_OK;
}

int ig_csr_transpose(int64_t M, int64_t K, int64_t nnz,
                     const int32_t* rowptr, const int32_t* colind, const void* vals,
                     int32_t* rowptr_t, int32_t* colind_t, void* vals_t) {
    if (M < 0 || K < 0 || nnz < 0 || !rowptr || !rowptr_t || (nnz > 0 && (!colind || !vals || !colind_t || !vals_t)))
        return ig_fail(nullptr, IG_ERR_ARG, "ig_csr_transpose: bad arguments");
// ... 28 lines not shown
```

indigo_amd/fused.py:

```python
import numpy as np
import scipy.sparse as spp

_C64 = np.dtype('complex64')


def permute_grid_columns(G, oN, order=(0, 2, 1)):
    n = [int(v) for v in oN]
    o = [int(a) for a in order]
    G = G.tocsr()
    idx = G.indices.astype(np.int64)
    k = (idx % n[0], (idx // n[0]) % n[1], idx // (n[0] * n[1]))
    out = spp.csr_matrix((G.data, (k[o[0]] + n[o[0]] * (k[o[1]] + n[o[1]] * k[o[2]])).astype(np.int32), G.indptr), shape=G.shape)
    out.sort_indices()
    return out


def image_permutation(backend, grid, ncoils=None):
    grid = tuple(int(v) for v in grid)
    if len(grid) != 3 or backend.supports_padded_fft(grid, ncoils):
        return None
    import itertools
    ok = [p for p in itertools.permutations(range(3))
          if p != (0, 1, 2) and backend.supports_padded_fft(tuple(grid[a] for a in p), ncoils)]
    if not ok:
        return None
    return min(ok, key=lambda p: (grid[p[0]] % 16 != 0, sum(p[a] != a for a in range(3)) != 2, p))


def touched_columns(G):
    c = getattr(G, '_ig_touched_columns', None)
    if c is None:
        mark = np.zeros(G.shape[1], dtype=bool)
        mark[G.indices] = True
        c = np.flatnonzero(mark)
        try:
            G._ig_touched_columns = c
        except AttributeError:
            pass
    return c


def grid_support(G, oN, tile=16, zw=(16, 16)):
    from indigo_amd import _lib
    n0, n1, n2 = (int(n) for n in oN)
    zi, zo = (int(v) for v in zw)
    assert n0 % tile == 0 and n2 <= 32 * min(zi, zo) and tile in (2, 4, 8, 16)
    nt = n0 // tile
    idx = np.ascontiguousarray(G.indices, dtype=np.int32)
    table = np.empty(2 * (n1 * nt + nt) + 2 * n1 * nt * (zi + (zo if zo != zi else 0)), dtype=np.int16)
    _lib.check(_lib.lib().ig_grid_support(idx.size, idx.ctypes.data, n0, n1, n2, int(tile), zi, zo, table.ctypes.data), None, "ig_grid_support")
    return table


def grid_support_numpy(G, oN, tile=16, zw=(16, 16)):
    n0, n1, n2 = (int(n) for n in oN)
    zi, zo = (int(v) for v in zw)
    assert n0 % tile == 0 and n2 <= 32 * min(zi, zo) and tile in (2, 4, 8, 16)
    nt = n0 // tile
    cols = touched_columns(G)
    kx = cols % n0
    kz = (cols // n0) % n2
    ky = cols // (n0 * n2)
    key = ky * nt + kx // tile
    bits = np.zeros((n1 * nt, zi), dtype=np.uint32)
    np.bitwise_or.at(bits, (key, kz % zi), np.uint32(1) << (kz // zi).astype(np.uint32))
    bits_out = None
    if zo != zi:
        bits_out = np.zeros((n1 * nt, zo), dtype=np.uint32)
        np.bitwise_or.at(bits_out, (key, kz % zo), np.uint32(1) << (kz // zo).astype(np.uint32))
    order = np.argsort(key, kind='stable')
    key, kz = key[order], kz[order]
    ranges = np.zeros((n1 * nt + nt, 2), dtype=np.int16)
    if key.size:
        starts = np.flatnonzero(np.r_[True, key[1:] != key[:-1]])
        ranges[key[starts], 0] = np.minimum.reduceat(kz, starts)
        ranges[key[starts], 1] = np.maximum.reduceat(kz, starts) + 1
    nonempty = (ranges[:n1 * nt, 1] > ranges[:n1 * nt, 0]).reshape(n1, nt)
    for t in range(nt):
        ys = np.flatnonzero(nonempty[:, t])
        if ys.size:
            ranges[n1 * nt + t] = (ys[0], ys[-1] + 1)
    parts = [ranges.reshape(-1), bits.reshape(-1).view(np.int16)]
    if bits_out is not None:
        parts.append(bits_out.reshape(-1).view(np.int16))
    return np.concatenate(parts)


def support_words(backend, oN):
    f = getattr(backend, 'support_words', None)
    if f is None or int(oN[0]) % 16:
        return None
    return f(int(oN[2]))


def split_support(table, oN, tile=16, zw_in=16):
    n0, n1, n2 = (int(n) for n in oN)
    nt = n0 // tile
    table = np.ascontiguousarray(table, dtype=np.int16).reshape(-1)
    a, b = 2 * n1 * nt, 2 * (n1 * nt + nt)
    return table[:a].reshape(-1, 2), table[a:b].reshape(-1, 2), table[b:b + 2 * n1 * nt * zw_in].view(np.uint32).reshape(n1 * nt, zw_in)


def pow2_divisor(n, cap):
    b = int(cap)
    while b > 1 and int(n) % b:
        b //= 2
    return max(b, 1)


CHUNK_COST = {16: 13.0, 8: 6.6, 4: 3.9, 2: 2.45, 1: 1.7}


def plan_chunks(Cn, chunk=8, single_ok=True, cost=None, pad=True):
    cost = dict(CHUNK_COST, **(cost or {}))
    widths = [w for w in (16, 8, 4, 2) if w <= max(int(chunk), 2)] + ([1] if single_ok else [])
    best = [(0.0, [])]
    for c in range(1, int(Cn) + 1):
        cand = [(best[max(c - w, 0)][0] + cost[w], best[max(c - w, 0)][1] + [w]) for w in widths if pad or w <= c]
        if not cand:
            cand = [(best[max(c - w, 0)][0] + cost[w], best[max(c - w, 0)][1] + [w]) for w in widths]
        best.append(min(cand, key=lambda t: (round(t[0], 6), len(t[1]))))
    out, lo = [], 0
    for w in sorted(best[int(Cn)][1], reverse=True):
        hi = min(lo + w, int(Cn))
        out.append((lo, hi, w))
        lo = hi
    return out


def coil_chunks(Cn, chunk=8):
    return [(lo, hi) for lo, hi, _ in plan_chunks(Cn, chunk)]


def choose_layout(Cn, chunk=8, layout=None, single_ok=True, cost=None, pad=True):
    if layout in (0, 1):
        return layout, [(0, int(Cn), 0)]
    chunks = plan_chunks(Cn, chunk, single_ok, cost, pad)
    return (2 if any(w > 1 for _, _, w in chunks) else 1), chunks


def pad_coils(w, width, interleaved=True):
    w = np.asarray(w)
    box, c = w.shape[:3], w.shape[3]
    if c == width:
        return w
    out = np.zeros(box[::-1] + (width,), dtype=_C64).transpose(2, 1, 0, 3) if interleaved else np.zeros(box + (width,), dtype=_C64, order='F')
    out[..., :c] = w
    return out


def assemble(backend, Gm, oN, N, weights_of, Cn, layout, chunks, table=None, box_lo=None, row_order=None,
             name='SENSE-fusedFFT', zw=(16, 16), sep=None, kshift=None):
    from indigo_amd import operators as op
    tuning = getattr(backend, 'tuning', {})
    chunks = [(c[0], c[1], (c[2] if len(c) > 2 else (c[1] - c[0] if layout == 2 else 0))) for c in chunks]
    il_widths = sorted({w for _, _, w in chunks if w > 1}, reverse=True)
    x16 = int(oN[0]) % 16 == 0

    tile_of = tuning.get('support_tile', 8)
    fine = {}
    by_tile = {}
    for w in il_widths:
        tile = int(tile_of.get(w, 8) if isinstance(tile_of, dict) else tile_of)
        if (table is not None and tile in (4, 8) and w * tile >= 32 and getattr(backend, 'supports_support_tile', False)
                and (w in tuning.get('bricks', ()) or (sep is not None and w in tuning.get('shares', ())))):
            if tile not in by_tile:
                by_tile[tile] = grid_support(Gm, oN, tile, zw)
            fine[w] = (by_tile[tile], tile)

    def gridding(interleaved, ncols=0):
        G = backend.SpMatrix(Gm, name='interp*mod*scale')
        if interleaved:
            G._grid_interleaved = True
            if sep is not None and tuning.get('separable', True):
                G._grid_separable = sep
        if table is not None:
            G._grid_support = (table, int(oN[0]), int(oN[2]), int(zw[0]))
        if row_order is not None:
            G._row_order = row_order
            return G
        bricks, slots, fines, shares = {}, {}, {}, {}
        for w in (il_widths if interleaved else [ncols]):
            if (interleaved and sep is not None and tuning.get('separable', True) and w in tuning.get('shares', ()) and x16
                    and sep['tw'] >= tuning.get('shares_min_tw', 6)):
                sshape = tuning.get('share_shape', {})
                sshape = tuple(sshape.get(w, (8, 2, 1024, 1024)) if isinstance(sshape, dict) else sshape)
                shares[w] = (int(sshape[0]), int(sshape[1])) + sshape[2:]
                if w in fine:
                    fines[w] = fine[w]
            elif interleaved and w in tuning.get('bricks', ()) and x16:
                shape = tuning.get('brick_shape', {})
                shape = shape.get(w, (2, 2, 4096, 4096)) if isinstance(shape, dict) else shape
                bricks[w] = (int(oN[0]), int(oN[2]), int(oN[1]), w, pow2_divisor(oN[2], shape[0]), pow2_divisor(oN[1], shape[1])) + tuple(shape[2:])
                if w in fine:
                    fines[w] = fine[w]
            elif w in tuning.get('slots', ()) and x16:
                sshape = tuple(tuning.get('slot_shape', (4, 4, 256, 64)))
                slots[w] = (int(oN[0]), int(oN[2]), int(oN[1]), w, pow2_divisor(oN[2], sshape[0]), pow2_divisor(oN[1], sshape[1])) + sshape[2:]
        if fines:
            G._grid_support_fine = fines
        if shares:
            G._grid_shares = shares
        if bricks:
            G._grid_bricks = bricks
        if slots:
            G._grid_slots = slots
        return G

    G_il = gridding(True) if il_widths else None
    kskw = {'kshift': tuple(int(v) for v in kshift)} if (kshift is not None and any(kshift)) else {}
    assert not kskw or all(w > 1 for _, _, w in chunks), "a transform that carries an axis shift exists for the coil-interleaved layout only"
    G_pc = None
    trees = []
    for lo, hi, w in chunks:
        real = hi - lo
        if w > 1:
            wts = pad_coils(weights_of(lo, hi), w)
            if w in fine:
                Z = backend.ZpadFFT(oN, N, wts, box_lo=box_lo, layout=2, support=fine[w][0], support_tile=fine[w][1], name='fft*zpad*apod*maps', **kskw)
            else:
                Z = backend.ZpadFFT(oN, N, wts, box_lo=box_lo, layout=2, support=table, name='fft*zpad*apod*maps', **kskw)
            Z._coil_range = (lo, hi)
            tree = backend.KronI(w, G_il) * Z
            if real < w:
                tree = op.HeadRows(backend, tree, real * Gm.shape[0], name='coils %d..%d of a %d-wide chunk' % (lo, hi, w))
        else:
            lay = layout if layout in (0, 1) else 1
            G_pc = G_pc or gridding(False, real)
            Z = backend.ZpadFFT(oN, N, weights_of(lo, hi), box_lo=box_lo, layout=lay, support=table if lay == 1 else None, name='fft*zpad*apod*maps')
            Z._coil_range = (lo, hi)
            tree = backend.KronI(real, G_pc) * Z
        trees.append(tree)
    A = trees[0] if len(trees) == 1 else backend.VStack(trees, name='coil-chunks')
    A._name = name
    A._support_fine = fine.get(il_widths[0]) if il_widths else None
    A._support_fine_by_width = fine
    A._support_zw = tuple(int(v) for v in zw)
    A._coil_chunks = chunks
    return A


def decode_zpad_maps(St, C, P, oN):
    St = St.tocsr()
    if St.shape[1] != C * P or St.nnz == 0:
        return None
    rows = np.repeat(np.arange(St.shape[0], dtype=np.int64), np.diff(St.indptr))
    return decode_zpad_entries(rows, St.indices.astype(np.int64), St.data, St.shape[0], C, P, oN)


def decode_zpad_entries(rows, cols, data, Nn, C, P, oN):
    rows, cols = np.asarray(rows, dtype=np.int64), np.asarray(cols, dtype=np.int64)
    Nn = int(Nn)
    if rows.size == 0 or cols.min() < 0 or cols.max() >= C * P or rows.min() < 0 or rows.max() >= Nn:
        return None
    coil, pos = cols // P, cols % P
    zrow = np.full(Nn, -1, dtype=np.int64)
    zrow[rows] = pos
    if not np.array_equal(pos, zrow[rows]):
        return None
    if np.bincount(rows * C + coil, minlength=Nn * C).max() > 1:
        return None
    present = np.flatnonzero(zrow >= 0)
    n0, n1, n2 = (int(n) for n in oN)
    z = zrow[present]
    kx, ky, kz = z % n0, (z // n0) % n1, z // (n0 * n1)
    if rows.size == Nn * C:
        dims = (int(kx.max() - kx.min()) + 1, int(ky.max() - ky.min()) + 1, int(kz.max() - kz.min()) + 1)
    else:
        Amat = np.stack([ky, kz, np.ones_like(ky)], axis=1).astype(np.float64)
        if np.linalg.matrix_rank(Amat) < 3:
            return None
        sol = np.linalg.lstsq(Amat, (present - kx).astype(np.float64), rcond=None)[0]
        d0, d01 = int(round(sol[0])), int(round(sol[1]))
        if d0 < 1 or d01 < d0 or d01 % d0 or Nn % d01:
            return None
        dims = (d0, d01 // d0, Nn // d01)
    if dims[0] * dims[1] * dims[2] != Nn:
        return None
    ix, iy, iz = present % dims[0], (present // dims[0]) % dims[1], present // (dims[0] * dims[1])
    lo = (int(kx[0] - ix[0]), int(ky[0] - iy[0]), int(kz[0] - iz[0]))
    if not (np.array_equal(kx, lo[0] + ix) and np.array_equal(ky, lo[1] + iy) and np.array_equal(kz, lo[2] + iz)):
        return None
    if min(lo) < 0 or lo[0] + dims[0] > n0 or lo[1] + dims[1] > n1 or lo[2] + dims[2] > n2:
        return None
    w = np.zeros((Nn, C), dtype=_C64)
    w[rows, coil] = np.conj(data)
    return lo, dims, np.asfortranarray(w).reshape(dims + (C,), order='F')
```

Baseline: 169.1.

## Support finer support tiles with paired FFT range records and quad-split brick flushes

Allows a support tile of 2 kx points (tile*coils == 16) and adds a quad-split brick gridding kernel that flushes at the finer tile granularity. The kernel body moves into a shared include so it can be instantiated both ways. The w32 FFT pass gains a 'pair' mode that merges two adjacent tile range records and bitmasks per wave-half, so it can still be selected under the finer tiling. The aim is to skip more empty grid regions in the scatter and FFT passes, at the cost of more support-table reads and extra readlane or hull logic.

```diff
diff --git a/indigo_amd/backends/hip_csr.py b/indigo_amd/backends/hip_csr.py
--- a/indigo_amd/backends/hip_csr.py
+++ b/indigo_amd/backends/hip_csr.py
@@ -70,7 +70,7 @@
         built, key = self._bricks_by, None if ncols is None else int(ncols)
         assert not (any(v is not None for v in built.values()) if key is None else built.get(key) is not None), \
             "set_grid_support_fine must come before set_grid_bricks: the runs of bricks are sized for the table's segments"
-        assert int(tile) in (4, 8, 16)
+        assert int(tile) in (2, 4, 8, 16)
         self._support_fine = (self._backend.copy_array(np.ascontiguousarray(table, dtype=np.int16).reshape(-1),
                                                        name=self._name + ".supportFine"), int(tile))
         self._support_fine_by[key] = self._support_fine
diff --git a/indigo_amd/csrc/ig_fft.hip b/indigo_amd/csrc/ig_fft.hip
--- a/indigo_amd/csrc/ig_fft.hip
+++ b/indigo_amd/csrc/ig_fft.hip
@@ -313,7 +313,7 @@
     int in_lo = d.in_lo, in_hi = d.in_hi, out_lo = d.out_lo, out_hi = d.out_hi;
     short2 k1r = make_short2(0, 0x7fff), trg = make_short2(0, 0x7fff);
     PassRecords rcd{0u, 0u, 0x7fff0000u, 0xffffffffu, false, false, false, true, false};
-    if (BOXED && !AXIS0) rcd = pass_records(d, tw, tr, k1, 16, t, true);
+    if (BOXED && !AXIS0) rcd = pass_records<W == 32>(d, tw, tr, k1, 16, t, true, (unsigned)w >> 4);
     const bool has_k1r = rcd.has_k1r, has_trg = rcd.has_trg, has_zb = rcd.has_zb;
     int64_t o_in = k0u * d.in_s[0], o_out = k0u * d.out_s[0];
     if (BOXED && !AXIS0 && WMODE == 0 && d.zc_log2) {
@@ -372,6 +372,7 @@
         gin = 0;
 #pragma unroll
         for (int l = 0; l < 64; l += W) gin |= (uint32_t)__builtin_amdgcn_readlane((int)ibits, l);
+        if (W == 32 && rcd.pair) gin |= (uint32_t)__builtin_amdgcn_readlane((int)ibits, 16) | (uint32_t)__builtin_amdgcn_readlane((int)ibits, 48);
     }
     constexpr bool GATE_ST = BOXED && !AXIS0 && WMODE == 0 && !HALF_OUT && HALF != 3;
     uint32_t gout = 0xffffffffu;
@@ -423,6 +424,7 @@
         gout = 0;
 #pragma unroll
         for (int l = 0; l < 64; l += W) gout |= (uint32_t)__builtin_amdgcn_readlane((int)obits, l);
+        if (W == 32 && rcd.pair) gout |= (uint32_t)__builtin_amdgcn_readlane((int)obits, 16) | (uint32_t)__builtin_amdgcn_readlane((int)obits, 48);
     }
     if (TW_LATE) {
 #pragma unroll
@@ -1058,7 +1060,7 @@
     const bool w32_generic = half == 0 && (big_stride || d.tile_bits != nullptr);
     const bool w32 = (ax.n == 512 && !axis0 && wmode == 0 && !d.cw && d.ext0 % 32 == 0 &&
         (half == 1 || half == 3 || half == 2 || half == 4 || w32_generic) &&
-        (!d.tile_range || d.tile_shift >= 1));
+        (!d.tile_range || d.tile_shift >= 1 || d.tile_pair));
     return d.wide ? d.wide == 2 : w32;
 }
 
@@ -1087,7 +1089,7 @@
     const bool w32 = two_stage_variant(ax, d, axis0, wmode, boxed, half);
     if (w32) {
         PassDesc d2 = d;
-        if (d2.tile_range) d2.tile_shift = d.tile_shift - 1;
+        if (d2.tile_range && d.tile_shift >= 1) { d2.tile_shift = d.tile_shift - 1; d2.tile_pair = 0; }
         const dim3 g2 = pass_grid(d2, d.ext0 / 32), b2(512);
         const size_t lds2 = ((size_t)16 * 16 * 32 + 512) * 8;
         if (!ctx->fft_w32_attr) {
@@ -1562,6 +1564,7 @@
     int64_t mid_base;
     int64_t snt;
     int tile_shift;
+    bool tile_pair;
     int zw_in, zw_out;
     int64_t hull_y, bits, bits_out;
 };
@@ -1586,6 +1589,7 @@
     if (p->layout >= 1) {
         g.snt = n0 / p->support_tile;
         g.tile_shift = g.interleaved ? lg2((int)(C * p->support_tile / 16)) : 0;
+        g.tile_pair = g.interleaved && p->support_tile < 16 && C * p->support_tile == 16;
         g.zw_in = p->zw_in; g.zw_out = p->zw_out;
         g.hull_y = n1 * g.snt; g.bits = g.hull_y + g.snt;
         g.bits_out = g.zw_out != g.zw_in ? n1 * g.snt * g.zw_in : 0;
@@ -1633,14 +1637,14 @@
 
 static PassDesc pass_y(const PaddedGeom& g, bool inverse, const PaddedBufs& m, const short2* support, int64_t z0, int64_t nz) {
     PassDesc d = pass_desc(g, 1, inverse, m.mid - g.l[1] * g.mid[1] + z0 * g.mid[2], g.mid, m.full + (g.l[2] + z0) * g.grid[2], g.grid, g.n[0], nz);
-    if (support) { d.tile_range = support + g.hull_y; d.tile_range_mode = inverse ? 2 : 1; d.tile_range_k1 = 0; d.tile_shift = g.tile_shift; }
+    if (support) { d.tile_range = support + g.hull_y; d.tile_range_mode = inverse ? 2 : 1; d.tile_range_k1 = 0; d.tile_shift = g.tile_shift; d.tile_pair = g.tile_pair; }
     return d;
 }
 
 static PassDesc pass_z(const PaddedGeom& g, bool inverse, const PaddedBufs& m, const short2* support) {
     PassDesc d = pass_desc(g, 2, inverse, m.full, g.grid, m.grid, g.grid, g.n[0], g.n[1]);
     if (g.snt) {
-        d.tile_range = support; d.tile_range_mode = inverse ? 2 : 1; d.tile_range_k1 = g.snt; d.tile_shift = g.tile_shift;
+        d.tile_range = support; d.tile_range_mode = inverse ? 2 : 1; d.tile_range_k1 = g.snt; d.tile_shift = g.tile_shift; d.tile_pair = support && g.tile_pair;
     }
     if (support) {
         d.tile_bits = reinterpret_cast<const uint32_t*>(support + g.bits) + (inverse ? 0 : g.bits_out);
diff --git a/indigo_amd/csrc/ig_fft_ab.h b/indigo_amd/csrc/ig_fft_ab.h
--- a/indigo_amd/csrc/ig_fft_ab.h
+++ b/indigo_amd/csrc/ig_fft_ab.h
@@ -25,6 +25,7 @@
     int zc_log2;
     int64_t in_zt, out_zt;
     int wide;
+    int tile_pair;
 };
 
 
@@ -34,21 +35,50 @@
     if (d.grid3) { tr = blockIdx.x; k1 = blockIdx.y; k2 = blockIdx.z; }
     else { const unsigned tile = blockIdx.x, rest = tile / d.tpr; tr = tile % d.tpr; k1 = rest % (unsigned)d.ext1; k2 = rest / (unsigned)d.ext1; }
 }
+__device__ __forceinline__ uint32_t range_hull(uint32_t a, uint32_t b) {
+    const uint32_t lo = (a & 0xffffu) < (b & 0xffffu) ? (a & 0xffffu) : (b & 0xffffu), hi = (a >> 16) > (b >> 16) ? (a >> 16) : (b >> 16);
+    return lo | (hi << 16);
+}
 struct PassRecords {
     uint32_t rec_v, rec_s, hull_s, zb_raw;
     bool has_k1r, has_trg, has_zb, word_ok, scalar;
-    __device__ __forceinline__ short2 k1_hull() const { return make_short2((short)(hull_s & 0xffffu), (short)(hull_s >> 16)); }
+    uint32_t rec_s2, hull_s2;
+    bool pair;
+    __device__ __forceinline__ short2 k1_hull() const {
+        uint32_t a = hull_s;
+        if (pair) a = range_hull(hull_s, hull_s2);
+        return make_short2((short)(a & 0xffffu), (short)(a >> 16));
+    }
     __device__ __forceinline__ short2 range() const {
-        const uint32_t a = scalar ? rec_s : (uint32_t)__builtin_amdgcn_readfirstlane((int)rec_v);
+        uint32_t a;
+        if (pair) a = scalar ? range_hull(rec_s, rec_s2)
+                             : range_hull((uint32_t)__builtin_amdgcn_readlane((int)rec_v, 0), (uint32_t)__builtin_amdgcn_readlane((int)rec_v, 16));
+        else a = scalar ? rec_s : (uint32_t)__builtin_amdgcn_readfirstlane((int)rec_v);
         return make_short2((short)(a & 0xffffu), (short)(a >> 16));
     }
     __device__ __forceinline__ uint32_t bits() const { return has_zb ? (word_ok ? zb_raw : 0u) : 0xffffffffu; }
 };
-__device__ __forceinline__ PassRecords pass_records(const PassDesc& d, const void* safe, unsigned tr, unsigned k1, int words, int word, bool word_ok) {
+template <bool PAIR_OK = false>
+__device__ __forceinline__ PassRecords pass_records(const PassDesc& d, const void* safe, unsigned tr, unsigned k1, int words, int word, bool word_ok, unsigned half = 0) {
     PassRecords r;
     r.rec_v = 0; r.rec_s = 0; r.hull_s = 0x7fff0000u; r.zb_raw = 0xffffffffu; r.word_ok = word_ok;
+    r.rec_s2 = 0; r.hull_s2 = 0x7fff0000u;
     r.has_k1r = d.k1_range != nullptr; r.has_trg = d.tile_range != nullptr; r.has_zb = d.tile_bits != nullptr;
     r.scalar = r.has_trg && d.tile_range_k1 == 0;
+    r.pair = PAIR_OK && d.tile_pair != 0;
+    if (PAIR_OK && r.pair) {
+        const unsigned es = 2u * tr;
+        if (r.has_k1r) { r.hull_s = *reinterpret_cast<const uint32_t*>(d.k1_range + es); r.hull_s2 = *reinterpret_cast<const uint32_t*>(d.k1_range + (es + 1u)); }
+        if (r.scalar) { r.rec_s = *reinterpret_cast<const uint32_t*>(d.tile_range + es); r.rec_s2 = *reinterpret_cast<const uint32_t*>(d.tile_range + (es + 1u)); }
+        if ((r.has_trg && !r.scalar) || r.has_zb) {
+            const int64_t tidx = (int64_t)k1 * d.tile_range_k1 + es;
+            const uint32_t* pt = (r.has_trg && !r.scalar) ? reinterpret_cast<const uint32_t*>(d.tile_range + tidx) + half : reinterpret_cast<const uint32_t*>(safe);
+            const uint32_t* pb = (r.has_zb && word_ok) ? d.tile_bits + tidx * words + (half * (unsigned)words + (unsigned)word) : reinterpret_cast<const uint32_t*>(safe);
+            r.zb_raw = *pb;
+            r.rec_v = *pt;
+        }
+        return r;
+    }
     if (r.has_k1r) r.hull_s = *reinterpret_cast<const uint32_t*>(d.k1_range + (tr >> d.tile_shift));
     if (r.scalar) r.rec_s = *reinterpret_cast<const uint32_t*>(d.tile_range + (tr >> d.tile_shift));
     if ((r.has_trg && !r.scalar) || r.has_zb) {
diff --git a/indigo_amd/csrc/ig_grid_bricks_body.inc b/indigo_amd/csrc/ig_grid_bricks_body.inc
--- /dev/null
+++ b/indigo_amd/csrc/ig_grid_bricks_body.inc
@@ -0,0 +1,202 @@
+    extern __shared__ float2 acc_all[];
+    constexpr int TPR = 64 / NC;
+    constexpr int RS = 64 / TPR;
+    const int tid = threadIdx.x, lane = tid & 63;
+    const int wv = __builtin_amdgcn_readfirstlane(tid >> 6);
+    const int task = blockIdx.x * WAVES_PER_BLOCK + wv;
+    if (task >= ntasks) return;
+    const BrickTask tk = tasks[task];
+    const int nb = tk.nb_flags & 0xffff;
+    const bool shared = (tk.nb_flags >> 16) & 1;
+    const int32_t nent = tk.hi - tk.lo, nround = nent / TPR;
+    const int xs_log2 = 4 - st_log2, seg_log2 = xs_log2 + bm_log2 + bs_log2;
+    const int BM = 1 << bm_log2, nseg = NSEG ? SPLIT * NSEG : 1 << seg_log2, ncell = 16 << (bm_log2 + bs_log2);
+    float2* __restrict__ acc = acc_all + (size_t)wv * ncell * NC;
+    const int coil = lane % NC, tsub = lane / NC, xround = (lane / NC) % RS;
+    constexpr bool REGS = NC == 8;
+    const int eslot = REGS ? ((lane & 15) >> 1) * 8 + 2 * (lane >> 4) + (lane & 1) : lane;
+    const rsrc_t r_en = REALW ? make_rsrc(reinterpret_cast<const float2*>(entries) + tk.lo) : make_rsrc(entries + tk.lo);
+    const rsrc_t r_rr = make_rsrc(round_rows + tk.lo / TPR), r_x = make_rsrc(Xp);
+
+    struct Set { u3 en; uint32_t rid; float2 x; };
+    Set s0, s1, s2, s3;
+    auto request_samples = [&](Set& s, int st) {
+        const int32_t q = st * RS + xround;
+        s.rid = (uint32_t)buf_ld_i32(r_rr, q < nround ? (unsigned)q * 4u : IG_OOB);
+    };
+    auto request_entries = [&](Set& s, int st) {
+        const int32_t idx = st * 64 + eslot;
+        if (REALW) {
+            const float2 t = buf_ld<false>(r_en, idx < nent ? (unsigned)idx * 8u : IG_OOB, 0);
+            s.en.x = __float_as_uint(t.x); s.en.y = __float_as_uint(t.y); s.en.z = 0u;
+        } else {
+            s.en = buf_ld_u3(r_en, idx < nent ? (unsigned)idx * 12u : IG_OOB);
+        }
+    };
+    auto request_rows = [&](Set& s, int st) {
+        const int32_t q = st * RS + xround;
+        s.x = buf_ld<false>(r_x, q < nround ? (s.rid * (unsigned)NC + (unsigned)coil) * 8u : IG_OOB, 0);
+    };
+    request_samples(s0, 0);
+    request_samples(s1, 1);
+    const float2 my_ref = buf_ld<false>(make_rsrc(btab + tk.bt), lane < nb ? (unsigned)lane * 8u : IG_OOB, 0);
+    request_entries(s0, 0);
+    request_samples(s2, 2);
+    request_samples(s3, 3);
+    request_entries(s1, 1);
+    request_entries(s2, 2);
+    request_rows(s0, 0);
+    request_samples(s0, 4);
+    request_rows(s1, 1);
+    int my_end = 0x7fffffff, my_pt = 0, my_bx = 0, my_m0 = 0, my_s0 = 0;
+    if (lane < nb) {
+        const int brick = (int)__float_as_uint(my_ref.x);
+        if (!shared) my_end = (int)__float_as_uint(my_ref.y) - tk.lo;
+        my_bx = brick % nbx;
+        my_m0 = ((brick / nbx) % nbm) << bm_log2;
+        my_s0 = (brick / (nbx * nbm)) << bs_log2;
+        my_pt = my_bx * 16 + n0 * (my_m0 + nm * my_s0);
+    }
+    uint32_t my_mask = 0xffffffffu;
+    if (bits) {
+        const int nt = n0 >> st_log2;
+        const rsrc_t r_bits = make_rsrc(bits);
+        uint32_t w[8];
+#pragma unroll
+        for (int p = 0; p < 8; ++p) {
+            const int pair = p * 64 + lane, j = pair >> seg_log2, seg = pair & (nseg - 1);
+            const int jbx = __shfl(my_bx, j & 63), jm0 = __shfl(my_m0, j & 63), js0 = __shfl(my_s0, j & 63);
+            const int xs = seg & ((1 << xs_log2) - 1), im = (seg >> xs_log2) & (BM - 1), is = seg >> (xs_log2 + bm_log2);
+            const int km = jm0 + im, ks = js0 + is;
+            const int kmq = km / zw, kmr = km - kmq * zw;
+            w[p] = (uint32_t)buf_ld_i32(r_bits, j < nb ? (unsigned)((ks * nt + (jbx << xs_log2) + xs) * zw + kmr) * 4u : IG_OOB) >> kmq;
+        }
+        my_mask = 0u;
+#pragma unroll
+        for (int p = 0; p < 8; ++p) {
+            const uint64_t bal = __ballot(w[p] & 1u);
+            const int first = (p * 64) >> seg_log2, per = 64 >> seg_log2;
+            if (lane >= first && lane < first + per)
+                my_mask = (uint32_t)(bal >> ((lane - first) << seg_log2)) & (nseg == 32 ? 0xffffffffu : (1u << (SPLIT * NSEG >= 32 ? 0 : nseg)) - 1u);
+        }
+    }
+    for (int e = lane; e < ncell * NC; e += 64) acc[e] = make_float2(0.f, 0.f);
+
+    int cur = 0;
+    int32_t cur_end = __builtin_amdgcn_readlane(my_end, 0);
+    auto flush_segment = [&](int pt, uint32_t mask, int seg) {
+        const uint32_t flags = (mask >> (SPLIT * seg)) & ((1u << SPLIT) - 1u);
+        if (!flags) return;
+        const bool mine = PAIR ? ((flags >> (lane >> (SPLIT == 4 ? 4 : 5))) & 1u) != 0 : true;
+        constexpr int G_LOG2 = NC == 8 ? 3 : NC == 4 ? 4 : 0;
+        static_assert(!PAIR || G_LOG2 != 0, "split flushes: 8 or 4 columns");
+        const int f_log2 = PAIR ? G_LOG2 : st_log2, fx_log2 = 4 - f_log2;
+        const int xs = seg & ((1 << fx_log2) - 1), im = (seg >> fx_log2) & (BM - 1), is = seg >> (fx_log2 + bm_log2);
+        const int cell0 = (xs << f_log2) + 16 * (im + BM * is);
+        float2* src = acc + (size_t)cell0 * NC;
+        float2* dst = Y + ((int64_t)pt + (xs << f_log2) + (int64_t)n0 * (im + (int64_t)nm * is)) * NC;
+        const int nel = NC << f_log2;
+        for (int e = lane; e < nel; e += 64) {
+            const float2 o = cmul(alpha, src[e]);
+            if (mine) {
+                if (shared) {
+                    asm volatile("global_atomic_add_f32 %0, %1, off\n\tglobal_atomic_add_f32 %0, %2, off offset:4"
+                                 :: "v"(dst + e), "v"(o.x), "v"(o.y) : "memory");
+                } else {
+                    asm volatile("global_store_dwordx2 %0, %1, off" :: "v"(dst + e), "v"(o) : "memory");
+                }
+            }
+            src[e] = make_float2(0.f, 0.f);
+        }
+    };
+    auto flush = [&]() {
+        const int pt = __builtin_amdgcn_readlane(my_pt, cur);
+        const uint32_t mask = (uint32_t)__builtin_amdgcn_readlane((int)my_mask, cur);
+        if (NSEG) {
+#pragma unroll
+            for (int seg = 0; seg < (NSEG ? NSEG : 1); ++seg) flush_segment(pt, mask, seg);
+        } else {
+            for (int seg = 0; seg < nseg; ++seg) flush_segment(pt, mask, seg);
+        }
+        ++cur;
+        cur_end = __builtin_amdgcn_readlane(my_end, cur & 63);
+    };
+    auto super_trip = [&](const Set& s, Set& next, Set& rows_ahead, Set& entries_ahead, int st) {
+        const uint32_t e_cell = s.en.x, e_re = s.en.y, e_im = s.en.z;
+        const float x_re = s.x.x, x_im = s.x.y;
+        request_rows(rows_ahead, st + 2);
+        request_entries(entries_ahead, st + 3);
+        request_samples(next, st + 5);
+        auto accumulate = [&](uint32_t cell, float vr, float vi, float xr, float xi) {
+            if (cell != 0xffffffffu) {
+                float2* a = acc + (int)cell * NC + coil;
+                float2 v = *a;
+                if (REALW) {
+                    v.x = fmaf(vr, xr, v.x);
+                    v.y = fmaf(vr, xi, v.y);
+                } else {
+                    v.x += fmaf(vr, xr, vi * xi);
+                    v.y += fmaf(vr, xi, -vi * xr);
+                }
+                *a = v;
+            }
+        };
+        if constexpr (REGS) {
+            int ur[4], ui[4];
+            {
+                const unsigned wr = __float_as_uint(x_re), wi = __float_as_uint(x_im);
+                const auto hr = __builtin_amdgcn_permlane32_swap(wr, wr, false, false);
+                const auto hi = __builtin_amdgcn_permlane32_swap(wi, wi, false, false);
+                const auto r01 = __builtin_amdgcn_permlane16_swap(hr[0], hr[0], false, false), r23 = __builtin_amdgcn_permlane16_swap(hr[1], hr[1], false, false);
+                const auto i01 = __builtin_amdgcn_permlane16_swap(hi[0], hi[0], false, false), i23 = __builtin_amdgcn_permlane16_swap(hi[1], hi[1], false, false);
+                ur[0] = (int)r01[0]; ur[1] = (int)r01[1]; ur[2] = (int)r23[0]; ur[3] = (int)r23[1];
+                ui[0] = (int)i01[0]; ui[1] = (int)i01[1]; ui[2] = (int)i23[0]; ui[3] = (int)i23[1];
+            }
+            int ec = (int)e_cell, ew = (int)e_re, ez = (int)e_im;
+            auto round = [&](int start, auto half) -> bool {
+                constexpr int H = decltype(half)::value;
+                if (start >= nent) return false;
+                if (start >= cur_end) flush();
+                constexpr int LO = 0x150 + 2 * H, HI = 0x151 + 2 * H;
+                const uint32_t cell = (uint32_t)__builtin_amdgcn_update_dpp(__builtin_amdgcn_mov_dpp(ec, LO, 0xf, 0x3, false), ec, HI, 0xf, 0xc, false);
+                const float vr = __int_as_float(__builtin_amdgcn_update_dpp(__builtin_amdgcn_mov_dpp(ew, LO, 0xf, 0x3, false), ew, HI, 0xf, 0xc, false));
+                const float vi = REALW ? 0.f : __int_as_float(__builtin_amdgcn_update_dpp(__builtin_amdgcn_mov_dpp(ez, LO, 0xf, 0x3, false), ez, HI, 0xf, 0xc, false));
+                const float xr = __int_as_float(__builtin_amdgcn_update_dpp(ur[0], ur[0], 0x128, 0xf, H ? 0x3 : 0xc, false));
+                const float xi = __int_as_float(__builtin_amdgcn_update_dpp(ui[0], ui[0], 0x128, 0xf, H ? 0x3 : 0xc, false));
+                accumulate(cell, vr, vi, xr, xi);
+                return true;
+            };
+#pragma unroll 1
+            for (int p = 0; p < RS / 2; ++p) {
+                const int32_t start = st * 64 + p * 2 * TPR;
+                if (!round(start, std::integral_constant<int, 0>())) break;
+                if (!round(start + TPR, std::integral_constant<int, 1>())) break;
+                ec = __builtin_amdgcn_mov_dpp(ec, 0x12c, 0xf, 0xf, false);
+                ew = __builtin_amdgcn_mov_dpp(ew, 0x12c, 0xf, 0xf, false);
+                if (!REALW) ez = __builtin_amdgcn_mov_dpp(ez, 0x12c, 0xf, 0xf, false);
+                ur[0] = ur[1]; ur[1] = ur[2]; ur[2] = ur[3];
+                ui[0] = ui[1]; ui[1] = ui[2]; ui[2] = ui[3];
+            }
+        } else {
+            for (int r = 0; r < RS; ++r) {
+                const int32_t start = st * 64 + r * TPR;
+                if (start >= nent) break;
+                if (start >= cur_end) flush();
+                const int from_e = (r * TPR + tsub) * 4, from_x = (r * NC + coil) * 4;
+                const uint32_t cell = (uint32_t)__builtin_amdgcn_ds_bpermute(from_e, (int)e_cell);
+                const float vr = __int_as_float(__builtin_amdgcn_ds_bpermute(from_e, (int)e_re));
+                const float vi = REALW ? 0.f : __int_as_float(__builtin_amdgcn_ds_bpermute(from_e, (int)e_im));
+                const float xr = __int_as_float(__builtin_amdgcn_ds_bpermute(from_x, __float_as_int(x_re)));
+                const float xi = __int_as_float(__builtin_amdgcn_ds_bpermute(from_x, __float_as_int(x_im)));
+                accumulate(cell, vr, vi, xr, xi);
+            }
+        }
+    };
+    const int nst = (nent + 63) / 64;
+    for (int st = 0; st < nst; st += 4) {
+        super_trip(s0, s1, s2, s3, st);
+        super_trip(s1, s2, s3, s0, st + 1);
+        super_trip(s2, s3, s0, s1, st + 2);
+        super_trip(s3, s0, s1, s2, st + 3);
+    }
+    flush();
diff --git a/indigo_amd/csrc/ig_spmm.hip b/indigo_amd/csrc/ig_spmm.hip
--- a/indigo_amd/csrc/ig_spmm.hip
+++ b/indigo_amd/csrc/ig_spmm.hip
@@ -910,214 +910,26 @@
 namespace {
 
 
+#define IG_BRICK_PARAMS const BrickTask* __restrict__ tasks, int ntasks, const BrickRef* __restrict__ btab,                                 \
+              const BrickEntry* __restrict__ entries , const uint32_t* __restrict__ round_rows,               \
+              const float2* __restrict__ Xp ,                                                                    \
+              float2* __restrict__ Y, float2 alpha, const uint32_t* __restrict__ bits,                                                     \
+              int n0, int nm, int bm_log2, int bs_log2, int nbx, int nbm, int st_log2 , int zw
 template <int NC, int NSEG , bool PAIR = false, bool REALW = false>
 __global__ void __launch_bounds__(BLK)
-k_grid_bricks(const BrickTask* __restrict__ tasks, int ntasks, const BrickRef* __restrict__ btab,
-              const BrickEntry* __restrict__ entries , const uint32_t* __restrict__ round_rows,
-              const float2* __restrict__ Xp ,
-              float2* __restrict__ Y, float2 alpha, const uint32_t* __restrict__ bits,
-              int n0, int nm, int bm_log2, int bs_log2, int nbx, int nbm, int st_log2 , int zw ) {
-    extern __shared__ float2 acc_all[];
-    constexpr int TPR = 64 / NC;
-    constexpr int RS = 64 / TPR;
-    const int tid = threadIdx.x, lane = tid & 63;
-    const int wv = __builtin_amdgcn_readfirstlane(tid >> 6);
-    const int task = blockIdx.x * WAVES_PER_BLOCK + wv;
-    if (task >= ntasks) return;
-    const BrickTask tk = tasks[task];
-    const int nb = tk.nb_flags & 0xffff;
-    const bool shared = (tk.nb_flags >> 16) & 1;
-    const int32_t nent = tk.hi - tk.lo, nround = nent / TPR;
-    const int xs_log2 = 4 - st_log2, seg_log2 = xs_log2 + bm_log2 + bs_log2;
-    const int BM = 1 << bm_log2, nseg = NSEG ? (PAIR ? 2 * NSEG : NSEG) : 1 << seg_log2, ncell = 16 << (bm_log2 + bs_log2);
-    float2* __restrict__ acc = acc_all + (size_t)wv * ncell * NC;
-    const int coil = lane % NC, tsub = lane / NC, xround = (lane / NC) % RS;
-    constexpr bool REGS = NC == 8;
-    const int eslot = REGS ? ((lane & 15) >> 1) * 8 + 2 * (lane >> 4) + (lane & 1) : lane;
-    const rsrc_t r_en = REALW ? make_rsrc(reinterpret_cast<const float2*>(entries) + tk.lo) : make_rsrc(entries + tk.lo);
-    const rsrc_t r_rr = make_rsrc(round_rows + tk.lo / TPR), r_x = make_rsrc(Xp);
-
-    struct Set { u3 en; uint32_t rid; float2 x; };
-    Set s0, s1, s2, s3;
-    auto request_samples = [&](Set& s, int st) {
-        const int32_t q = st * RS + xround;
-        s.rid = (uint32_t)buf_ld_i32(r_rr, q < nround ? (unsigned)q * 4u : IG_OOB);
-    };
-    auto request_entries = [&](Set& s, int st) {
-        const int32_t idx = st * 64 + eslot;
-        if (REALW) {
-            const float2 t = buf_ld<false>(r_en, idx < nent ? (unsigned)idx * 8u : IG_OOB, 0);
-            s.en.x = __float_as_uint(t.x); s.en.y = __float_as_uint(t.y); s.en.z = 0u;
-        } else {
-            s.en = buf_ld_u3(r_en, idx < nent ? (unsigned)idx * 12u : IG_OOB);
-        }
-    };
-    auto request_rows = [&](Set& s, int st) {
-        const int32_t q = st * RS + xround;
-        s.x = buf_ld<false>(r_x, q < nround ? (s.rid * (unsigned)NC + (unsigned)coil) * 8u : IG_OOB, 0);
-    };
-    request_samples(s0, 0);
-    request_samples(s1, 1);
-    const float2 my_ref = buf_ld<false>(make_rsrc(btab + tk.bt), lane < nb ? (unsigned)lane * 8u : IG_OOB, 0);
-    request_entries(s0, 0);
-    request_samples(s2, 2);
-    request_samples(s3, 3);
-    request_entries(s1, 1);
-    request_entries(s2, 2);
-    request_rows(s0, 0);
-    request_samples(s0, 4);
-    request_rows(s1, 1);
-    int my_end = 0x7fffffff, my_pt = 0, my_bx = 0, my_m0 = 0, my_s0 = 0;
-    if (lane < nb) {
-        const int brick = (int)__float_as_uint(my_ref.x);
-        if (!shared) my_end = (int)__float_as_uint(my_ref.y) - tk.lo;
-        my_bx = brick % nbx;
-        my_m0 = ((brick / nbx) % nbm) << bm_log2;
-        my_s0 = (brick / (nbx * nbm)) << bs_log2;
-        my_pt = my_bx * 16 + n0 * (my_m0 + nm * my_s0);
-    }
-    uint32_t my_mask = 0xffffffffu;
-    if (bits) {
-        const int nt = n0 >> st_log2;
-        const rsrc_t r_bits = make_rsrc(bits);
-        uint32_t w[8];
-#pragma unroll
-        for (int p = 0; p < 8; ++p) {
-            const int pair = p * 64 + lane, j = pair >> seg_log2, seg = pair & (nseg - 1);
-            const int jbx = __shfl(my_bx, j & 63), jm0 = __shfl(my_m0, j & 63), js0 = __shfl(my_s0, j & 63);
-            const int xs = seg & ((1 << xs_log2) - 1), im = (seg >> xs_log2) & (BM - 1), is = seg >> (xs_log2 + bm_log2);
-            const int km = jm0 + im, ks = js0 + is;
-            const int kmq = km / zw, kmr = km - kmq * zw;
-            w[p] = (uint32_t)buf_ld_i32(r_bits, j < nb ? (unsigned)((ks * nt + (jbx << xs_log2) + xs) * zw + kmr) * 4u : IG_OOB) >> kmq;
-        }
-        my_mask = 0u;
-#pragma unroll
-        for (int p = 0; p < 8; ++p) {
-            const uint64_t bal = __ballot(w[p] & 1u);
-            const int first = (p * 64) >> seg_log2, per = 64 >> seg_log2;
-            if (lane >= first && lane < first + per)
-                my_mask = (uint32_t)(bal >> ((lane - first) << seg_log2)) & (nseg == 32 ? 0xffffffffu : (1u << nseg) - 1u);
-        }
-    }
-    for (int e = lane; e < ncell * NC; e += 64) acc[e] = make_float2(0.f, 0.f);
-
-    int cur = 0;
-    int32_t cur_end = __builtin_amdgcn_readlane(my_end, 0);
-    auto flush_segment = [&](int pt, uint32_t mask, int seg) {
-        const uint32_t flags = PAIR ? (mask >> (2 * seg)) & 3u : (mask >> seg) & 1u;
-        if (!flags) return;
-        const bool mine = PAIR ? ((flags >> (lane >> 5)) & 1u) != 0 : true;
-        const int f_log2 = PAIR ? 3 : st_log2, fx_log2 = 4 - f_log2;
-        const int xs = seg & ((1 << fx_log2) - 1), im = (seg >> fx_log2) & (BM - 1), is = seg >> (fx_log2 + bm_log2);
-        const int cell0 = (xs << f_log2) + 16 * (im + BM * is);
-        float2* src = acc + (size_t)cell0 * NC;
-        float2* dst = Y + ((int64_t)pt + (xs << f_log2) + (int64_t)n0 * (im + (int64_t)nm * is)) * NC;
-        const int nel = NC << f_log2;
-        for (int e = lane; e < nel; e += 64) {
-            const float2 o = cmul(alpha, src[e]);
-            if (mine) {
-                if (shared) {
-                    asm volatile("global_atomic_add_f32 %0, %1, off\n\tglobal_atomic_add_f32 %0, %2, off offset:4"
-                                 :: "v"(dst + e), "v"(o.x), "v"(o.y) : "memory");
-                } else {
-                    asm volatile("global_store_dwordx2 %0, %1, off" :: "v"(dst + e), "v"(o) : "memory");
-                }
-            }
-            src[e] = make_float2(0.f, 0.f);
-        }
-    };
-    auto flush = [&]() {
-        const int pt = __builtin_amdgcn_readlane(my_pt, cur);
-        const uint32_t mask = (uint32_t)__builtin_amdgcn_readlane((int)my_mask, cur);
-        if (NSEG) {
-#pragma unroll
-            for (int seg = 0; seg < (NSEG ? NSEG : 1); ++seg) flush_segment(pt, mask, seg);
-        } else {
-            for (int seg = 0; seg < nseg; ++seg) flush_segment(pt, mask, seg);
-        }
-        ++cur;
-        cur_end = __builtin_amdgcn_readlane(my_end, cur & 63);
-    };
-    auto super_trip = [&](const Set& s, Set& next, Set& rows_ahead, Set& entries_ahead, int st) {
-        const uint32_t e_cell = s.en.x, e_re = s.en.y, e_im = s.en.z;
-        const float x_re = s.x.x, x_im = s.x.y;
-        request_rows(rows_ahead, st + 2);
-        request_entries(entries_ahead, st + 3);
-        request_samples(next, st + 5);
-        auto accumulate = [&](uint32_t cell, float vr, float vi, float xr, float xi) {
-            if (cell != 0xffffffffu) {
-                float2* a = acc + (int)cell * NC + coil;
-                float2 v = *a;
-                if (REALW) {
-                    v.x = fmaf(vr, xr, v.x);
-                    v.y = fmaf(vr, xi, v.y);
-                } else {
-                    v.x += fmaf(vr, xr, vi * xi);
-                    v.y += fmaf(vr, xi, -vi * xr);
-                }
-                *a = v;
-            }
-        };
-        if constexpr (REGS) {
-            int ur[4], ui[4];
-            {
-                const unsigned wr = __float_as_uint(x_re), wi = __float_as_uint(x_im);
-                const auto hr = __builtin_amdgcn_permlane32_swap(wr, wr, false, false);
-                const auto hi = __builtin_amdgcn_permlane32_swap(wi, wi, false, false);
-                const auto r01 = __builtin_amdgcn_permlane16_swap(hr[0], hr[0], false, false), r23 = __builtin_amdgcn_permlane16_swap(hr[1], hr[1], false, false);
-                const auto i01 = __builtin_amdgcn_permlane16_swap(hi[0], hi[0], false, false), i23 = __builtin_amdgcn_permlane16_swap(hi[1], hi[1], false, false);
-                ur[0] = (int)r01[0]; ur[1] = (int)r01[1]; ur[2] = (int)r23[0]; ur[3] = (int)r23[1];
-                ui[0] = (int)i01[0]; ui[1] = (int)i01[1]; ui[2] = (int)i23[0]; ui[3] = (int)i23[1];
-            }
-            int ec = (int)e_cell, ew = (int)e_re, ez = (int)e_im;
-            auto round = [&](int start, auto half) -> bool {
-                constexpr int H = decltype(half)::value;
-                if (start >= nent) return false;
-                if (start >= cur_end) flush();
-                constexpr int LO = 0x150 + 2 * H, HI = 0x151 + 2 * H;
-                const uint32_t cell = (uint32_t)__builtin_amdgcn_update_dpp(__builtin_amdgcn_mov_dpp(ec, LO, 0xf, 0x3, false), ec, HI, 0xf, 0xc, false);
-                const float vr = __int_as_float(__builtin_amdgcn_update_dpp(__builtin_amdgcn_mov_dpp(ew, LO, 0xf, 0x3, false), ew, HI, 0xf, 0xc, false));
-                const float vi = REALW ? 0.f : __int_as_float(__builtin_amdgcn_update_dpp(__builtin_amdgcn_mov_dpp(ez, LO, 0xf, 0x3, false), ez, HI, 0xf, 0xc, false));
-                const float xr = __int_as_float(__builtin_amdgcn_update_dpp(ur[0], ur[0], 0x128, 0xf, H ? 0x3 : 0xc, false));
-                const float xi = __int_as_float(__builtin_amdgcn_update_dpp(ui[0], ui[0], 0x128, 0xf, H ? 0x3 : 0xc, false));
-                accumulate(cell, vr, vi, xr, xi);
-                return true;
-            };
-#pragma unroll 1
-            for (int p = 0; p < RS / 2; ++p) {
-                const int32_t start = st * 64 + p * 2 * TPR;
-                if (!round(start, std::integral_constant<int, 0>())) break;
-                if (!round(start + TPR, std::integral_constant<int, 1>())) break;
-                ec = __builtin_amdgcn_mov_dpp(ec, 0x12c, 0xf, 0xf, false);
-                ew = __builtin_amdgcn_mov_dpp(ew, 0x12c, 0xf, 0xf, false);
-                if (!REALW) ez = __builtin_amdgcn_mov_dpp(ez, 0x12c, 0xf, 0xf, false);
-                ur[0] = ur[1]; ur[1] = ur[2]; ur[2] = ur[3];
-                ui[0] = ui[1]; ui[1] = ui[2]; ui[2] = ui[3];
-            }
-        } else {
-            for (int r = 0; r < RS; ++r) {
-                const int32_t start = st * 64 + r * TPR;
-                if (start >= nent) break;
-                if (start >= cur_end) flush();
-                const int from_e = (r * TPR + tsub) * 4, from_x = (r * NC + coil) * 4;
-                const uint32_t cell = (uint32_t)__builtin_amdgcn_ds_bpermute(from_e, (int)e_cell);
-                const float vr = __int_as_float(__builtin_amdgcn_ds_bpermute(from_e, (int)e_re));
-                const float vi = REALW ? 0.f : __int_as_float(__builtin_amdgcn_ds_bpermute(from_e, (int)e_im));
-                const float xr = __int_as_float(__builtin_amdgcn_ds_bpermute(from_x, __float_as_int(x_re)));
-                const float xi = __int_as_float(__builtin_amdgcn_ds_bpermute(from_x, __float_as_int(x_im)));
-                accumulate(cell, vr, vi, xr, xi);
-            }
-        }
-    };
-    const int nst = (nent + 63) / 64;
-    for (int st = 0; st < nst; st += 4) {
-        super_trip(s0, s1, s2, s3, st);
-        super_trip(s1, s2, s3, s0, st + 1);
-        super_trip(s2, s3, s0, s1, st + 2);
-        super_trip(s3, s0, s1, s2, st + 3);
-    }
-    flush();
-}
+k_grid_bricks(IG_BRICK_PARAMS) {
+    constexpr int SPLIT = PAIR ? 2 : 1;
+#include "ig_grid_bricks_body.inc"
+}
+template <int NC, bool REALW = false>
+__global__ void __launch_bounds__(BLK)
+k_grid_bricks_quad(IG_BRICK_PARAMS) {
+    constexpr int NSEG = 8, SPLIT = 4;
+    constexpr bool PAIR = true;
+    static_assert(NC == 8 || NC == 4, "a wave store of 8 cells x 8 columns or 16 cells x 4");
+#include "ig_grid_bricks_body.inc"
+}
+#undef IG_BRICK_PARAMS
 
 struct SlotEntry { uint32_t cell; float re, im; uint32_t row; };
 
@@ -1845,9 +1657,9 @@
                "ig_ccsrmm_t_bricks: rows (%lld) are not a grid of n0=%lld x nm=%lld x ... that divides into 16 x %d x %d bricks", (long long)K, (long long)n0, (long long)nm, bm, bs);
     const int64_t ns = K / (n0 * nm);
     IG_REQUIRE(ctx, !support || (zw <= 64 && nm <= 32 * (int64_t)zw), "ig_ccsrmm_t_bricks: the support bitmaps hold 32 bits in each of %d words: nm <= %d", zw, 32 * zw);
-    IG_REQUIRE(ctx, support_tile == 16 || support_tile == 8 || support_tile == 4, "ig_ccsrmm_t_bricks: support_tile %d (kx points per entry of the support table: 16, 8 or 4)", support_tile);
+    IG_REQUIRE(ctx, support_tile == 16 || support_tile == 8 || support_tile == 4 || support_tile == 2, "ig_ccsrmm_t_bricks: support_tile %d (kx points per entry of the support table: 16, 8, 4 or 2)", support_tile);
     IG_REQUIRE(ctx, (16 / support_tile) * bm * bs <= 32, "ig_ccsrmm_t_bricks: at most 32 segments per brick (%d x %d x %d)", 16 / support_tile, bm, bs);
-    const int st_log2 = support_tile == 16 ? 4 : support_tile == 8 ? 3 : 2;
+    const int st_log2 = support_tile == 16 ? 4 : support_tile == 8 ? 3 : support_tile == 4 ? 2 : 1;
     IG_REQUIRE(ctx, ntasks >= 0 && ntasks <= 0x7fffffffLL && (ntasks == 0 || (tasks && brick_table)) && nshared >= 0 && (nshared == 0 || shared_bricks), "ig_ccsrmm_t_bricks: bad task list");
     IG_REQUIRE(ctx, M * N * 8 < 0x7fffffffLL, "ig_ccsrmm_t_bricks: the panel (%lld x %lld) exceeds the 2 GB window of a buffer descriptor", (long long)M, (long long)N);
     if (K == 0 || ntasks == 0) return IG_OK;
@@ -1875,13 +1687,23 @@
             hipLaunchKernelGGL((k_grid_bricks<NC_, NSEG_, PAIR_, rw>), dim3(blocks), dim3(BLK), lds, ctx->stream, (const BrickTask*)tasks, (int)ntasks, (const BrickRef*)brick_table, (const BrickEntry*)entries, round_rows, \
                            xp, (float2*)Y_il, alpha, bits, (int)n0, (int)nm, bm_log2, bs_log2, nbx, nbm, st_log2, zw); }); } while (0)
     const int nseg_total = (16 / support_tile) * bm * bs;
-    if (N == 8 && nseg_total == 4) IG_BRICKS(8, 4);
+#define IG_BRICKS_Q(NC_) do {                                                                                                   \
+        if (nshared) {                                                                                                          \
+            ig_prof_scope prof(ctx, "grid_bricks_zero");                                                                        \
+            hipLaunchKernelGGL((k_grid_bricks_zero<NC_>), dim3((unsigned)nshared), dim3(BLK), 0, ctx->stream, shared_bricks, (float2*)Y_il, bits, (int)n0, (int)nm, bm_log2, bs_log2, nbx, nbm, st_log2, zw); } \
+        ig_prof_scope prof(ctx, "csrmm_bricks_conj");                                                                           \
+        with_flag(realw, [&](auto rw) {                                                                                         \
+            hipLaunchKernelGGL((k_grid_bricks_quad<NC_, rw>), dim3(blocks), dim3(BLK), lds, ctx->stream, (const BrickTask*)tasks, (int)ntasks, (const BrickRef*)brick_table, (const BrickEntry*)entries, round_rows, \
+                           xp, (float2*)Y_il, alpha, bits, (int)n0, (int)nm, bm_log2, bs_log2, nbx, nbm, st_log2, zw); }); } while (0)
+    if (nseg_total == 32 && bm * bs == (N == 8 ? 4 : 8) && support_tile * N == 16) { if (N == 8) IG_BRICKS_Q(8); else IG_BRICKS_Q(4); }
+    else if (N == 8 && nseg_total == 4) IG_BRICKS(8, 4);
     else if (N == 8 && nseg_total == 8) IG_BRICKS(8, 8);
     else if (N == 8 && nseg_total == 16 && support_tile == 4) IG_BRICKS_P(8, 8, true);
     else if (N == 8) IG_BRICKS(8, 0);
     else IG_BRICKS(4, 0);
 #undef IG_BRICKS
 #undef IG_BRICKS_P
+#undef IG_BRICKS_Q
     IG_LAUNCH_CHECK(ctx, "k_grid_bricks");
     return IG_OK;
 }
diff --git a/indigo_amd/fused.py b/indigo_amd/fused.py
--- a/indigo_amd/fused.py
+++ b/indigo_amd/fused.py
@@ -157,12 +157,21 @@
     il_widths = sorted({w for _, _, w in chunks if w > 1}, reverse=True)
     x16 = int(oN[0]) % 16 == 0
 
+    def scatter_route(w):
+        if sep is not None and tuning.get('separable', True) and w in tuning.get('shares', ()) and x16 and sep['tw'] >= tuning.get('shares_min_tw', 6):
+            return 'shares'
+        if w in tuning.get('bricks', ()) and x16:
+            return 'bricks'
+        return 'slots' if (w in tuning.get('slots', ()) and x16) else None
+
     tile_of = tuning.get('support_tile', 8)
     fine = {}
     by_tile = {}
     for w in il_widths:
         tile = int(tile_of.get(w, 8) if isinstance(tile_of, dict) else tile_of)
-        if (table is not None and tile in (4, 8) and w * tile >= 32 and getattr(backend, 'supports_support_tile', False)
+        if tile in (2, 4, 8) and w * tile == 16 and scatter_route(w) != 'bricks':
+            tile *= 2
+        if (table is not None and tile in (2, 4, 8) and w * tile >= 16 and int(oN[0]) % tile == 0 and getattr(backend, 'supports_support_tile', False)
                 and (w in tuning.get('bricks', ()) or (sep is not None and w in tuning.get('shares', ())))):
             if tile not in by_tile:
                 by_tile[tile] = grid_support(Gm, oN, tile, zw)
@@ -181,14 +190,13 @@
             return G
         bricks, slots, fines, shares = {}, {}, {}, {}
         for w in (il_widths if interleaved else [ncols]):
-            if (interleaved and sep is not None and tuning.get('separable', True) and w in tuning.get('shares', ()) and x16
-                    and sep['tw'] >= tuning.get('shares_min_tw', 6)):
+            if interleaved and scatter_route(w) == 'shares':
                 sshape = tuning.get('share_shape', {})
                 sshape = tuple(sshape.get(w, (8, 2, 1024, 1024)) if isinstance(sshape, dict) else sshape)
                 shares[w] = (int(sshape[0]), int(sshape[1])) + sshape[2:]
                 if w in fine:
                     fines[w] = fine[w]
-            elif interleaved and w in tuning.get('bricks', ()) and x16:
+            elif interleaved and scatter_route(w) == 'bricks':
                 shape = tuning.get('brick_shape', {})
                 shape = shape.get(w, (2, 2, 4096, 4096)) if isinstance(shape, dict) else shape
                 bricks[w] = (int(oN[0]), int(oN[2]), int(oN[1]), w, pow2_divisor(oN[2], shape[0]), pow2_divisor(oN[1], shape[1])) + tuple(shape[2:])
```

Result: slower. 166.7 (-1.4%).
